# piwell/CS348B-pbrt

Measured on AMD Instinct MI355X. Metric: volumetric photon-gather throughput (camera samples through PhotonVolumeIntegrator::Li per second), higher is better.
Workload: dtype f32

## Files before the change

### cs348b-pbrt_amd/csrc/pvol_api.hip

```cpp
#include <hip/hip_runtime.h>
#include <math.h>
#include <stdlib.h>
#include <string.h>
#include <algorithm>
#include <mutex>
#include <new>
#include <vector>

#include "pvol_dev.h"

#include "pvol_host.h"

static bool ok(hipError_t e) { return e == hipSuccess; }

extern "C" {

int pvol_abi_version(void) { return PVOL_ABI_VERSION; }

const char *pvol_strerror(int s) {
    switch (s) {
    case PVOL_OK: return "ok";
    case PVOL_E_INVALID: return "invalid argument";
    case PVOL_E_NO_DEVICE: return "no usable HIP device (this library has no CPU path)";
    case PVOL_E_NO_SCENE: return "no scene set";
    case PVOL_E_NO_MEMORY: return "out of memory";
    case PVOL_E_UNSUPPORTED: return "unsupported volume/light/material kind or size";
    case PVOL_E_LIMIT: return "a ray needs more march steps than the kernel's LDS plan";
    case PVOL_E_SHOOT_FAILED: return "unable to store enough photons";
    default: return "unknown status";
    }
}

int pvol_device_count(void) {
    int n = 0;
    if (!ok(hipGetDeviceCount(&n))) return 0;
    return n;
}

void pvol_default_params(pvol_params *p) {
    memset(p, 0, sizeof(*p));
    p->step_size = 1.f;
    p->n_used = 250;
    p->max_dist = 0.1f;
    p->n_volume_photons = 0;
    p->shooter_step_size = 0.1f;
    p->max_photon_depth = 5;
    p->n_caustic_photons = 20000;
    p->n_indirect_photons = 10000;
    p->final_gather = 1;
    p->device = 0;
    p->grid_cell_scale = 0.f;
    p->keep_surface_photons = 0;
}

int pvol_create(const pvol_params *params, pvol_ctx **out) {
    if (!params || !out) return PVOL_E_INVALID;
    *out = 0;
    if (params->n_used < 1 || !(params->step_size > 0.f) || !(params->max_dist > 0.f)) return PVOL_E_INVALID;
    if (params->n_used > 576) return PVOL_E_UNSUPPORTED;
    int n = 0;
    if (!ok(hipGetDeviceCount(&n)) || n <= 0 || params->device < 0 || params->device >= n) return PVOL_E_NO_DEVICE;
    if (!ok(hipSetDevice(params->device))) return PVOL_E_NO_DEVICE;
    pvol_ctx *c = new (std::nothrow) pvol_ctx();
    if (!c) return PVOL_E_NO_MEMORY;
    c->params = *params;
    { const char *fs = getenv("PVOL_FORCE_SEQ"); c->forceSeq = fs && fs[0] == '1'; }
    { const char *ng = getenv("PVOL_NO_GROUP"); c->noGroup = ng && ng[0] == '1'; }
    { const char *nl = getenv("PVOL_NO_LITE"); c->noLite = nl && nl[0] == '1'; }
    { const char *nm = getenv("PVOL_NO_MOMENTS"); c->noMoments = nm && nm[0] == '1'; }
    { const char *gw = getenv("PVOL_GROUP_WAVES"); if (gw) c->groupWavesPerCU = std::max(1, atoi(gw)); }
    { const char *tw = getenv("PVOL_TILE_WAVES"); if (tw) c->tileWaves = std::max(0, atoi(tw)); }
    { const char *fw = getenv("PVOL_FIX_WAVES"); if (fw) c->fixWavesPerCU = std::max(1, atoi(fw)); }
    { const char *lc = getenv("PVOL_LI_COALESCE"); const long v = lc ? atol(lc) : 0; c->coMaxBatch = (v > 1 && v <= PVOL_LI_MAX_BATCH) ? (uint32_t)v : 0u; }
    { hipDeviceProp_t prop; if (ok(hipGetDeviceProperties(&prop, params->device))) c->nCU = prop.multiProcessorCount; }
    if (!c->ds.alloc(1) || !c->dCounters.alloc(1) || !c->dWords.alloc(4) || !c->dsh.alloc(1) ||
        !ok(hipMemset(c->dCounters.get(), 0, sizeof(DevCounters)))) {
        delete c;
        return PVOL_E_NO_DEVICE;
    }
    *out = c;
    return PVOL_OK;
}

void pvol_destroy(pvol_ctx *c) {
    if (!c) return;
    hipSetDevice(c->params.device);
    hipDeviceSynchronize();
    for (auto &p : c->pending) { hipEventDestroy(p.first); hipEventDestroy(p.second); }
    for (auto &p : c->pool) { hipEventDestroy(p.first); hipEventDestroy(p.second); }
    for (auto &p : c->phaseMarks) hipEventDestroy(p.second);
    for (auto &e : c->phasePool) hipEventDestroy(e);
    if (c->groupFilmEv) hipEventDestroy(c->groupFilmEv);
    if (c->groupStageEv) hipEventDestroy(c->groupStageEv);
    pvol_free_li_staging(c);
    delete c;
}

int pvol_get_accel_info(pvol_ctx *c, double *out2) {
    if (!c || !out2) return PVOL_E_INVALID;
    out2[0] = (double)c->hs.nBvhTris; out2[1] = c->bvhBuildMs;
    return PVOL_OK;
}

int pvol_push_scene(pvol_ctx *c) {
    return ok(hipMemcpy(c->ds.get(), &c->hs, sizeof(DevScene), hipMemcpyHostToDevice)) ? PVOL_OK : PVOL_E_NO_DEVICE;
}

size_t pvol_rec_stride(int maxSteps, bool grid) {
    const size_t stride = 16 + (size_t)((maxSteps + 15) & ~15) + (grid ? 8 * (size_t)maxSteps : 0);
    return (stride + 15) & ~(size_t)15;
}

BatchPlan plan_path(const PlanIn &in) {
    BatchPlan p = {};
    const bool tile = in.hasTile, grid = is_density_region(in.volKind), homog = in.volKind == PVOL_VOLUME_HOMOGENEOUS;
    const bool parOk = in.nLights <= 1 && !grid && !in.hasInit;
    const bool tileCount = tile && parOk && !in.roulette;
    const bool tileGridCount = tile && in.nLights <= 1 && grid && !in.hasInit && !in.roulette && !in.forceSeq && !in.noLite;
    const bool par = parOk && !in.forceSeq && (!tile || tileCount);
    const bool sliced = !par && !in.forceSeq && !in.transOnly && (in.volKind != PVOL_VOLUME_NONE || tile);
    p.kernel = "li_seq_kernel";
    p.path = par ? PVOL_PATH_PAR : sliced ? PVOL_PATH_SLICED : PVOL_PATH_SEQ;
    p.tile = !tile ? PVOL_TILE_NONE : !sliced ? PVOL_TILE_COUNT : tileGridCount ? PVOL_TILE_GRID_COUNT : PVOL_TILE_FUSED;
    if (p.tile == PVOL_TILE_COUNT && !tileCount) p.rc = PVOL_E_UNSUPPORTED;
    if (in.hasTauOut && grid) p.rc = PVOL_E_UNSUPPORTED;
    const bool bucket = !in.noGroup && in.g == 0.f && in.nPhotons > 0 && in.nUsed >= 10;
    if (par) {
        p.groupForm = bucket && homog && in.nUsed <= 64 && in.candCap <= 4 * 64;
#ifdef GRP_PHASE_DIAG
        const bool momStats = true;
#else
        const bool momStats = !in.statsOn;
#endif
        if (p.groupForm && in.momentTerms > 0 && in.outXYZ && !in.noMoments && momStats) p.groupForm = GRP_FORM_MOMENTS;
        p.kernel = p.groupForm ? "li_group_kernel" : "li_par_kernel";
    } else if (sliced) {
        p.liteResolve = !in.noLite && !in.roulette;
        p.resolve = p.tile == PVOL_TILE_NONE || p.tile == PVOL_TILE_GRID_COUNT;
        if (bucket && !in.statsOn && !in.roulette && (homog || grid)) p.groupForm = grid ? 2 : 1;
        p.fixGroup = p.groupForm && in.nUsed > 100 && !in.knobs.fixExact;
        p.kernel = p.groupForm ? "li_group_kernel" : "li_replay_kernel";
        if (in.specOn && !(p.tile == PVOL_TILE_FUSED && p.liteResolve)) p.rc = PVOL_E_UNSUPPORTED;
    }
    return p;
}

static int tile_waves_per_task(const PlanIn &in) {
    if (in.tileWaves > 0) return in.tileWaves;
    const double perCU = (double)in.nStreams / (double)std::max(1, in.nCU);
    return perCU >= 12.0 ? 1 : (perCU >= 3.0 ? 2 : 4);
}

void plan_size(const PlanIn &in, BatchPlan &p) {
    typedef unsigned long long ull;
    const bool slicedPath = p.path == PVOL_PATH_SLICED;
    p.ldsPar = (size_t)in.candCap * 8 + 256 * 4 + 1024 * 4; p.ldsResolve = 624 * 4 + (size_t)in.maxSteps * 4;
    p.ldsSeq = p.ldsResolve + p.ldsPar; p.ldsGroup = pvol_group_lds_bytes(in.candCap);
    if (p.tile == PVOL_TILE_FUSED) { p.ldsTile = pvol_tile_lds_bytes(in.maxSteps, in.spp, true, in.nTris, false); p.tileWavesPerTask = 1; }
    else if (p.tile != PVOL_TILE_NONE) { p.ldsTile = pvol_tile_lds_bytes(0, in.spp, false, in.nTris, in.distant != 0); p.tileWavesPerTask = tile_waves_per_task(in); }
    if (slicedPath) {
        const size_t stride = pvol_rec_stride(in.maxSteps, is_density_region(in.volKind));
        size_t m = ((size_t)4 << 30) / (stride * (size_t)in.nStreams);
        if (in.nUsed > 100) m = std::min<size_t>(m, std::max<size_t>(64, (((size_t)8 << 30) / sizeof(DeferRec) / 64) / (size_t)in.nStreams));
        if (in.specOn) m = std::min<size_t>(m, std::max<size_t>(64, ((size_t)8 << 20) / (size_t)in.nStreams));
        m = std::max<size_t>(64, std::min<size_t>(m, ((size_t)in.maxRays + 63) & ~(size_t)63));
        m &= ~(size_t)63;
        if (in.knobs.sliceRays >= 64) m = (size_t)in.knobs.sliceRays & ~(size_t)63;
        if (in.hasTile) {
            const size_t unit = std::max<size_t>(64, in.spp);
            m = std::max(unit, m / unit * unit);
        }
        p.recStride = (uint32_t)stride; p.sliceM = (uint32_t)m;
        p.nSlices = in.maxRays ? (in.maxRays + p.sliceM - 1) / p.sliceM : 1;
        p.recBytes = stride * (size_t)in.nStreams * p.sliceM; p.stateBytes = sizeof(uint32_t) * 625 * (size_t)in.nStreams;
    }
    const ull chunks = slicedPath ? (ull)((p.sliceM + 63) / 64) * in.nStreams : ((ull)in.nRays + 63ull) / 64ull;
    const ull gchunks = slicedPath ? (ull)((p.sliceM + 511) / 512) * in.nStreams : ((ull)in.nRays + 511ull) / 512ull;
    const size_t inFlight = slicedPath ? (size_t)p.sliceM * in.nStreams : (size_t)in.nRays;
    if (p.path != PVOL_PATH_SEQ) p.nWaves = (uint32_t)std::min<ull>(chunks, (ull)in.nCU * 16ull);
    p.fixWaves = (uint32_t)(in.nCU * in.fixWavesPerCU);
    if (p.groupForm) {
        p.gWaves = (uint32_t)std::min<ull>(gchunks, (ull)in.nCU * (ull)in.groupWavesPerCU);
        if (!slicedPath) p.deferWant = inFlight / 2 + 65536;
        else p.deferWant = std::min<size_t>((in.nUsed > 100 ? inFlight * 64 : inFlight) + 65536, ((size_t)8 << 30) / sizeof(DeferRec));
    }
    if (in.specOn) {
        const size_t cap = in.knobs.specPool > 0 ? (size_t)in.knobs.specPool : std::max<size_t>(65536, 2 * inFlight);
        p.specCap = std::min<size_t>(cap, (size_t)1 << 24);
    }
}

void pvol_plan_batch(const PlanIn *in, BatchPlan *out) {
    *out = plan_path(*in);
    if (out->rc == PVOL_OK) plan_size(*in, *out);
}

static float moment_sig_bar(const float *sigA, const float *sigS, double *maxDelta) {
    float lo = INFINITY, hi = -INFINITY;
    for (int b = 0; b < PVOL_NBINS; ++b) { const float t = sigA[b] + sigS[b]; lo = std::min(lo, t); hi = std::max(hi, t); }
    const float bar = (float)(0.5 * ((double)lo + (double)hi));
    *maxDelta = std::max((double)hi - (double)bar, (double)bar - (double)lo);
    return bar;
}
static int moment_terms(const float *sigA, const float *sigS, double pathBound, int maxN) {
    double maxDelta = 0.0;
    const float bar = moment_sig_bar(sigA, sigS, &maxDelta);
    if (!std::isfinite(bar) || !std::isfinite(pathBound) || !(pathBound >= 0.0)) return 0;
    const double x = maxDelta * pathBound;
    double term = exp(x);
    for (int n = 1; n <= maxN; ++n) {
        term *= x / n;
        if (term < ldexp(1.0, -25)) return n;
    }
    return 0;
}
int pvol_moment_gate(const float *sigA, const float *sigS, double pathBound) {
    if (!sigA || !sigS) return 0;
    return moment_terms(sigA, sigS, pathBound, MOM_ORDERS);
}

static double extent_world_diagonal(const DevScene &h) {
    const float *w = h.w2v;
    if (w[12] != 0.f || w[13] != 0.f || w[14] != 0.f || w[15] != 1.f) return INFINITY;
    const double m[3][3] = {{w[0], w[1], w[2]}, {w[4], w[5], w[6]}, {w[8], w[9], w[10]}};
    const double det = m[0][0] * (m[1][1] * m[2][2] - m[1][2] * m[2][1]) - m[0][1] * (m[1][0] * m[2][2] - m[1][2] * m[2][0]) +
                       m[0][2] * (m[1][0] * m[2][1] - m[1][1] * m[2][0]);
    if (!std::isfinite(det) || det == 0.0) return INFINITY;
    double inv[3][3];
    for (int i = 0; i < 3; ++i)
        for (int j = 0; j < 3; ++j) {
            const int a = (j + 1) % 3, b = (j + 2) % 3, c = (i + 1) % 3, d = (i + 2) % 3;
            inv[i][j] = (m[a][c] * m[b][d] - m[a][d] * m[b][c]) / det;
        }
    const double e[3] = {(double)h.extHi[0] - h.extLo[0], (double)h.extHi[1] - h.extLo[1], (double)h.extHi[2] - h.extLo[2]};
    double best = 0.0;
    for (int s = 0; s < 4; ++s) {
        const double v[3] = {e[0], (s & 1) ? -e[1] : e[1], (s & 2) ? -e[2] : e[2]};
        double l2 = 0.0;
        for (int i = 0; i < 3; ++i) { const double u = inv[i][0] * v[0] + inv[i][1] * v[1] + inv[i][2] * v[2]; l2 += u * u; }
        best = std::max(best, sqrt(l2));
    }
    return best * (1.0 + 1e-6);
}

int pvol_moment_scene(DevScene &h, MomentWeights *wts) {
    h.momSigBar = 0.f;
    memset(h.momEmit, 0, sizeof(h.momEmit)); memset(h.momDirect, 0, sizeof(h.momDirect));
    if (wts) memset(wts, 0, sizeof(*wts));
    if (h.volKind != PVOL_VOLUME_HOMOGENEOUS) return 0;
    const double diag = extent_world_diagonal(h);
    const int terms = moment_terms(h.sigA, h.sigS, diag, MOM_ORDERS);
    if (terms < 1 || moment_terms(h.sigA, h.sigS, 2.0 * diag, MOM_ORDERS + 1) < 1) return 0;
    double maxDelta = 0.0;
    h.momSigBar = moment_sig_bar(h.sigA, h.sigS, &maxDelta);
    const float *cie[3] = {h.cieX, h.cieY, h.cieZ};
    double emit[9] = {0}, direct[PVOL_MAX_LIGHTS][12] = {{0}};
    for (int b = 0; b < PVOL_NBINS; ++b) {
        const float sigT = h.sigA[b] + h.sigS[b];
        const double d = 0.6931471805599453 * ((double)sigT - (double)h.momSigBar);
        const double albedo = sigT != 0.f ? (double)h.sigS[b] / (double)sigT : 0.0;
        double pw = 1.0;
        for (int n = 0; n <= MOM_ORDERS; ++n) {
            for (int c = 0; c < 3; ++c) {
                if (n < MOM_ORDERS) {
                    if (wts) wts->w[4 * n + c][b] = (float)(cie[c][b] * albedo * pw);
                    emit[3 * n + c] += (double)cie[c][b] * ((double)h.sigA[b] * (double)h.le[b]) * pw;
                }
                for (int l = 0; l < h.nLights && l < PVOL_MAX_LIGHTS; ++l)
                    direct[l][3 * n + c] += (double)cie[c][b] * ((double)h.sigS[b] * (double)h.lights[l].intensity[b]) * pw;
            }
            pw *= d / (n + 1);
        }
    }
    for (int i = 0; i < 9; ++i) h.momEmit[i] = (float)emit[i];
    for (int l = 0; l < PVOL_MAX_LIGHTS; ++l) for (int i = 0; i < 12; ++i) h.momDirect[l][i] = (float)direct[l][i];
    return terms;
}

LaunchKnobs pvol_read_knobs() {
    auto num = [](const char *name) { const char *v = getenv(name); return v ? (int64_t)atoll(v) : (int64_t)0; };
    auto real = [](const char *name) { const char *v = getenv(name); return v ? (float)atof(v) : 0.f; };
    LaunchKnobs k;
    k.sliceRays = num("PVOL_SLICE_RAYS"); k.specPool = num("PVOL_SPEC_POOL"); k.tileBatchRays = num("PVOL_TILE_BATCH_RAYS");
    k.groupGuess = real("PVOL_GROUP_GUESS"); if (!(k.groupGuess >= 1.f)) k.groupGuess = 1.15f;
    k.fxgWiden = real("PVOL_FXG_WIDEN"); k.fxgAim = real("PVOL_FXG_AIM"); k.fixExact = getenv("PVOL_FIX_EXACT") != 0;
    return k;
}

static bool roulette_possible(const pvol_ctx *c) {
    float m = 0.f;
    for (int i = 0; i < PVOL_NBINS; ++i) m = std::max(m, c->hs.sigA[i] + c->hs.sigS[i]);
    const float dens = is_density_region(c->hs.volKind) ? 1.5f * c->maxDensity : 1.f;
    return !(c->hs.stepSize * m * dens < 6.8f);
}

static PlanIn plan_input(const pvol_ctx *c, const BatchArgs &b) {
    const DevScene &h = c->hs;
    PlanIn in = {};
    in.nLights = h.nLights; in.volKind = h.volKind; in.g = h.g; in.nPhotons = h.nPhotons; in.nUsed = h.nUsed; in.candCap = h.candCap;
    in.maxSteps = h.maxSteps; in.nTris = h.nTris; in.roulette = roulette_possible(c); in.distant = h.nLights > 0 && h.lights[0].kind == PVOL_LIGHT_DISTANT;
    in.forceSeq = c->forceSeq; in.noGroup = c->noGroup; in.noLite = c->noLite; in.statsOn = c->statsOn;
    in.nCU = c->nCU; in.groupWavesPerCU = c->groupWavesPerCU; in.fixWavesPerCU = c->fixWavesPerCU; in.tileWaves = c->tileWaves;
    in.nRays = b.nRays; in.nStreams = b.nStreams; in.maxRays = b.maxRaysPerStream; in.hasInit = b.initState != 0; in.transOnly = b.transOnly != 0; in.hasTile = b.tile != 0;
    in.spp = b.tile ? b.tile->spp : 0; in.specOn = b.tile && b.tile->specOn; in.hasTauOut = b.tauOut != 0;
    in.momentTerms = (int16_t)(h.mom ? c->momentTerms : 0); in.outXYZ = b.outputKind == PVOL_OUT_XYZ; in.noMoments = c->noMoments;
    in.knobs = pvol_read_knobs();
    return in;
}

bool pvol_reserve(DevBuf &b, size_t want, hipStream_t stream) {
    if (want <= b.bytes) return true;
    hipStreamSynchronize(stream);
    b.bytes = 0;
    if (!b.p.alloc(want)) return false;
    b.bytes = want;
    return true;
}

static bool harvest_events(pvol_ctx *c, bool wait) {
    size_t keep = 0;
    for (size_t i = 0; i < c->pending.size(); ++i) {
        std::pair<hipEvent_t, hipEvent_t> p = c->pending[i];
        const bool block = wait || c->pending.size() - i > 64;
        hipError_t q = block ? hipEventSynchronize(p.second) : hipEventQuery(p.second);
        if (q == hipSuccess) {
            float ms = 0.f;
            if (ok(hipEventElapsedTime(&ms, p.first, p.second))) { c->timeMs += ms; c->launches += 1; }
            c->pool.push_back(p);
        } else if (q == hipErrorNotReady) {
            c->pending[keep++] = p;
        } else {
            (void)hipGetLastError();
            c->pool.push_back(p);
            if (wait) { c->pending.erase(c->pending.begin(), c->pending.begin() + (i + 1 - keep)); return false; }
        }
    }
    c->pending.resize(keep);
    return true;
}

int pvol_order_after_pending(pvol_ctx *c, hipStream_t stream) {
    std::lock_guard<std::mutex> g(c->mu);
    harvest_events(c, false);
    for (const auto &p : c->pending)
        if (!ok(hipStreamWaitEvent(stream, p.second, 0))) return PVOL_E_NO_DEVICE;
    return PVOL_OK;
}

void pvol_phase_mark(pvol_ctx *c, hipStream_t stream, int id) {
    if (!c->phaseOn) return;
    std::lock_guard<std::mutex> g(c->mu);
    hipEvent_t e;
    if (!c->phasePool.empty()) { e = c->phasePool.back(); c->phasePool.pop_back(); }
    else if (!ok(hipEventCreate(&e))) return;
    hipEventRecord(e, stream);
    c->phaseMarks.push_back(std::make_pair(id, e));
}

static int spec_pool_reset(pvol_ctx *c, TileArgs *t, size_t cap, hipStream_t stream) {
    memset(&c->hSegStream, 0, sizeof(pvol_stream)); c->hSegStream.n_rays = (uint32_t)cap;
    pvol_ray *segRays = pvol_buf<pvol_ray>(c, PVOL_BUF_SEG_RAYS);
    uint32_t *segCounter = pvol_buf<uint32_t>(c, PVOL_BUF_SEG_COUNTER);
    if (!ok(hipMemsetAsync(segCounter, 0, 16, stream)) || !ok(hipMemcpyAsync(pvol_buf<pvol_stream>(c, PVOL_BUF_SEG_STREAM), &c->hSegStream, sizeof(pvol_stream), hipMemcpyHostToDevice, stream)) ||
        !ok(pvol_launch_spec_fill(segRays, (uint32_t)cap, stream)) || !ok(hipMemsetAsync(pvol_buf<float>(c, PVOL_BUF_SEG_OUT), 0, sizeof(float) * 60 * cap, stream)))
        return PVOL_E_NO_DEVICE;
    t->specOn = 1; t->segRays = segRays; t->segInfo = pvol_buf<SegInfo>(c, PVOL_BUF_SEG_INFO); t->segCounter = segCounter; t->segCap = (uint32_t)cap;
    t->segRecords = pvol_buf<unsigned char>(c, PVOL_BUF_SEG_RECORDS);
    return PVOL_OK;
}
static int spec_finish(pvol_ctx *c, const BatchArgs &b, const BatchPlan &p, const LiArgs &a, bool replay) {
    const size_t cap = p.specCap;
    pvol_ray *segRays = pvol_buf<pvol_ray>(c, PVOL_BUF_SEG_RAYS);
    float *segOut = pvol_buf<float>(c, PVOL_BUF_SEG_OUT);
    LiArgs sa = a;
    sa.rays = segRays; sa.nRays = (uint32_t)cap; sa.streams = pvol_buf<pvol_stream>(c, PVOL_BUF_SEG_STREAM); sa.nStreams = 1; sa.outputKind = PVOL_OUT_SPECTRAL;
    sa.out = segOut; sa.draws = 0; sa.initState = 0; sa.finalState = 0; sa.tauOut = 0; sa.defer = 0; sa.deferCount = 0; sa.deferCap = 0; sa.gated = 0;
    sa.records = pvol_buf<unsigned char>(c, PVOL_BUF_SEG_RECORDS); sa.sliceM = (uint32_t)cap; sa.sliceK = 0; sa.state = 0; sa.status = 0;
    const uint32_t nWaves = (uint32_t)std::min<unsigned long long>((cap + 63) / 64, (unsigned long long)c->nCU * 16ull);
    if (!ok(hipMemsetAsync(c->dWords.get(), 0, 4 * sizeof(uint32_t), b.stream))) return PVOL_E_NO_DEVICE;
    const RegionLaunchers &K = pvol_launchers(c->hs.volKind);
    hipError_t e = replay ? K.liReplay(&sa, p.ldsPar, c->hs.candCap, nWaves, b.stream)
                          : K.liPar(&sa, p.ldsPar, c->hs.candCap, false, nWaves, b.stream);
    if (!ok(e)) return PVOL_E_NO_DEVICE;
    SurfArgs su = {};
    su.scene = c->ds.get(); su.rays = segRays; su.nRays = (uint32_t)cap; su.out = segOut; su.tau = 0; su.surfOut = 0; su.counters = c->dCounters.get(); su.link = 0; su.spectral = 1;
    if (!ok(K.surface(&su, (uint32_t)std::min<unsigned long long>((cap + 63) / 64, (unsigned long long)c->nCU * 24ull), b.stream))) return PVOL_E_NO_DEVICE;
    SpecComposeArgs ca = {};
    ca.scene = c->ds.get(); ca.link = pvol_buf<uint32_t>(c, PVOL_BUF_SPEC_LINK); ca.info = pvol_buf<SegInfo>(c, PVOL_BUF_SEG_INFO); ca.segOut = segOut; ca.tau = a.tauOut;
    ca.out = b.out; ca.surfOut = b.specSurfOut; ca.first = 0; ca.nRays = b.nRays;
    return ok(pvol_launch_spec_compose(&ca, b.stream)) ? PVOL_OK : PVOL_E_NO_DEVICE;
}

static int run_tile_count(pvol_ctx *c, const BatchArgs &b, const BatchPlan &p, const LiArgs &t, const TileArgs *tile) {
    pvol_phase_mark(c, b.stream, PVOL_PHASE_TILE);
    return ok(pvol_launchers(c->hs.volKind).tile(&t, tile, false, p.ldsTile, c->hs.candCap, b.stream, p.tileWavesPerTask, &c->lastTileKernel)) ? PVOL_OK : PVOL_E_NO_DEVICE;
}
static int run_par(pvol_ctx *c, const BatchArgs &b, const BatchPlan &p, LiArgs &a) {
    const RegionLaunchers &K = pvol_launchers(c->hs.volKind);
    hipError_t e = p.groupForm ? K.liGroup(&a, p.ldsGroup, c->hs.candCap, c->statsOn, p.gWaves, p.fixWaves, 0, b.stream)
                               : K.liPar(&a, p.ldsPar, c->hs.candCap, c->statsOn, p.nWaves, b.stream);
    if (ok(e)) {
        a.gated = 1;
        e = K.liSeq(&a, p.ldsSeq, c->hs.candCap, c->statsOn, b.stream);
        a.gated = 0;
    }
    if (!ok(e)) return PVOL_E_NO_DEVICE;
    return p.specCap ? spec_finish(c, b, p, a, false) : PVOL_OK;
}

static int run_sliced(pvol_ctx *c, const BatchArgs &b, const BatchPlan &p, LiArgs &a, TileArgs *tile) {
    a.records = pvol_buf<unsigned char>(c, PVOL_BUF_RECORDS); a.recStride = p.recStride; a.sliceM = p.sliceM; a.state = pvol_buf<uint32_t>(c, PVOL_BUF_STATE);
    a.liteResolve = p.liteResolve; a.fixGroup = p.fixGroup;
    if (p.tile == PVOL_TILE_GRID_COUNT) {
        LiArgs t = a;
        t.sliceK = 0; t.sliceM = 0xffffffc0u; t.state = 0;
        if (run_tile_count(c, b, p, t, tile) != PVOL_OK) return PVOL_E_NO_DEVICE;
    }
    const RegionLaunchers &K = pvol_launchers(c->hs.volKind);
    for (uint32_t k = 0; k < p.nSlices; ++k) {
        a.sliceK = k;
        hipMemsetAsync(c->dWords.get(), 0, 4 * sizeof(uint32_t), b.stream);
        if (p.specCap && spec_pool_reset(c, tile, p.specCap, b.stream) != PVOL_OK) return PVOL_E_NO_DEVICE;
        if (p.tile == PVOL_TILE_FUSED) {
            pvol_phase_mark(c, b.stream, PVOL_PHASE_TILE);
            if (!ok(K.tile(&a, tile, true, p.ldsTile, c->hs.candCap, b.stream, p.tileWavesPerTask, &c->lastTileKernel))) return PVOL_E_NO_DEVICE;
        }
        pvol_phase_mark(c, b.stream, PVOL_PHASE_MARCH);
        if (!ok(K.liSlice(&a, p.ldsResolve, p.ldsPar, c->hs.candCap, c->statsOn, p.nWaves, b.stream, p.resolve != 0, p.groupForm, p.ldsGroup,
                                     p.gWaves, p.fixWaves))) return PVOL_E_NO_DEVICE;
        if (p.specCap && spec_finish(c, b, p, a, true) != PVOL_OK) return PVOL_E_NO_DEVICE;
    }
    return PVOL_OK;
}

static int run_seq(pvol_ctx *c, const BatchArgs &b, const BatchPlan &p, LiArgs &a) {
    return ok(pvol_launchers(c->hs.volKind).liSeq(&a, p.ldsSeq, c->hs.candCap, c->statsOn, b.stream)) ? PVOL_OK : PVOL_E_NO_DEVICE;
}

static int reserve_scratch(pvol_ctx *c, const BatchPlan &p, hipStream_t stream) {
    const size_t cap = p.specCap;
    if (!pvol_reserve(c->buf[PVOL_BUF_RECORDS], p.recBytes, stream) || !pvol_reserve(c->buf[PVOL_BUF_STATE], p.stateBytes, stream) ||
        !pvol_reserve(c->buf[PVOL_BUF_DEFER], p.deferWant * sizeof(DeferRec), stream) ||
        !pvol_reserve(c->buf[PVOL_BUF_SEG_RAYS], sizeof(pvol_ray) * cap, stream) || !pvol_reserve(c->buf[PVOL_BUF_SEG_INFO], sizeof(SegInfo) * cap, stream) ||
        !pvol_reserve(c->buf[PVOL_BUF_SEG_OUT], sizeof(float) * 60 * cap, stream) || !pvol_reserve(c->buf[PVOL_BUF_SEG_RECORDS], p.recStride * cap, stream) ||
        !pvol_reserve(c->buf[PVOL_BUF_SEG_COUNTER], cap ? 16 : 0, stream) || !pvol_reserve(c->buf[PVOL_BUF_SEG_STREAM], cap ? sizeof(pvol_stream) : 0, stream))
        return PVOL_E_NO_MEMORY;
    return PVOL_OK;
}

int pvol_launch_batch(pvol_ctx *c, const BatchArgs &b) {
    PlanIn in = plan_input(c, b);
    BatchPlan p = plan_path(in);
    if (p.rc != PVOL_OK) return p.rc;
    const hipStream_t stream = b.stream;
    std::pair<hipEvent_t, hipEvent_t> ev;
    {
        std::lock_guard<std::mutex> g(c->mu);
        harvest_events(c, false);
        if (!c->pool.empty()) { ev = c->pool.back(); c->pool.pop_back(); }
        else if (!ok(hipEventCreate(&ev.first)) || !ok(hipEventCreate(&ev.second))) return PVOL_E_NO_DEVICE;
    }
    struct EventReturn {
        pvol_ctx *c; std::pair<hipEvent_t, hipEvent_t> ev; bool keep = false;
        ~EventReturn() { if (!keep) { std::lock_guard<std::mutex> g(c->mu); c->pool.push_back(ev); } }
    } evGuard{c, ev};
    if (p.path == PVOL_PATH_SLICED && in.maxRays == 0) {
        std::vector<pvol_stream> hs(b.nStreams);
        if (!ok(hipMemcpyAsync(hs.data(), b.streams, sizeof(pvol_stream) * (size_t)b.nStreams, hipMemcpyDeviceToHost, stream)) ||
            !ok(hipStreamSynchronize(stream))) return PVOL_E_NO_DEVICE;
        for (uint32_t i = 0; i < b.nStreams; ++i) in.maxRays = std::max(in.maxRays, hs[i].n_rays);
    }
    plan_size(in, p);
    int rc = reserve_scratch(c, p, stream);
    if (rc != PVOL_OK) return rc;
    c->lastKernel = p.kernel;
    TileArgs tile;
    if (b.tile) tile = *b.tile;
    LiArgs a = {};
    a.scene = c->ds.get(); a.rays = b.rays; a.streams = b.streams; a.nStreams = b.nStreams; a.nRays = b.nRays; a.outputKind = b.outputKind;
    a.out = b.out; a.draws = b.draws; a.initState = b.initState; a.finalState = b.finalState; a.counters = c->dCounters.get();
    a.transmittanceOnly = b.transOnly; a.chunkCounter = c->dWords.get(); a.needSeq = c->dWords.get() + 1; a.gated = 0;
    a.tauOut = b.tauOut; a.status = b.status; a.grpGuess = in.knobs.groupGuess; a.moments = p.groupForm == GRP_FORM_MOMENTS;
    if (p.groupForm) {
        a.defer = pvol_buf<DeferRec>(c, PVOL_BUF_DEFER); a.deferCount = c->dWords.get() + 2;
        a.deferCap = (uint32_t)std::min<size_t>(c->buf[PVOL_BUF_DEFER].bytes / sizeof(DeferRec), 0xffffffffu);
        if (p.path == PVOL_PATH_SLICED) { a.fxgWiden = in.knobs.fxgWiden; a.fxgAim = in.knobs.fxgAim; }
    }
    if (p.path == PVOL_PATH_PAR) hipMemsetAsync(c->dWords.get(), 0, 3 * sizeof(uint32_t), stream);
    if (p.tile == PVOL_TILE_COUNT) {
        a.sliceK = 0; a.sliceM = 0xffffffc0u; a.state = 0;
        if (p.specCap) rc = spec_pool_reset(c, &tile, p.specCap, stream);
        if (rc == PVOL_OK) rc = run_tile_count(c, b, p, a, &tile);
        if (rc != PVOL_OK) return rc;
    }
    hipEventRecord(ev.first, stream);
    pvol_phase_mark(c, stream, PVOL_PHASE_MARCH);
    rc = p.path == PVOL_PATH_PAR ? run_par(c, b, p, a) : p.path == PVOL_PATH_SLICED ? run_sliced(c, b, p, a, &tile) : run_seq(c, b, p, a);
    if (rc != PVOL_OK) return rc;
    hipEventRecord(ev.second, stream);
    pvol_phase_mark(c, stream, PVOL_PHASE_END);
    std::lock_guard<std::mutex> g(c->mu);
    c->pending.push_back(ev);
    evGuard.keep = true;
    return PVOL_OK;
}

static int check_errors(pvol_ctx *c) {
    DevCounters h;
    if (!ok(hipMemcpy(&h, c->dCounters.get(), sizeof(h), hipMemcpyDeviceToHost))) return PVOL_E_NO_DEVICE;
    if (h.nErrors) {
        unsigned long long zero = 0;
        hipMemcpy(&c->dCounters.get()->nErrors, &zero, sizeof(zero), hipMemcpyHostToDevice);
        return PVOL_E_LIMIT;
    }
    return PVOL_OK;
}

int pvol_li_batch_device(pvol_ctx *c, const pvol_ray *dRays, uint32_t nRays, pvol_stream *dStreams, uint32_t nStreams,
                         int outputKind, float *dOut, uint32_t *dDraws, void *hipStream) {
    if (!c || (nRays && !dRays) || (nStreams && !dStreams) || (nRays && !dOut)) return PVOL_E_INVALID;
    if (outputKind != PVOL_OUT_SPECTRAL && outputKind != PVOL_OUT_XYZ) return PVOL_E_INVALID;
    if (!c->haveScene) return PVOL_E_NO_SCENE;
    if (!nStreams) return PVOL_OK;
    std::lock_guard<std::recursive_mutex> api(c->apiMu);
    if (!ok(hipSetDevice(c->params.device))) return PVOL_E_NO_DEVICE;
    BatchArgs b = {};
    b.rays = dRays; b.nRays = nRays; b.streams = dStreams; b.nStreams = nStreams; b.outputKind = outputKind; b.out = dOut; b.draws = dDraws;
    b.stream = (hipStream_t)hipStream;
    return pvol_launch_batch(c, b);
}

int pvol_check_errors(pvol_ctx *c) {
    if (!c) return PVOL_E_INVALID;
    std::lock_guard<std::recursive_mutex> api(c->apiMu);
    if (!ok(hipSetDevice(c->params.device)) || !ok(hipDeviceSynchronize())) return PVOL_E_NO_DEVICE;
    return check_errors(c);
}

static int host_batch(pvol_ctx *c, const pvol_ray *rays, uint32_t nRays, pvol_stream *streams, uint32_t nStreams, int outputKind,
                      float *out, uint32_t *draws, uint32_t *mtState, int transOnly) {
    if (!c || (nRays && (!rays || !out)) || (nStreams && !streams)) return PVOL_E_INVALID;
    if (!c->haveScene) return PVOL_E_NO_SCENE;
    std::lock_guard<std::recursive_mutex> api(c->apiMu);
    if (!ok(hipSetDevice(c->params.device))) return PVOL_E_NO_DEVICE;
    uint32_t maxRays = 1;
    {
        uint64_t next = 0;
        for (uint32_t s = 0; s < nStreams; ++s) {
            if (streams[s].first_ray != next) return PVOL_E_INVALID;
            next += streams[s].n_rays;
            maxRays = std::max(maxRays, streams[s].n_rays);
        }
        if (next != nRays) return PVOL_E_INVALID;
    }
    if (!nStreams || !nRays) return PVOL_OK;
    const size_t width = transOnly ? 60 : (outputKind == PVOL_OUT_SPECTRAL ? 60 : 4);
    DevPtr<pvol_ray> dRays; DevPtr<pvol_stream> dStreams; DevPtr<float> dOut; DevPtr<uint32_t> dDraws, dState;
    if (!dRays.alloc(nRays) || !dStreams.alloc(nStreams) || !dOut.alloc(width * nRays) || !dDraws.alloc(nRays) ||
        (mtState && !dState.alloc(625 * (size_t)nStreams)))
        return PVOL_E_NO_MEMORY;
    bool good = ok(hipMemcpy(dRays.get(), rays, sizeof(pvol_ray) * (size_t)nRays, hipMemcpyHostToDevice)) &&
                ok(hipMemcpy(dStreams.get(), streams, sizeof(pvol_stream) * (size_t)nStreams, hipMemcpyHostToDevice)) &&
                ok(hipMemset(dOut.get(), 0, sizeof(float) * width * nRays));
    if (good && mtState) good = ok(hipMemcpy(dState.get(), mtState, sizeof(uint32_t) * 625 * (size_t)nStreams, hipMemcpyHostToDevice));
    if (!good) return PVOL_E_NO_DEVICE;
    BatchArgs b = {};
    b.rays = dRays.get(); b.nRays = nRays; b.streams = dStreams.get(); b.nStreams = nStreams; b.outputKind = transOnly ? PVOL_OUT_SPECTRAL : outputKind;
    b.out = dOut.get(); b.draws = dDraws.get(); b.initState = dState.get(); b.finalState = dState.get(); b.transOnly = transOnly; b.maxRaysPerStream = maxRays;
    int rc = pvol_launch_batch(c, b);
    if (rc == PVOL_OK && !ok(hipStreamSynchronize(0))) rc = PVOL_E_NO_DEVICE;
    if (rc == PVOL_OK) rc = check_errors(c);
    if (rc != PVOL_OK) return rc;
    if (transOnly) {
        std::vector<float> tmp(width * nRays);
        good = ok(hipMemcpy(tmp.data(), dOut.get(), sizeof(float) * width * nRays, hipMemcpyDeviceToHost));
        if (good) for (uint32_t i = 0; i < nRays; ++i) memcpy(out + (size_t)i * 30, tmp.data() + (size_t)i * 60 + 30, sizeof(float) * 30);
    } else {
        good = ok(hipMemcpy(out, dOut.get(), sizeof(float) * width * nRays, hipMemcpyDeviceToHost));
    }
    good = good && ok(hipMemcpy(streams, dStreams.get(), sizeof(pvol_stream) * (size_t)nStreams, hipMemcpyDeviceToHost));
    if (good && draws) good = ok(hipMemcpy(draws, dDraws.get(), sizeof(uint32_t) * (size_t)nRays, hipMemcpyDeviceToHost));
    if (good && mtState) good = ok(hipMemcpy(mtState, dState.get(), sizeof(uint32_t) * 625 * (size_t)nStreams, hipMemcpyDeviceToHost));
    return good ? PVOL_OK : PVOL_E_NO_DEVICE;
}

int pvol_li_batch(pvol_ctx *c, const pvol_ray *rays, uint32_t nRays, pvol_stream *streams, uint32_t nStreams, int outputKind,
                  float *out, uint32_t *draws) {
    if (outputKind != PVOL_OUT_SPECTRAL && outputKind != PVOL_OUT_XYZ) return PVOL_E_INVALID;
    return host_batch(c, rays, nRays, streams, nStreams, outputKind, out, draws, 0, 0);
}

int pvol_transmittance_batch(pvol_ctx *c, const pvol_ray *rays, uint32_t nRays, pvol_stream *streams, uint32_t nStreams, float *out) {
    return host_batch(c, rays, nRays, streams, nStreams, PVOL_OUT_SPECTRAL, out, 0, 0, 1);
}

int pvol_li(pvol_ctx *c, const pvol_ray *ray, uint32_t *mt, int32_t *mti, float *Lv, float *T) {
    if (!c || !ray || !mt || !mti || !Lv || !T) return PVOL_E_INVALID;
    if (*mti < 0 || *mti > 624) return PVOL_E_INVALID;
    if (c->coMaxBatch.load(std::memory_order_relaxed) > 1) return pvol_li_coalesced(c, ray, mt, mti, Lv, T);
    return pvol_li_lone(c, ray, mt, mti, Lv, T);
}

int pvol_li_lone(pvol_ctx *c, const pvol_ray *ray, uint32_t *mt, int32_t *mti, float *Lv, float *T) {
    uint32_t state[625];
    memcpy(state, mt, sizeof(uint32_t) * 624);
    state[624] = (uint32_t)*mti;
    pvol_stream st;
    memset(&st, 0, sizeof(st));
    st.n_rays = 1;
    float out[60];
    int rc = host_batch(c, ray, 1, &st, 1, PVOL_OUT_SPECTRAL, out, 0, state, 0);
    if (rc != PVOL_OK) return rc;
    memcpy(Lv, out, sizeof(float) * 30);
    memcpy(T, out + 30, sizeof(float) * 30);
    memcpy(mt, state, sizeof(uint32_t) * 624);
    *mti = (int32_t)state[624];
    return PVOL_OK;
}

int pvol_enable_stats(pvol_ctx *c, int on) {
    if (!c) return PVOL_E_INVALID;
    c->statsOn = on != 0;
    return PVOL_OK;
}

int pvol_get_stats(pvol_ctx *c, pvol_stats *out, int reset) {
    if (!c || !out) return PVOL_E_INVALID;
    if (!ok(hipSetDevice(c->params.device)) || !ok(hipDeviceSynchronize())) return PVOL_E_NO_DEVICE;
    DevCounters h;
    if (!ok(hipMemcpy(&h, c->dCounters.get(), sizeof(h), hipMemcpyDeviceToHost))) return PVOL_E_NO_DEVICE;
    memset(out, 0, sizeof(*out));
    out->n_rays = h.nRays; out->n_steps = h.nSteps; out->n_tested = h.nTested; out->n_kept = h.nKept;
    out->n_lookups_lt10 = h.nLookupsLt10; out->n_shadow_unoccluded = h.nShadowUnoccluded;
    out->n_guess_retries = h.pad;
    out->group_guess_failed = h.diag[0]; out->group_plan_skipped = h.diag[1]; out->cy_fallback = h.diag[2];
    out->group_deferred_overflow = h.diag[3]; out->group_deferred_too_few = h.diag[4]; out->group_attempts = h.diag[5];
    out->cy_search = h.cySearch; out->cy_select = h.cySelect; out->cy_flux = h.cyFlux; out->cy_total = h.cyTotal;
    if (reset && !ok(hipMemset(c->dCounters.get(), 0, sizeof(DevCounters)))) return PVOL_E_NO_DEVICE;
    return PVOL_OK;
}

const char *pvol_march_kernel_name(pvol_ctx *c) { return c ? c->lastKernel : ""; }
const char *pvol_tile_kernel_name(pvol_ctx *c) { return c ? c->lastTileKernel : ""; }

int pvol_enable_phase_timing(pvol_ctx *c, int on) {
    if (!c) return PVOL_E_INVALID;
    c->phaseOn = on != 0;
    return PVOL_OK;
}

int pvol_get_phase_ms(pvol_ctx *c, double *out6, int reset) {
    if (!c || !out6) return PVOL_E_INVALID;
    if (!ok(hipSetDevice(c->params.device)) || !ok(hipDeviceSynchronize())) return PVOL_E_NO_DEVICE;
    std::lock_guard<std::mutex> g(c->mu);
    for (size_t i = 0; i + 1 < c->phaseMarks.size(); ++i) {
        const int id = c->phaseMarks[i].first;
        float ms = 0.f;
        if (id >= 0 && id < PVOL_N_PHASES && ok(hipEventElapsedTime(&ms, c->phaseMarks[i].second, c->phaseMarks[i + 1].second))) c->phaseMs[id] += ms;
    }
    for (size_t i = 0; i < c->phaseMarks.size(); ++i) c->phasePool.push_back(c->phaseMarks[i].second);
    c->phaseMarks.clear();
    for (int i = 0; i < PVOL_N_PHASES; ++i) out6[i] = c->phaseMs[i];
    if (reset) for (int i = 0; i < PVOL_N_PHASES; ++i) c->phaseMs[i] = 0.0;
    return PVOL_OK;
}

int pvol_kernel_time_ms(pvol_ctx *c, double *avgMs, uint64_t *launches, int reset) {
    if (!c || !avgMs) return PVOL_E_INVALID;
    std::lock_guard<std::mutex> g(c->mu);
    if (!harvest_events(c, true)) return PVOL_E_NO_DEVICE;
    *avgMs = c->launches ? c->timeMs / (double)c->launches : 0.0;
    if (launches) *launches = c->launches;
    if (reset) { c->timeMs = 0; c->launches = 0; }
    return PVOL_OK;
}

}
```

### cs348b-pbrt_amd/csrc/pvol_host.h

```cpp
#ifndef PVOL_HOST_H
#define PVOL_HOST_H
#include <hip/hip_runtime.h>
#include <atomic>
#include <condition_variable>
#include <deque>
#include <functional>
#include <mutex>
#include <vector>
#include "pvol_dev.h"

#define PVOL_LOCAL __attribute__((visibility("hidden")))

template <class T> struct PVOL_LOCAL DevPtr {
    DevPtr() {}
    DevPtr(DevPtr &&o) : p(o.release()) {}
    DevPtr &operator=(DevPtr &&o) { reset(o.release()); return *this; }
    DevPtr(const DevPtr &) = delete;
    DevPtr &operator=(const DevPtr &) = delete;
    ~DevPtr() { reset(); }
    bool alloc(size_t count) {
        reset();
        if (hipMalloc(&p, sizeof(T) * count) == hipSuccess) return true;
        p = 0; (void)hipGetLastError();
        return false;
    }
    T *get() const { return p; }
    T *release() { T *q = p; p = 0; return q; }
    void reset(T *q = 0) { if (p) hipFree(p); p = q; }
private:
    T *p = 0;
};

#include "pvol_liargs.h"
struct GridBuildArgs {
    const float *p;
    const float *wi;
    const float *alpha;
    uint32_t n;
    float lo[3];
    float inv;
    int32_t gdim[3];
    int32_t sub;
    int32_t volKind;
    float extLo[3], extHi[3];
    float w2v[16];
};
extern "C" hipError_t pvol_launch_li_seq(const LiArgs *args, size_t ldsBytes, int candCap, bool stats, hipStream_t stream);
extern "C" hipError_t pvol_launch_li_slice(const LiArgs *args, size_t ldsResolve, size_t ldsReplay, int candCap, bool stats,
                                           uint32_t nWaves, hipStream_t stream, bool resolve, int groupForm, size_t ldsGroup, uint32_t nGroupWaves,
                                           uint32_t nFixWaves);
extern "C" size_t pvol_group_lds_bytes(int candCap);
extern "C" hipError_t pvol_launch_li_group(const LiArgs *args, size_t ldsBytes, int candCap, bool stats, uint32_t nWaves, uint32_t nFixWaves,
                                           int replay, hipStream_t stream);
extern "C" hipError_t pvol_launch_spec_compose(const SpecComposeArgs *a, hipStream_t stream);
extern "C" hipError_t pvol_launch_spec_fill(pvol_ray *rays, uint32_t n, hipStream_t stream);
extern "C" hipError_t pvol_launch_li_replay(const LiArgs *args, size_t ldsReplay, int candCap, uint32_t nWaves, hipStream_t stream);
extern "C" hipError_t pvol_launch_surface(const SurfArgs *a, uint32_t nWaves, hipStream_t stream);
extern "C" size_t pvol_tile_lds_bytes(int maxSteps, uint32_t spp, bool fused, int nTris, bool shadowRows);
extern "C" hipError_t pvol_launch_tile(const LiArgs *args, const TileArgs *tile, bool fused, size_t ldsBytes, int candCap, hipStream_t stream, int wavesPerTask,
                                       const char **form);
extern "C" hipError_t pvol_launch_li_par(const LiArgs *args, size_t ldsBytes, int candCap, bool stats, uint32_t nWaves, hipStream_t stream);
struct RegionLaunchers {
    decltype(&pvol_launch_li_seq) liSeq;
    decltype(&pvol_launch_li_slice) liSlice;
    decltype(&pvol_launch_li_group) liGroup;
    decltype(&pvol_launch_li_replay) liReplay;
    decltype(&pvol_launch_li_par) liPar;
    decltype(&pvol_launch_surface) surface;
    decltype(&pvol_launch_tile) tile;
};
#if !PVOL_REGION_EXP
extern "C" hipError_t pvol_launch_li_seq_exp(const LiArgs *args, size_t ldsBytes, int candCap, bool stats, hipStream_t stream);
extern "C" hipError_t pvol_launch_li_slice_exp(const LiArgs *args, size_t ldsResolve, size_t ldsReplay, int candCap, bool stats,
                                               uint32_t nWaves, hipStream_t stream, bool resolve, int groupForm, size_t ldsGroup, uint32_t nGroupWaves,
                                               uint32_t nFixWaves);
extern "C" hipError_t pvol_launch_li_group_exp(const LiArgs *args, size_t ldsBytes, int candCap, bool stats, uint32_t nWaves, uint32_t nFixWaves,
                                               int replay, hipStream_t stream);
extern "C" hipError_t pvol_launch_li_replay_exp(const LiArgs *args, size_t ldsReplay, int candCap, uint32_t nWaves, hipStream_t stream);
extern "C" hipError_t pvol_launch_li_par_exp(const LiArgs *args, size_t ldsBytes, int candCap, bool stats, uint32_t nWaves, hipStream_t stream);
extern "C" hipError_t pvol_launch_surface_exp(const SurfArgs *a, uint32_t nWaves, hipStream_t stream);
extern "C" hipError_t pvol_launch_tile_exp(const LiArgs *args, const TileArgs *tile, bool fused, size_t ldsBytes, int candCap, hipStream_t stream,
                                           int wavesPerTask, const char **form);
static inline const RegionLaunchers &pvol_launchers(int volKind) {
    static const RegionLaunchers base = {pvol_launch_li_seq, pvol_launch_li_slice, pvol_launch_li_group, pvol_launch_li_replay, pvol_launch_li_par,
                                         pvol_launch_surface, pvol_launch_tile};
    static const RegionLaunchers expo = {pvol_launch_li_seq_exp, pvol_launch_li_slice_exp, pvol_launch_li_group_exp, pvol_launch_li_replay_exp,
                                         pvol_launch_li_par_exp, pvol_launch_surface_exp, pvol_launch_tile_exp};
    return volKind == PVOL_VOLUME_EXPONENTIAL ? expo : base;
}
#endif
extern "C" hipError_t pvol_build_grid(const GridBuildArgs *args, float4 *pos4, float4 *alpha4, float4 *wi4,
                                      uint32_t *cellStart, uint32_t *subStart, hipStream_t stream);
extern "C" hipError_t pvol_build_bvh(const float *dTri, const int32_t *dMat, const int32_t *dFlip, uint32_t n, float pad, float4 *tris,
                                     float4 *nodes, hipStream_t stream);
extern "C" hipError_t pvol_grid_occupancy(const uint32_t *cellStart, uint32_t ncells, double *sumSquares, hipStream_t stream);

#define PVOL_N_PHASES 6
enum { PVOL_PHASE_END = -1, PVOL_PHASE_TILE = 0, PVOL_PHASE_RNG = 1, PVOL_PHASE_MARCH = 2, PVOL_PHASE_SURFACE = 3, PVOL_PHASE_FILM = 4, PVOL_PHASE_OTHER = 5 };

struct PVOL_LOCAL DevBuf { DevPtr<unsigned char> p; size_t bytes = 0; };
enum {
    PVOL_BUF_RECORDS, PVOL_BUF_STATE,
    PVOL_BUF_DEFER,
    PVOL_BUF_TAU, PVOL_BUF_SPEC_LINK,
    PVOL_BUF_SEG_RAYS, PVOL_BUF_SEG_INFO, PVOL_BUF_SEG_OUT, PVOL_BUF_SEG_RECORDS,
    PVOL_BUF_SEG_COUNTER, PVOL_BUF_SEG_STREAM,
    PVOL_BUF_TILE_RAYS, PVOL_BUF_TILE_XY, PVOL_BUF_TILE_OUT, PVOL_BUF_TILE_STREAMS, PVOL_BUF_TILE_WINDOWS,
    PVOL_BUF_LI_IN, PVOL_BUF_LI_OUT,
    PVOL_BUF_GROUP_STAGE,
    PVOL_BUF_FG_DIRS, PVOL_BUF_FG_RAYS,
    PVOL_N_BUFS
};
extern "C" bool pvol_reserve(DevBuf &b, size_t want, hipStream_t stream);

struct PVOL_LOCAL PhotonGrid {
    DevPtr<float4> pos4, alpha4, wi4;
    DevPtr<uint32_t> cellStart, subStart;
    DevPtr<float> mom;
    uint32_t n = 0;
    float gridLo[3] = {0.f, 0.f, 0.f}, cellSize = 0.f, invCell = 0.f;
    int32_t gdim[3] = {0, 0, 0};
    size_t cells() const { return (size_t)gdim[0] * gdim[1] * gdim[2]; }
};

struct MapFilter { int32_t volKind; float extLo[3], extHi[3], w2v[16]; };
PVOL_LOCAL int build_photon_grid(PhotonGrid &G, const float *const raw[3], const float *hostP, uint32_t n, double minExt,
                                 const std::function<double(double)> &firstCell, const MapFilter &f);

struct PVOL_LOCAL RadianceResult {
    bool have = false;
    uint32_t n = 0;
    DevPtr<float> p, nrm, lo;
    PhotonGrid map;
};

struct PVOL_LOCAL GatherMap {
    bool have = false;
    uint32_t n = 0;
    int depth = 0;
    DevPtr<float4> nodes4;
    DevPtr<float> wi;
};

struct pvol_ctx {
    pvol_params params = {};
    bool haveScene = false;
    DevScene hs = {};
    DevPtr<DevScene> ds;
    DevPtr<float> dDensity;
    DevPtr<float4> dBvhNodes, dBvhTris;
    std::vector<int32_t> triMatHost;
    uint32_t nSceneTris = 0;
    DevPtr<float> dTriN;
    double bvhBuildMs = 0.0;
    DevPtr<float> dRawP, dRawWi, dRawAlpha;
    PhotonGrid volMap;
    DevPtr<DevCounters> dCounters;
    DevPtr<uint32_t> dWords;
    int nCU = 256;
    float maxDensity = 1.f;
    bool noLite = false;
    const char *lastKernel = "";
    const char *lastTileKernel = "";
    int fixWavesPerCU = 16;
    int groupWavesPerCU = 12;
    bool noGroup = false;
    bool forceSeq = false;
    bool noMoments = false;
    int momentTerms = 0;
    bool statsOn = false;
    std::vector<std::pair<hipEvent_t, hipEvent_t> > pending;
    std::vector<std::pair<hipEvent_t, hipEvent_t> > pool;
    double timeMs = 0.0;
    uint64_t launches = 0;
    std::mutex mu;
    int tileWaves = 0;
    bool phaseOn = false;
    std::vector<std::pair<int, hipEvent_t> > phaseMarks;
    std::vector<hipEvent_t> phasePool;
    double phaseMs[PVOL_N_PHASES] = {0, 0, 0, 0, 0, 0};
    std::recursive_mutex apiMu;
    DevBuf buf[PVOL_N_BUFS];
    DevShootScene hsh = {};
    DevPtr<DevShootScene> dsh;
    uint64_t shootStats[12] = {};
    struct PVOL_LOCAL SurfStore { DevPtr<float> p, wo, alpha; uint32_t n = 0, nPaths = 0; } surf[3];
    bool surfKept = false;
    DevPtr<float> dRad;
    uint32_t nRad = 0;
    RadianceResult rad;
    GatherMap gather;
    uint64_t fgScratchBound = 0;
    PhotonGrid causticMap;
    PhotonGrid indirectMap;
    bool specOn = false;
    pvol_stream hSegStream = {};
    double exchangeSeconds = 0.0;
    double prepSeconds[2] = {0.0, 0.0};
    std::atomic<uint32_t> coMaxBatch{0};
    uint32_t coMaxWaitUs = 0;
    std::mutex coMu;
    std::condition_variable coDone, coMore;
    std::deque<struct LiRequest *> coQueue;
    bool coBusy = false;
    uint64_t coStats[6] = {0, 0, 0, 0, 0, 0};
    hipStream_t coStream = 0;
    unsigned char *coHostIn = 0, *coHostOut = 0;
    uint32_t coCap = 0;
    hipEvent_t groupFilmEv = 0, groupStageEv = 0;
};

struct LiRequest {
    const pvol_ray *ray;
    uint32_t *mt;
    int32_t *mti;
    float *Lv, *T;
    int rc;
    bool done;
};
#define PVOL_LI_MAX_BATCH 4096u
#define PVOL_LI_MAX_WAIT_US 1000u

struct BatchArgs {
    const pvol_ray *rays; uint32_t nRays; pvol_stream *streams; uint32_t nStreams;
    int outputKind; float *out; uint32_t *draws; const uint32_t *initState; uint32_t *finalState;
    int transOnly; uint32_t maxRaysPerStream; const TileArgs *tile; hipStream_t stream;
    TauRec *tauOut;
    int32_t *status;
    float *specSurfOut;
};
extern "C" int pvol_launch_batch(pvol_ctx *c, const BatchArgs &b);
template <class T> static inline T *pvol_buf(const pvol_ctx *c, int which) { return (T *)c->buf[which].p.get(); }

struct LaunchKnobs {
    int64_t sliceRays, specPool, tileBatchRays;
    float groupGuess;
    float fxgWiden, fxgAim;
    int32_t fixExact;
};
extern "C" LaunchKnobs pvol_read_knobs();
struct PlanIn {
    int32_t nLights, volKind; float g; uint32_t nPhotons; int32_t nUsed, candCap, maxSteps, nTris;
    int32_t roulette, distant;
    int32_t forceSeq, noGroup, noLite, statsOn, nCU, groupWavesPerCU, fixWavesPerCU, tileWaves;
    uint32_t nRays, nStreams, maxRays; int32_t hasInit, transOnly, hasTile; uint32_t spp; int32_t specOn, hasTauOut;
    int16_t momentTerms; int8_t outXYZ, noMoments;
    LaunchKnobs knobs;
};
enum { PVOL_PATH_PAR, PVOL_PATH_SLICED, PVOL_PATH_SEQ };
enum { PVOL_TILE_NONE, PVOL_TILE_COUNT, PVOL_TILE_GRID_COUNT, PVOL_TILE_FUSED };
struct BatchPlan {
    int32_t rc, path, tile;
    int32_t groupForm;
    int32_t fixGroup, liteResolve;
    int32_t resolve;
    uint32_t recStride, sliceM, nSlices, nWaves, gWaves, fixWaves; int32_t tileWavesPerTask;
    uint64_t recBytes, stateBytes, deferWant, specCap, ldsSeq, ldsPar, ldsResolve, ldsGroup, ldsTile;
    const char *kernel;
};
static_assert(sizeof(PlanIn) == 152 && sizeof(BatchPlan) == 136, "tests/test_launch_plan.py mirrors both");
extern "C" size_t pvol_rec_stride(int maxSteps, bool grid);
extern "C" BatchPlan plan_path(const PlanIn &in);
extern "C" void plan_size(const PlanIn &in, BatchPlan &p);
#define GRP_FORM_MOMENTS 3
extern "C" int pvol_moment_gate(const float *sigA, const float *sigS, double pathBound);
struct MomentWeights { float w[12][32]; };
extern "C" int pvol_moment_scene(DevScene &h, MomentWeights *w);
extern "C" hipError_t pvol_fill_moments(const MomentWeights *w, const float4 *alpha4, float *mom, uint32_t n, hipStream_t stream);

extern "C" {
void pvol_phase_mark(pvol_ctx *c, hipStream_t stream, int id);
int pvol_finish_map(pvol_ctx *c, uint32_t n, const float *hostPositions);
void pvol_free_photons(pvol_ctx *c);
void pvol_free_surface_stores(pvol_ctx *c);
void pvol_free_caustic_map(pvol_ctx *c);
int pvol_push_scene(pvol_ctx *c);
int pvol_li_lone(pvol_ctx *c, const pvol_ray *ray, uint32_t *mt, int32_t *mti, float *Lv, float *T);
int pvol_li_coalesced(pvol_ctx *c, const pvol_ray *ray, uint32_t *mt, int32_t *mti, float *Lv, float *T);
void pvol_free_li_staging(pvol_ctx *c);
int pvol_order_after_pending(pvol_ctx *c, hipStream_t stream);
void *pvol_rccl_symbol(const char *name);
void pvol_plan_batch(const PlanIn *in, BatchPlan *out);
int pvol_gather_tree_build(const float *p, uint32_t n, void *nodes, int32_t *depth);
struct GatherCheck {
    const pvol_photon_array *indirect;
    const float *p; uint32_t count; float maxDist;
    const void *outIndex, *outD2, *outFound, *outRounds;
    const float *frames, *wo, *uBsdf, *uPhoton; int32_t nSamples; float cosGatherAngle; const void *outBsdf, *outPhoton;
};
int pvol_check_gather(int what, int haveCtx, int haveState, uint32_t storeN, const GatherCheck *args, int hostPointers);
struct FinalGatherCheck {
    const float *p, *frames, *wo, *kd, *rayEps; uint32_t count; float maxDist; int32_t nSamples; float cosGatherAngle;
    const float *uBsdf, *uPhoton; const void *L, *draws;
};
int pvol_check_final_gather(int haveCtx, const FinalGatherCheck *args, int haveScene, int volKind, int haveGather, int haveRad, uint32_t radN);
uint32_t pvol_final_gather_slice(int32_t nSamples, uint64_t bound);
int pvol_final_gather_set_scratch_bound(pvol_ctx *c, uint64_t bytes);
size_t pvol_shoot_merge_replay(const uint32_t *cfg, const uint32_t *tables, uint32_t nTables, uint64_t *out, size_t cap);
size_t pvol_render_plan_flat(const pvol_camera *camera, const pvol_film *film, const pvol_film_window *window, const pvol_sampler *smp,
                             const uint32_t *taskIds, uint32_t nTaskIds, const int32_t *flags, int64_t tileBatchRays, uint64_t *out, size_t cap);
int pvol_check_scene(const pvol_params *params, const pvol_scene *s);
int pvol_check_triangle_normals(const pvol_scene *s, const float *n, uint32_t nTriangles);
int pvol_check_exponential(const pvol_volume *v, float *up3);
int pvol_check_radiance(int what, int haveCtx, int haveState, int32_t nLookup, float maxDist, const pvol_photon_array *const *maps, const float *a,
                        const float *b, const float *rhoR, const float *rhoT, uint32_t count, const void *outLo, const void *outFound, int hostPointers);
int pvol_check_surface_maps(const pvol_surface_params *sp, int haveScene, int materials, int storesKept, const uint32_t *storeN,
                            const uint32_t *storePaths, const pvol_photon_array *caustic, const pvol_photon_array *indirect, int hostPointers);
int pvol_probe_hits(pvol_ctx *c, const pvol_ray *rays, uint32_t n, int mode, float *out, int32_t *outi);
float pvol_exponential_max_density(const pvol_volume *v, const float *up3);
}

struct PVOL_LOCAL SceneImage {
    DevScene scene;
    DevShootScene shoot;
    float maxDensity;
    float bvhPad;
    std::vector<int32_t> primMat;
};
PVOL_LOCAL int pvol_scene_image(const pvol_params *params, const pvol_scene *s, SceneImage *out);

PVOL_LOCAL void pvol_map_to_scene(const PhotonGrid &G, DevScene &h);
PVOL_LOCAL int pvol_map_moments(const PhotonGrid &G, DevScene &h, DevPtr<float> &mom, int *terms);

static inline bool pvol_window_ok(const pvol_film *f, const pvol_film_window *w) {
    return !w || (w->x_pixel_start >= 0 && w->y_pixel_start >= 0 && w->x_pixel_count > 0 && w->y_pixel_count > 0 &&
                  w->x_pixel_count <= f->x_resolution - w->x_pixel_start && w->y_pixel_count <= f->y_resolution - w->y_pixel_start);
}
static inline pvol_film_window pvol_window_or_full(const pvol_film *f, const pvol_film_window *w) {
    if (w) return *w;
    pvol_film_window full = {0, 0, f->x_resolution, f->y_resolution};
    return full;
}
static inline bool film_ok(const pvol_film *f) {
    return f && f->x_resolution > 0 && f->y_resolution > 0 && f->filter_xwidth > 0.f && f->filter_ywidth > 0.f &&
           f->filter_xwidth <= 3.f && f->filter_ywidth <= 3.f;
}
PVOL_LOCAL int film_add(pvol_ctx *c, const pvol_film *film, const pvol_film_window *window, const float *dXY, const float *dXYZ, uint32_t stride,
                        uint64_t n, int guard, float *dPixels, hipStream_t stream);

static inline uint64_t pvol_task_samples(const pvol_sampler *s, uint32_t task, int32_t win[4]) {
    pvol_compute_sub_window(s, task, win);
    return (uint64_t)(win[1] - win[0]) * (uint64_t)(win[3] - win[2]) * s->pixel_samples;
}
struct RenderBatch {
    uint32_t b0, b1;
    uint32_t maxRays;
    int32_t surfOn, specOn;
    uint64_t nRays;
    uint64_t doneRays;
    uint64_t want[7];
};
struct PVOL_LOCAL RenderPlan {
    int rc;
    TileArgs tile;
    uint64_t batchRays;
    std::vector<int32_t> win;
    std::vector<uint64_t> count;
    std::vector<pvol_stream> streams;
    std::vector<RenderBatch> batches;
};
PVOL_LOCAL RenderPlan pvol_render_plan(const pvol_camera *camera, const pvol_film *film, const pvol_film_window *window, const pvol_sampler *smp,
                                       const uint32_t *taskIds, uint32_t nTaskIds, bool havePixels, bool haveScene, bool surfOn, bool specOn,
                                       int64_t tileBatchRays);
PVOL_LOCAL int render_share(pvol_ctx *c, const pvol_camera *camera, const pvol_film *film, const pvol_film_window *window, const pvol_sampler *smp,
                            uint32_t rank, uint32_t nRanks, float *dPixels, hipStream_t stream);
#endif
```

### cs348b-pbrt_amd/csrc/pvol_tile_dev.h

```cpp

__device__ __forceinline__ float sobol2(uint32_t n, uint32_t scramble) {
    for (uint32_t v = 1u << 31; n != 0; n >>= 1, v ^= v >> 1)
        if (n & 0x1) scramble ^= v;
    return fminf(((scramble >> 8) & 0xffffff) / float(1 << 24), 0x1.fffffep-1f);
}

template <bool WG1 = true>
__device__ void tile_shuffle(float *samp, uint32_t count, uint32_t dims, uint32_t *oth, Rng &rng, int lane, bool skipSwaps = false) {
    for (uint32_t base = 0; base < count; base += LANES) {
        const int cnt = (int)min((uint32_t)LANES, count - base);
        const uint32_t r = rng_bulk<WG1>(rng, cnt, lane);
        const uint32_t i = base + (uint32_t)lane;
        if (lane < cnt) oth[i] = i + (r % (count - i));
    }
    rng_sync<WG1>();
    if (lane == 0 && !skipSwaps) {
        uint32_t oNext = oth[0];
        for (uint32_t i = 0; i < count; ++i) {
            const uint32_t o = oNext;
            if (i + 1 < count) oNext = oth[i + 1];
            if (dims == 2) {
                float2 *s2 = reinterpret_cast<float2 *>(samp);
                const float2 a = s2[i], b = s2[o];
                s2[i] = b;
                s2[o] = a;
            } else {
                for (uint32_t j = 0; j < dims; ++j) {
                    float a = samp[dims * i + j], b = samp[dims * o + j];
                    samp[dims * i + j] = b;
                    samp[dims * o + j] = a;
                }
            }
        }
    }
    rng_sync<WG1>();
}

struct TileLds {
    float *image;
    float *time;
    float *scatter;
    uint32_t *oth;
};

template <bool WG1 = true>
__device__ void tile_pixel_sample(const TileArgs &T, TileLds &L, Rng &rng, int lane) {
    const uint32_t n = T.spp;
    {
        const uint32_t s0 = rng_uint<true, WG1>(rng, lane), s1 = rng_uint<true, WG1>(rng, lane);
        for (uint32_t i = lane; i < n; i += LANES) { L.image[2 * i] = van_der_corput(i, s0); L.image[2 * i + 1] = sobol2(i, s1); }
        rng_skip<true, WG1>(rng, n, lane);
        rng_sync<WG1>();
        tile_shuffle<WG1>(L.image, n, 2, L.oth, rng, lane, (T.debugSkip & 1u) != 0u);
    }
    rng_skip<true, WG1>(rng, 2ull + 2ull * n, lane);
    {
        const uint32_t s = rng_uint<true, WG1>(rng, lane);
        for (uint32_t i = lane; i < n; i += LANES) L.time[i] = van_der_corput(i, s);
        rng_skip<true, WG1>(rng, n, lane);
        rng_sync<WG1>();
        tile_shuffle<WG1>(L.time, n, 1, L.oth, rng, lane, (T.debugSkip & 1u) != 0u);
    }
    unsigned long long pend = 0ull;
    for (uint32_t a = 0; a < T.n1dCount; ++a) {
        if (a == T.scatterIndex) {
            if (pend) { rng_skip<true, WG1, true>(rng, pend, lane); pend = 0ull; }
            const uint32_t s = rng_uint<true, WG1>(rng, lane);
            for (uint32_t i = lane; i < n; i += LANES) L.scatter[i] = van_der_corput(i, s);
            rng_skip<true, WG1>(rng, n, lane);
            rng_sync<WG1>();
            tile_shuffle<WG1>(L.scatter, n, 1, L.oth, rng, lane, (T.debugSkip & 1u) != 0u);
        } else {
            pend += 1ull + (unsigned long long)T.n1d[a] * n + n;
        }
    }
    for (uint32_t a = 0; a < T.n2dCount; ++a) pend += 2ull + (unsigned long long)T.n2d[a] * n + n;
    if (pend) rng_skip<true, WG1, true>(rng, pend, lane);
}

__device__ __forceinline__ void tile_camera_ray(const TileArgs &T, float imageX, float imageY, V3 *o, V3 *d) {
    const float *m = T.r2c;
    V3 pc;
    pc.x = m[0] * imageX + m[1] * imageY + m[2] * 0.f + m[3];
    pc.y = m[4] * imageX + m[5] * imageY + m[6] * 0.f + m[7];
    pc.z = m[8] * imageX + m[9] * imageY + m[10] * 0.f + m[11];
    const float w = m[12] * imageX + m[13] * imageY + m[14] * 0.f + m[15];
    if (w != 1.f) { const float inv = 1.f / w; pc.x *= inv; pc.y *= inv; pc.z *= inv; }
    const V3 dir = normalize(pc);
    const float *c = T.c2w;
    V3 ow = v3(c[0] * 0.f + c[1] * 0.f + c[2] * 0.f + c[3], c[4] * 0.f + c[5] * 0.f + c[6] * 0.f + c[7],
               c[8] * 0.f + c[9] * 0.f + c[10] * 0.f + c[11]);
    const float ww = c[12] * 0.f + c[13] * 0.f + c[14] * 0.f + c[15];
    if (ww != 1.f) { const float inv = 1.f / ww; ow.x *= inv; ow.y *= inv; ow.z *= inv; }
    *o = ow;
    *d = xform_vector(c, dir);
}

__device__ __forceinline__ float tile_clip(const float *ltri, int nTris, V3 o, V3 d) {
    float mt = INFINITY;
    for (int i = 0; i < nTris; ++i) {
        const f4 a = *reinterpret_cast<const f4 *>(ltri + 12 * i), b = *reinterpret_cast<const f4 *>(ltri + 12 * i + 4),
                 c = *reinterpret_cast<const f4 *>(ltri + 12 * i + 8);
        float t;
        if (tri_closest_v(v3(a.x, a.y, a.z), v3(a.w, b.x, b.y), v3(b.z, b.w, c.x), o, d, 0.f, mt, &t)) mt = t;
    }
    return mt;
}

struct CountConsts {
    float w2v[16];
    float lo[3], hi[3];
    float stepSize;
    int volKind, nLights, nTris, lightKind;
    bool bvh;
    int nSpheres;
    float ldir[3], lpos[3], w2l[9], cosTotalWidth, cosFalloffStart;
};
__device__ __forceinline__ CountConsts count_consts(const DevScene &S) {
    CountConsts C;
    for (int i = 0; i < 16; ++i) C.w2v[i] = S.w2v[i];
    for (int i = 0; i < 3; ++i) { C.lo[i] = S.extLo[i]; C.hi[i] = S.extHi[i]; }
    C.stepSize = S.stepSize; C.volKind = S.volKind; C.nLights = S.nLights; C.nTris = S.nTris; C.bvh = S.bvhNodes != 0; C.nSpheres = S.nSpheres;
    const DevLight &light = S.lights[0];
    C.lightKind = light.kind;
    for (int i = 0; i < 3; ++i) { C.ldir[i] = light.dir[i]; C.lpos[i] = light.pos[i]; }
    for (int r = 0; r < 3; ++r) for (int c = 0; c < 3; ++c) C.w2l[3 * r + c] = light.w2l[4 * r + c];
    C.cosTotalWidth = light.cosTotalWidth; C.cosFalloffStart = light.cosFalloffStart;
    return C;
}

__device__ uint32_t tile_count_draws(const DevScene &S, const CountConsts &C, const float *ltri, const float *trows, V3 o, V3 d, float maxt, float scatterU, bool blackS, bool lightBlack, uint32_t dbg = 0u,
                                     int slice = 0, int nSlices = 1, float mint = 0.f) {
    float t0, t1;
    if (C.volKind == PVOL_VOLUME_NONE || !box_intersect(C.lo, C.hi, xform_point(C.w2v, o), xform_vector(C.w2v, d), mint, maxt, &t0, &t1) || (t1 - t0) == 0.f) return 0u;
    const int nSamples = (int)ceilf((t1 - t0) / C.stepSize);
    const float step = (t1 - t0) / nSamples;
    float tcur = t0 + scatterU * step;
    uint32_t u = 0;
    const bool tryLight = !blackS && C.nLights > 0 && !lightBlack;
    const uint32_t fixedDraws = slice == 0 ? 4u + 7u * (uint32_t)nSamples : 0u;
    if (!tryLight || (dbg & 16u)) return fixedDraws;
    if (trows && !C.bvh && !C.nSpheres && !(dbg & 8u)) {
        const V3 ld = v3(C.ldir[0], C.ldir[1], C.ldir[2]);
        for (int j = 0; j < nSamples; j += 2) {
            const V3 pA = o + d * tcur;
            tcur += step;
            const V3 pB = o + d * tcur;
            tcur += step;
            if (nSlices > 1 && ((j >> 1) % nSlices) != slice) continue;
            const V3 pvA = xform_point(C.w2v, pA), pvB = xform_point(C.w2v, pB);
            bool inA, inB = j + 1 < nSamples;
            if (is_region(C.volKind)) { inA = region_density(S, pvA) != 0.f; inB = inB && region_density(S, pvB) != 0.f; }
            else { inA = box_inside(C.lo, C.hi, pvA); inB = inB && box_inside(C.lo, C.hi, pvB); }
            if (!inA && !inB) continue;
            bool occA = false, occB = false;
            for (int t = 0; t < C.nTris; ++t) {
                const f4 r0 = *reinterpret_cast<const f4 *>(trows + 16 * t), r1 = *reinterpret_cast<const f4 *>(trows + 16 * t + 4),
                         r2 = *reinterpret_cast<const f4 *>(trows + 16 * t + 8), r3 = *reinterpret_cast<const f4 *>(trows + 16 * t + 12);
                TriPre tp;
                tp.p1 = v3(r0.x, r0.y, r0.z); tp.e1 = v3(r0.w, r1.x, r1.y); tp.e2 = v3(r1.z, r1.w, r2.x); tp.s1 = v3(r2.y, r2.z, r2.w);
                tp.invDivisor = r3.x; tp.valid = r3.y != 0.f;
                occA = occA | tri_test(tp, pA, ld, 0.f, INFINITY);
                occB = occB | tri_test(tp, pB, ld, 0.f, INFINITY);
            }
            u += ((inA && !occA) ? 1u : 0u) + ((inB && !occB) ? 1u : 0u);
        }
        return fixedDraws + u;
    }
    for (int j = 0; j < nSamples; ++j) {
        const V3 p = o + d * tcur;
        tcur += step;
        if (nSlices > 1 && (j % nSlices) != slice) continue;
        const V3 pv = xform_point(C.w2v, p);
        if (is_region(C.volKind) ? region_density(S, pv) == 0.f : !box_inside(C.lo, C.hi, pv)) continue;
        RayD vis;
        if (C.lightKind == PVOL_LIGHT_DISTANT) {
            vis.o = p; vis.d = v3(C.ldir[0], C.ldir[1], C.ldir[2]); vis.mint = 0.f; vis.maxt = INFINITY;
        } else {
            const V3 lp = v3(C.lpos[0], C.lpos[1], C.lpos[2]);
            const V3 wo = normalize(lp - p);
            const float dist = len(p - lp);
            vis.o = p; vis.d = vdiv(lp - p, dist); vis.mint = 0.f; vis.maxt = dist * (1.f - 0.f);
            if (C.lightKind == PVOL_LIGHT_SPOT) {
                V3 wl = normalize(v3(C.w2l[0] * -wo.x + C.w2l[1] * -wo.y + C.w2l[2] * -wo.z,
                                     C.w2l[3] * -wo.x + C.w2l[4] * -wo.y + C.w2l[5] * -wo.z,
                                     C.w2l[6] * -wo.x + C.w2l[7] * -wo.y + C.w2l[8] * -wo.z));
                const float costheta = wl.z;
                float fall = 1.f;
                if (costheta < C.cosTotalWidth) fall = 0.f;
                else if (!(costheta > C.cosFalloffStart)) {
                    const float delta = (costheta - C.cosTotalWidth) / (C.cosFalloffStart - C.cosTotalWidth);
                    fall = delta * delta * delta * delta;
                }
                if (fall == 0.f) continue;
            }
        }
        bool occ = false;
        if (C.nSpheres && spheres_occluded(S, vis.o, vis.d, vis.mint, vis.maxt)) {
            occ = true;
        } else if (C.bvh) {
            occ = bvh_occluded(S, vis.o, vis.d, vis.mint, vis.maxt);
        } else if (trows) {
            if (!(dbg & 8u)) occ = tri_rows_occluded(trows, C.nTris, vis.o, vis.d, vis.mint, vis.maxt);
        } else {
            for (int t = 0; t < ((dbg & 8u) ? 0 : C.nTris); ++t) {
                const f4 a = *reinterpret_cast<const f4 *>(ltri + 12 * t), b = *reinterpret_cast<const f4 *>(ltri + 12 * t + 4),
                         c = *reinterpret_cast<const f4 *>(ltri + 12 * t + 8);
                occ = occ | tri_hit_v(v3(a.x, a.y, a.z), v3(a.w, b.x, b.y), v3(b.z, b.w, c.x), vis);
            }
        }
        if (!occ) ++u;
    }
    return fixedDraws + u;
}

struct SpecCountPol {
    const DevScene *S; const CountConsts *C; const float *ltri, *trows; float su; bool blackS, lightBlack;
    uint32_t total;
    __device__ void visit(SpecCtx &X, int, int, int, float, float, float, V3 o, V3 d, float mint, float maxt) {
        total += X.pending + tile_count_draws(*S, *C, ltri, trows, o, d, maxt, su, blackS, lightBlack, 0u, 0, 1, mint);
        X.pending = 0u;
    }
};
struct SpecEmitPol {
    pvol_ray *rays; SegInfo *info; uint32_t base, sample; float su, time;
    __device__ void visit(SpecCtx &X, int D, int lobe, int mat, float Fs, float awz, float g, V3 o, V3 d, float mint, float maxt) {
        const uint32_t idx = base + X.nSeg;
        pvol_ray r;
        r.o[0] = o.x; r.o[1] = o.y; r.o[2] = o.z; r.mint = mint;
        r.d[0] = d.x; r.d[1] = d.y; r.d[2] = d.z; r.maxt = maxt;
        r.time = time; r.scatter_u = su; r.rng_skip = X.pending; r.flags = 0u;
        rays[idx] = r;
        SegInfo si;
        si.sample = sample; si.depthLobeMat = (uint32_t)D | ((uint32_t)lobe << 8) | ((uint32_t)mat << 16);
        si.Fs = Fs; si.awz = awz; si.g = g; si.pad[0] = si.pad[1] = si.pad[2] = 0u;
        info[idx] = si;
        X.pending = 0u;
    }
};
template <bool SPEC>
__device__ uint32_t tile_surface_draws(const DevScene &S, const TileArgs &T, const CountConsts &CC, const float *ltri, const float *trows, const SurfHit &sh,
                                       V3 d, float su, float tm, size_t ri, bool blackS, bool lightBlack, unsigned blackMask, DevCounters *counters, uint32_t *link) {
    *link = 0u;
    if (!SPEC || S.shootScene->mats[sh.mat].kind == PVOL_MATERIAL_MATTE || !T.specOn) return surf_count_draws(S, sh, d, blackMask);
    if constexpr (SPEC) {
    SpecCtx X;
    X.blackMask = blackMask; X.pending = 0u; X.nSeg = 0u;
    SpecCountPol cp;
    cp.S = &S; cp.C = &CC; cp.ltri = ltri; cp.trows = trows; cp.su = su; cp.blackS = blackS; cp.lightBlack = lightBlack; cp.total = 0u;
    spec_surface<0>(S, X, cp, d, sh);
    const uint32_t draws = cp.total + X.pending, n = X.nSeg;
    if (n) {
        const uint32_t base = atomicAdd(T.segCounter, n);
        if (base + n <= T.segCap) {
            SpecEmitPol ep;
            ep.rays = T.segRays; ep.info = T.segInfo; ep.base = base; ep.sample = (uint32_t)ri; ep.su = su; ep.time = tm;
            X.pending = 0u; X.nSeg = 0u;
            spec_surface<0>(S, X, ep, d, sh);
            *link = (base << SPEC_LINK_COUNT_BITS) | n;
        } else {
            atomicAdd(&counters->nErrors, 1ull);
        }
    }
    return draws;
    }
    return 0u;
}

struct SpecNullPol {
    __device__ void visit(SpecCtx &X, int, int, int, float, float, float, V3, V3, float, float) { X.pending = 0u; }
};
struct SpecWalkPol {
    const DevScene *S; const LiArgs *A; const TileArgs *T; Rng *rng; float *lightNum;
    uint32_t base, sample; float su, time; int lane; bool grid, blackS; unsigned blackMask;
    __device__ void visit(SpecCtx &X, int D, int lobe, int mat, float Fs, float awz, float g, V3 o, V3 d, float mint, float maxt) {
        rng_skip<true>(*rng, X.pending, lane);
        const uint32_t idx = base + X.nSeg;
        pvol_ray r;
        r.o[0] = o.x; r.o[1] = o.y; r.o[2] = o.z; r.mint = mint;
        r.d[0] = d.x; r.d[1] = d.y; r.d[2] = d.z; r.maxt = maxt;
        r.time = time; r.scatter_u = su; r.rng_skip = X.pending; r.flags = 0u;
        if (lane == 0) {
            T->segRays[idx] = r;
            SegInfo si;
            si.sample = sample; si.depthLobeMat = (uint32_t)D | ((uint32_t)lobe << 8) | ((uint32_t)mat << 16);
            si.Fs = Fs; si.awz = awz; si.g = g; si.pad[0] = si.pad[1] = si.pad[2] = 0u;
            T->segInfo[idx] = si;
        }
        X.pending = 0u;
        RayRec rec = ray_rec(T->segRecords + (size_t)idx * A->recStride, S->maxSteps, grid);
        const unsigned long long r0 = rng->draws;
        const int nSteps = geo_ray(*S, *A, r, rec, lane, grid, blackS, blackMask);
        lite_ray(*S, rec, nSteps, *rng, lightNum, lane, grid, S->nLights);
        if (lane == 0) rec.hdr[2] = (uint32_t)(rng->draws - r0);
    }
};

template <bool FUSED, int NREG, bool SPEC>
__global__ __launch_bounds__(LANES, FUSED ? 2 : 4) void tile_kernel(LiArgs A, TileArgs T) {
    extern __shared__ __align__(16) unsigned char lds[];
    const DevScene &S = *A.scene;
    const int lane = threadIdx.x;
    const uint32_t sidx = blockIdx.x;
    if (sidx >= A.nStreams) return;
    uint32_t *mt = reinterpret_cast<uint32_t *>(lds);
    MarchLds M;
    M.G.cap = 0; M.G.cd = 0; M.G.ci = 0; M.G.paint = 0;
    M.lightNum = reinterpret_cast<float *>(lds + MT_N * 4);
    M.prevRk = 0;
    TileLds L;
    L.image = M.lightNum + (FUSED ? ((S.maxSteps + 1) & ~1) : 0);
    L.time = L.image + 2 * T.spp;
    L.scatter = L.time + T.spp;
    L.oth = reinterpret_cast<uint32_t *>(L.scatter + T.spp);
    const size_t triOff = (((size_t)MT_N * 4 + (FUSED ? (size_t)((S.maxSteps + 1) & ~1) * 4 : 0) + (size_t)T.spp * 5 * 4) + 15) & ~(size_t)15;
    float *ltri = reinterpret_cast<float *>(lds + triOff);
    for (int i = lane; i < S.nTris * 12; i += LANES) {
        const int t = i / 12, c = i - 12 * t;
        const DevTri &tr = S.tris[t];
        ltri[i] = c < 3 ? tr.p1[c] : c < 6 ? tr.p2[c - 3] : c < 9 ? tr.p3[c - 6] : 0.f;
    }
    __syncthreads();
    float *trows = 0;
    if (!FUSED && S.nLights > 0 && S.lights[0].kind == PVOL_LIGHT_DISTANT) {
        trows = ltri + S.nTris * 12;
        tri_rows_prepare(S, v3(S.lights[0].dir[0], S.lights[0].dir[1], S.lights[0].dir[2]), trows, lane);
    }
    const pvol_stream st = A.streams[sidx];
    const uint32_t begin = A.sliceK * A.sliceM;
    if (begin >= st.n_rays && !(A.sliceK == 0)) return;
    Rng rng;
    rng.mt = mt;
    rng.draws = 0;
    uint32_t *state = A.state ? A.state + (size_t)sidx * (MT_N + 1) : 0;
    if (A.sliceK == 0) {
        mt_seed(mt, st.seed, lane);
        rng.mti = MT_N;
        rng_skip<true>(rng, st.start_draw, lane);
    } else {
        for (int i = lane; i < MT_N; i += LANES) mt[i] = state[i];
        rng.mti = (int)state[MT_N];
        rng.draws = st.end_draw;
        __syncthreads();
    }
    WaveCounters wc = {};
    const bool grid = is_region(S.volKind);
    const uint32_t end = min(st.n_rays, begin + A.sliceM);
    const int4 w = T.windows[sidx];
    const uint32_t width = (uint32_t)(w.y - w.x);
    const int q = lane & 7;
    const bool blackS = spec_is_black(ld4(S.sigS, q));
    const bool lightBlack = S.nLights > 0 ? spec_is_black(ld4(S.lights[0].intensity, q)) : true;
    unsigned blackMask = 0u;
    for (int l = 0; l < S.nLights; ++l) if (spec_is_black(ld4(S.lights[l].intensity, q))) blackMask |= 1u << l;
    const bool surfOn = S.surf.enabled != 0;
    pvol_ray *rays = T.rays;
    const CountConsts CC = count_consts(S);
    for (uint32_t k = begin; k < end; k += T.spp) {
        const uint32_t pix = k / T.spp;
        const int xPos = w.x + (int)(pix % width), yPos = w.z + (int)(pix / width);
        const unsigned long long d0 = rng.draws;
        tile_pixel_sample(T, L, rng, lane);
        const uint32_t samplerDraws = (uint32_t)(rng.draws - d0);
        for (uint32_t s0 = 0; s0 < T.spp; s0 += LANES) {
            const uint32_t i = s0 + (uint32_t)lane;
            const bool on = i < T.spp;
            const int cnt = (int)min((uint32_t)LANES, T.spp - s0);
            float imageX = 0.f, imageY = 0.f, tm = 0.f, su = 0.f, maxt = INFINITY;
            V3 o = v3(0.f, 0.f, 0.f), d = v3(0.f, 0.f, 1.f);
            const size_t ri = (size_t)st.first_ray + k + i;
            uint32_t surfDraws = 0u;
            int glass = 0;
            if (on) {
                imageX = xPos + L.image[2 * i];
                imageY = yPos + L.image[2 * i + 1];
                tm = lerpf(L.time[i], T.shutterOpen, T.shutterClose);
                su = L.scatter[i];
                tile_camera_ray(T, imageX, imageY, &o, &d);
                if (S.bvhNodes) { float th; if (bvh_closest(S, o, d, 0.f, INFINITY, &th) >= 0) maxt = th; }
                else maxt = tile_clip(ltri, S.nTris, o, d);
                if (S.nSpheres) { V3 ph; spheres_closest(S, o, d, 0.f, &maxt, &ph); }
                uint32_t link = 0u;
                if (surfOn && maxt < INFINITY) {
                    SurfHit sh;
                    if (surf_closest(S, o, d, 0.f, &sh)) {
                        if (!FUSED) surfDraws = tile_surface_draws<SPEC>(S, T, CC, ltri, trows, sh, d, su, tm, ri, blackS, lightBlack, blackMask, A.counters, &link);
                        else if (!SPEC || S.shootScene->mats[sh.mat].kind == PVOL_MATERIAL_MATTE || !T.specOn) surfDraws = surf_count_draws(S, sh, d, blackMask);
                        else glass = 1;
                    }
                }
                if (!FUSED && T.specLink) T.specLink[ri] = link;
                pvol_ray pr;
                pr.o[0] = o.x; pr.o[1] = o.y; pr.o[2] = o.z; pr.mint = 0.f;
                pr.d[0] = d.x; pr.d[1] = d.y; pr.d[2] = d.z; pr.maxt = maxt;
                pr.time = tm; pr.scatter_u = su; pr.rng_skip = ((i == 0) ? samplerDraws : 0u) + surfDraws; pr.flags = 0u;
                rays[ri] = pr;
                T.xy[2 * ri] = imageX;
                T.xy[2 * ri + 1] = imageY;
            }
            if (!FUSED) {
                uint32_t nd = (on && !(T.debugSkip & 2u)) ? tile_count_draws(S, CC, ltri, trows, o, d, maxt, su, blackS, lightBlack, T.debugSkip) : ((T.debugSkip & 2u) ? 270u : 0u);
                unsigned long long tot = nd + surfDraws;
                for (int off = 32; off > 0; off >>= 1) tot += __shfl_xor(tot, off);
                if (!(T.debugSkip & 4u)) rng_skip<true, true, true>(rng, tot, lane);

            } else {
                for (int j = 0; j < cnt; ++j) {
                    pvol_ray pr;
                    pr.o[0] = lane_f(o.x, j); pr.o[1] = lane_f(o.y, j); pr.o[2] = lane_f(o.z, j); pr.mint = 0.f;
                    pr.d[0] = lane_f(d.x, j); pr.d[1] = lane_f(d.y, j); pr.d[2] = lane_f(d.z, j); pr.maxt = lane_f(maxt, j);
                    pr.time = lane_f(tm, j); pr.scatter_u = lane_f(su, j); pr.rng_skip = 0u; pr.flags = 0u;
                    const size_t rj = (size_t)st.first_ray + k + s0 + (uint32_t)j;
                    if (surfOn) {
                        uint32_t linkj = 0u;
                        bool walked = false;
                        if constexpr (SPEC) if (lane_i(glass, j)) {
                            walked = true;
                            const unsigned long long t0 = rng.draws;
                            const V3 oj = v3(pr.o[0], pr.o[1], pr.o[2]), dj = v3(pr.d[0], pr.d[1], pr.d[2]);
                            SurfHit shj;
                            shj.tri = 0; shj.mat = 0; shj.t = 0.f; shj.rayEps = 0.f; shj.p = shj.nn = shj.dpdu = v3(0.f, 0.f, 0.f);
                            surf_closest(S, oj, dj, 0.f, &shj);
                            SpecCtx X;
                            X.blackMask = blackMask; X.pending = 0u; X.nSeg = 0u;
                            SpecNullPol np;
                            spec_surface<0>(S, X, np, dj, shj);
                            const uint32_t nSeg = X.nSeg;
                            uint32_t base = 0u;
                            if (nSeg) { if (lane == 0) base = atomicAdd(T.segCounter, nSeg); base = (uint32_t)lane_i((int)base, 0); }
                            X.pending = 0u; X.nSeg = 0u;
                            if (nSeg && base + nSeg <= T.segCap && A.liteResolve) {
                                SpecWalkPol wp;
                                wp.S = &S; wp.A = &A; wp.T = &T; wp.rng = &rng; wp.lightNum = M.lightNum; wp.base = base; wp.sample = (uint32_t)rj;
                                wp.su = pr.scatter_u; wp.time = pr.time; wp.lane = lane; wp.grid = grid; wp.blackS = blackS; wp.blackMask = blackMask;
                                spec_surface<0>(S, X, wp, dj, shj);
                                linkj = (base << SPEC_LINK_COUNT_BITS) | nSeg;
                            } else {
                                if (nSeg && lane == 0) atomicAdd(&A.counters->nErrors, 1ull);
                                spec_surface<0>(S, X, np, dj, shj);
                            }
                            rng_skip<true>(rng, X.pending, lane);
                            if (lane == j) rays[rj].rng_skip += (uint32_t)(rng.draws - t0);
                        }
                        if (!walked) rng_skip<true>(rng, (unsigned long long)lane_i((int)surfDraws, j), lane);
                        if (T.specLink && lane == j) T.specLink[rj] = linkj;
                    }
                    const unsigned long long r0 = rng.draws;
                    RayRec rec = ray_rec(A.records + ((size_t)sidx * A.sliceM + (k + s0 + (uint32_t)j - begin)) * A.recStride, S.maxSteps, grid);
                    if (A.liteResolve) {
                        const int nSteps = geo_ray(S, A, pr, rec, lane, grid, (T.debugSkip & 32u) ? true : blackS, blackMask);
                        if (T.debugSkip & 128u) rng_skip<true>(rng, 4ull + 7ull * (unsigned long long)nSteps, lane);
                        else lite_ray(S, rec, nSteps, rng, M.lightNum, lane, grid, (T.debugSkip & 64u) ? 1 : S.nLights, (T.debugSkip & 256u) != 0u);
                    } else {
                        f4 Lv, Tr;
                        march_ray<false, MODE_RESOLVE, NREG>(S, A, pr, rng, M, lane, wc, &Lv, &Tr, rec);
                    }
                    if (lane == 0) rec.hdr[2] = (uint32_t)(rng.draws - r0);
                    if (A.draws && lane == 0) A.draws[rj] = (uint32_t)(rng.draws - r0);
                }
            }
        }
    }
    if (lane == 0) A.streams[sidx].end_draw = rng.draws;
    if (state) {
        __syncthreads();
        for (int i = lane; i < MT_N; i += LANES) state[i] = mt[i];
        if (lane == 0) state[MT_N] = (uint32_t)rng.mti;
    }
}

template <int NW, bool SPEC>
__global__ __launch_bounds__(LANES * NW, (NW >= 8 ? 4 : 2)) void tile_mw_kernel(LiArgs A, TileArgs T, uint32_t partOff) {
    extern __shared__ __align__(16) unsigned char lds[];
    constexpr bool W1 = (NW == 1);
    const DevScene &S = *A.scene;
    const int tid = threadIdx.x, lane = tid & (LANES - 1), wave = tid / LANES;
    const uint32_t sidx = blockIdx.x;
    if (sidx >= A.nStreams) return;
    uint32_t *mt = reinterpret_cast<uint32_t *>(lds);
    TileLds L;
    L.image = reinterpret_cast<float *>(lds + MT_N * 4);
    L.time = L.image + 2 * T.spp;
    L.scatter = L.time + T.spp;
    L.oth = reinterpret_cast<uint32_t *>(L.scatter + T.spp);
    const size_t triOff = (((size_t)MT_N * 4 + (size_t)T.spp * 5 * 4) + 15) & ~(size_t)15;
    float *ltri = reinterpret_cast<float *>(lds + triOff);
    const bool shadowRows = S.nLights > 0 && S.lights[0].kind == PVOL_LIGHT_DISTANT;
    const size_t partHere = (triOff + (size_t)S.nTris * 12 * 4 + (shadowRows ? (size_t)S.nTris * 16 * 4 : 0) + 64 + 15) & ~(size_t)15;
    unsigned long long *part = reinterpret_cast<unsigned long long *>(lds + partHere);
    for (int i = tid; i < S.nTris * 12; i += LANES * NW) {
        const int t = i / 12, c = i - 12 * t;
        const DevTri &tr = S.tris[t];
        ltri[i] = c < 3 ? tr.p1[c] : c < 6 ? tr.p2[c - 3] : c < 9 ? tr.p3[c - 6] : 0.f;
    }
    __syncthreads();
    float *trows = 0;
    if (S.nLights > 0 && S.lights[0].kind == PVOL_LIGHT_DISTANT) {
        trows = ltri + S.nTris * 12;
        tri_rows_prepare(S, v3(S.lights[0].dir[0], S.lights[0].dir[1], S.lights[0].dir[2]), trows, tid);
    }
    const pvol_stream st = A.streams[sidx];
    Rng rng;
    rng.mt = mt; rng.draws = 0; rng.mti = MT_N;
    if (wave == 0) {
        mt_seed<W1>(mt, st.seed, lane);
        rng_skip<true, W1>(rng, st.start_draw, lane);
    }
    const int4 w = T.windows[sidx];
    const uint32_t width = (uint32_t)(w.y - w.x);
    const int q = lane & 7;
    const bool blackS = spec_is_black(ld4(S.sigS, q));
    const bool lightBlack = S.nLights > 0 ? spec_is_black(ld4(S.lights[0].intensity, q)) : true;
    unsigned blackMask = 0u;
    for (int l = 0; l < S.nLights; ++l) if (spec_is_black(ld4(S.lights[l].intensity, q))) blackMask |= 1u << l;
    const bool surfOn = S.surf.enabled != 0;
    pvol_ray *rays = T.rays;
    const CountConsts CC = count_consts(S);
    const int groupsPerPixel = (int)((T.spp + LANES - 1) / LANES);
    const int G = groupsPerPixel < NW ? groupsPerPixel : NW;
    const int NSL = NW / G;
    const int g = wave % G, slice = wave / G;
    for (uint32_t k = 0; k < st.n_rays; k += T.spp) {
        const uint32_t pix = k / T.spp;
        const int xPos = w.x + (int)(pix % width), yPos = w.z + (int)(pix / width);
        uint32_t samplerDraws = 0u;
        if (wave == 0) {
            const unsigned long long d0 = rng.draws;
            tile_pixel_sample<W1>(T, L, rng, lane);
            samplerDraws = (uint32_t)(rng.draws - d0);
        }
        __syncthreads();
        unsigned long long mine = 0ull;
        for (uint32_t s0 = (uint32_t)g * LANES; s0 < T.spp; s0 += (uint32_t)G * LANES) {
            const uint32_t i = s0 + (uint32_t)lane;
            if (i >= T.spp) continue;
            const float imageX = xPos + L.image[2 * i], imageY = yPos + L.image[2 * i + 1];
            const float tm = lerpf(L.time[i], T.shutterOpen, T.shutterClose), su = L.scatter[i];
            V3 o, d;
            tile_camera_ray(T, imageX, imageY, &o, &d);
            float maxt = INFINITY;
            if (S.bvhNodes) { float th; if (bvh_closest(S, o, d, 0.f, INFINITY, &th) >= 0) maxt = th; }
            else maxt = tile_clip(ltri, S.nTris, o, d);
            if (S.nSpheres) { V3 ph; spheres_closest(S, o, d, 0.f, &maxt, &ph); }
            if (slice == 0) {
                uint32_t surfDraws = 0u;
                const size_t ri = (size_t)st.first_ray + k + i;
                uint32_t link = 0u;
                if (surfOn && maxt < INFINITY) {
                    SurfHit sh;
                    if (surf_closest(S, o, d, 0.f, &sh)) surfDraws = tile_surface_draws<SPEC>(S, T, CC, ltri, trows, sh, d, su, tm, ri, blackS, lightBlack, blackMask, A.counters, &link);
                }
                if (T.specLink) T.specLink[ri] = link;
                pvol_ray pr;
                pr.o[0] = o.x; pr.o[1] = o.y; pr.o[2] = o.z; pr.mint = 0.f;
                pr.d[0] = d.x; pr.d[1] = d.y; pr.d[2] = d.z; pr.maxt = maxt;
                pr.time = tm; pr.scatter_u = su; pr.rng_skip = ((i == 0) ? samplerDraws : 0u) + surfDraws; pr.flags = 0u;
                rays[ri] = pr;
                T.xy[2 * ri] = imageX;
                T.xy[2 * ri + 1] = imageY;
                mine += surfDraws;
            }
            if (!(T.debugSkip & 2u)) mine += tile_count_draws(S, CC, ltri, trows, o, d, maxt, su, blackS, lightBlack, 0u, slice, NSL);
            else if (slice == 0) mine += 270ull;
        }
        for (int off = 32; off > 0; off >>= 1) mine += __shfl_xor(mine, off);
        if (lane == 0) part[wave] = mine;
        __syncthreads();
        if (wave == 0) {
            unsigned long long tot = lane < NW ? part[lane] : 0ull;
            for (int off = 32; off > 0; off >>= 1) tot += __shfl_xor(tot, off);
            if (!(T.debugSkip & 4u)) rng_skip<true, W1>(rng, tot, lane);
        }
    }
    if (wave == 0 && lane == 0) A.streams[sidx].end_draw = rng.draws;
}

extern "C" size_t pvol_tile_lds_bytes(int maxSteps, uint32_t spp, bool fused, int nTris, bool shadowRows) {
    return (((size_t)MT_N * 4 + (fused ? (size_t)((maxSteps + 1) & ~1) * 4 : 0) + (size_t)spp * 5 * 4 + 15) & ~(size_t)15) + (size_t)nTris * 12 * 4 +
           (shadowRows ? (size_t)nTris * 16 * 4 : 0) + 64;
}

template <bool SPEC>
static hipError_t launch_tile_t(const LiArgs *args, const TileArgs *tile, bool fused, size_t ldsBytes, int candCap, hipStream_t stream, int wavesPerTask,
                                const char **form) {
    dim3 grid(args->nStreams), block(LANES);
    if (!fused && wavesPerTask > 1 && args->state == 0 && args->sliceK == 0) {
        const uint32_t partOff = (uint32_t)((ldsBytes + 15) & ~(size_t)15);
        const size_t bytes = partOff + 16 * 8;
        if (wavesPerTask >= 16) { *form = "tile_mw_kernel<16>"; hipLaunchKernelGGL((tile_mw_kernel<16, SPEC>), grid, dim3(LANES * 16), bytes, stream, *args, *tile, partOff); }
        else if (wavesPerTask >= 8) { *form = "tile_mw_kernel<8>"; hipLaunchKernelGGL((tile_mw_kernel<8, SPEC>), grid, dim3(LANES * 8), bytes, stream, *args, *tile, partOff); }
        else if (wavesPerTask >= 4) { *form = "tile_mw_kernel<4>"; hipLaunchKernelGGL((tile_mw_kernel<4, SPEC>), grid, dim3(LANES * 4), bytes, stream, *args, *tile, partOff); }
        else { *form = "tile_mw_kernel<2>"; hipLaunchKernelGGL((tile_mw_kernel<2, SPEC>), grid, dim3(LANES * 2), bytes, stream, *args, *tile, partOff); }
        return hipGetLastError();
    }
    *form = fused ? "tile_kernel<fused>" : "tile_kernel<count>";
    if (!fused) hipLaunchKernelGGL((tile_kernel<false, 4, SPEC>), grid, block, ldsBytes, stream, *args, *tile);
    else if (candCap <= 4 * LANES) hipLaunchKernelGGL((tile_kernel<true, 4, SPEC>), grid, block, ldsBytes, stream, *args, *tile);
    else hipLaunchKernelGGL((tile_kernel<true, 12, SPEC>), grid, block, ldsBytes, stream, *args, *tile);
    return hipGetLastError();
}
extern "C" hipError_t pvol_launch_tile(const LiArgs *args, const TileArgs *tile, bool fused, size_t ldsBytes, int candCap, hipStream_t stream, int wavesPerTask,
                                       const char **form) {
    return tile->specOn ? launch_tile_t<true>(args, tile, fused, ldsBytes, candCap, stream, wavesPerTask, form)
                        : launch_tile_t<false>(args, tile, fused, ldsBytes, candCap, stream, wavesPerTask, form);
}
```

### cs348b-pbrt_amd/pvol.py

```python
import ctypes as C
import os

import numpy as np

from . import abi

_HERE = os.path.dirname(os.path.abspath(__file__))
LIB_PATH = os.environ.get("PVOL_LIB") or os.path.join(_HERE, "libpvol.so")

_f32p = C.POINTER(C.c_float)
_u32p = C.POINTER(C.c_uint32)


class PvolError(RuntimeError):
    def __init__(self, status, where):
        self.status = status
        RuntimeError.__init__(self, "%s: %s (%d)" % (where, lib().pvol_strerror(status).decode(), status))


ALLGATHER_FN = C.CFUNCTYPE(C.c_int, C.c_void_p, C.c_void_p, C.c_void_p, C.c_uint64)


class ShootComm(C.Structure):
    _fields_ = [("nccl_comm", C.c_void_p), ("allgather", ALLGATHER_FN), ("user", C.c_void_p)]


GATHER_K = 50
GATHER_SAMPLE_DTYPE = np.dtype([("wi", "<f4", 3), ("weight", "<f4"), ("bsdf_pdf", "<f4"), ("photon_pdf", "<f4"), ("photon_index", "<u4"), ("valid", "<u4")])
GATHER_NODE_DTYPE = np.dtype([("p", "<f4", 3), ("split_pos", "<f4"), ("split_axis", "<u4"), ("has_left_child", "<u4"), ("right_child", "<u4"),
                              ("index", "<u4")])
GATHER_RAY_DTYPE = np.dtype([("t", "<f4"), ("n_gather", "<f4", 3), ("radiance_index", "<u4"), ("prim", "<i4"), ("hit", "<u4"), ("drew", "<u4")])
GATHER_NONE = 0xffffffff
assert GATHER_SAMPLE_DTYPE.itemsize == 32 and GATHER_NODE_DTYPE.itemsize == 32 and GATHER_RAY_DTYPE.itemsize == 32


class GatherCheck(C.Structure):
    _fields_ = [("indirect", C.POINTER(abi.PhotonArray)), ("p", _f32p), ("count", C.c_uint32), ("max_dist", C.c_float),
                ("out_index", C.c_void_p), ("out_d2", C.c_void_p), ("out_found", C.c_void_p), ("out_rounds", C.c_void_p),
                ("frames", _f32p), ("wo", _f32p), ("u_bsdf", _f32p), ("u_photon", _f32p), ("n_samples", C.c_int32), ("cos_gather_angle", C.c_float),
                ("out_bsdf", C.c_void_p), ("out_photon", C.c_void_p)]


class FinalGatherCheck(C.Structure):
    _fields_ = [("p", _f32p), ("frames", _f32p), ("wo", _f32p), ("kd", _f32p), ("ray_eps", _f32p), ("count", C.c_uint32), ("max_dist", C.c_float),
                ("n_samples", C.c_int32), ("cos_gather_angle", C.c_float), ("u_bsdf", _f32p), ("u_photon", _f32p), ("L", C.c_void_p),
                ("draws", C.c_void_p)]


def gather_cos_angle(gather_angle):
    rad = np.float32(np.float32(np.float32(3.14159265358979323846) / np.float32(180.0)) * np.float32(gather_angle))
    return float(np.float32(np.cos(np.float64(rad))))


def gather_tree(p):
    p = np.ascontiguousarray(p, np.float32).reshape(-1)
    n = p.size // 3
    nodes, depth = np.zeros(n, GATHER_NODE_DTYPE), C.c_int32()
    _check(lib().pvol_gather_tree_build(p.ctypes.data_as(_f32p), n, nodes.ctypes.data, C.byref(depth)), "pvol_gather_tree_build")
    return nodes, depth.value


def gloo_allgather(group=None):
    import torch
    import torch.distributed as dist

    def allgather(data):
        n = dist.get_world_size(group)
        if not data:
            return [b""] * n
        t = torch.frombuffer(bytearray(data), dtype=torch.uint8)
        out = [torch.empty_like(t) for _ in range(n)]
        dist.all_gather(out, t, group=group)
        return [o.numpy().tobytes() for o in out]
    return allgather


_lib = None


def lib():
    global _lib
    if _lib is None:
        if not os.path.exists(LIB_PATH):
            raise ImportError("%s is missing: run `python -c 'import __graft_entry__ as g; g.build()'` "
                              "(hipcc --offload-arch=gfx950); there is no fallback path" % LIB_PATH)
        L = C.CDLL(LIB_PATH)
        L.pvol_abi_version.restype = C.c_int
        L.pvol_strerror.restype = C.c_char_p
        L.pvol_strerror.argtypes = [C.c_int]
        L.pvol_device_count.restype = C.c_int
        L.pvol_default_params.argtypes = [C.POINTER(abi.Params)]
        L.pvol_default_params.restype = None
        L.pvol_create.argtypes = [C.POINTER(abi.Params), C.POINTER(C.c_void_p)]
        L.pvol_destroy.argtypes = [C.c_void_p]
        L.pvol_destroy.restype = None
        L.pvol_set_scene.argtypes = [C.c_void_p, C.POINTER(abi.Scene)]
        L.pvol_set_triangle_normals.argtypes = [C.c_void_p, _f32p, C.c_uint32]
        L.pvol_check_triangle_normals.argtypes = [C.POINTER(abi.Scene), _f32p, C.c_uint32]
        L.pvol_upload_photons.argtypes = [C.c_void_p, _f32p, _f32p, _f32p, C.c_uint32]
        L.pvol_preprocess.argtypes = [C.c_void_p, C.c_uint32]
        L.pvol_preprocess_blocks.argtypes = [C.c_void_p, C.c_uint32, C.c_uint32]
        L.pvol_preprocess_ranks.argtypes = [C.c_void_p, C.c_uint32, C.c_uint32, C.c_uint32, C.c_uint32, C.POINTER(ShootComm)]
        L.pvol_get_exchange_seconds.argtypes = [C.c_void_p, C.POINTER(C.c_double)]
        L.pvol_photon_count.argtypes = [C.c_void_p, _u32p]
        L.pvol_download_photons.argtypes = [C.c_void_p, _f32p, _f32p, _f32p, C.c_uint32]
        L.pvol_li_batch.argtypes = [C.c_void_p, C.c_void_p, C.c_uint32, C.c_void_p, C.c_uint32, C.c_int, _f32p, _u32p]
        L.pvol_li_batch_device.argtypes = [C.c_void_p, C.c_void_p, C.c_uint32, C.c_void_p, C.c_uint32, C.c_int,
                                           C.c_void_p, C.c_void_p, C.c_void_p]
        L.pvol_li.argtypes = [C.c_void_p, C.c_void_p, _u32p, C.POINTER(C.c_int32), _f32p, _f32p]
        L.pvol_li_many.argtypes = [C.c_void_p, C.c_void_p, C.c_uint32, _u32p, C.POINTER(C.c_int32), _f32p, _f32p, C.POINTER(C.c_int32)]
        L.pvol_set_li_coalescing.argtypes = [C.c_void_p, C.c_uint32, C.c_uint32]
        L.pvol_get_li_coalescing_stats.argtypes = [C.c_void_p, C.POINTER(C.c_uint64), C.c_int]
        L.pvol_transmittance_batch.argtypes = [C.c_void_p, C.c_void_p, C.c_uint32, C.c_void_p, C.c_uint32, _f32p]
        L.pvol_get_stats.argtypes = [C.c_void_p, C.POINTER(abi.Stats), C.c_int]
        L.pvol_enable_stats.argtypes = [C.c_void_p, C.c_int]
        L.pvol_kernel_time_ms.argtypes = [C.c_void_p, C.POINTER(C.c_double), C.POINTER(C.c_uint64), C.c_int]
        L.pvol_get_shoot_stats.argtypes = [C.c_void_p, C.POINTER(C.c_uint64)]
        L.pvol_march_kernel_name.argtypes = [C.c_void_p]
        L.pvol_check_errors.argtypes = [C.c_void_p]
        L.pvol_get_preprocess_seconds.argtypes = [C.c_void_p, C.POINTER(C.c_double)]
        L.pvol_get_accel_info.argtypes = [C.c_void_p, C.POINTER(C.c_double)]
        L.pvol_surface_photon_count.argtypes = [C.c_void_p, C.c_int, _u32p, _u32p]
        L.pvol_download_surface_photons.argtypes = [C.c_void_p, C.c_int, _f32p, _f32p, _f32p, C.c_uint32]
        L.pvol_radiance_photon_count.argtypes = [C.c_void_p, _u32p]
        L.pvol_download_radiance_photons.argtypes = [C.c_void_p, _f32p, _f32p, _f32p, _f32p, C.c_uint32]
        L.pvol_compute_radiance.argtypes = [C.c_void_p, C.c_int32, C.c_float]
        L.pvol_compute_radiance_arrays.argtypes = [C.c_void_p, C.c_int32, C.c_float, C.POINTER(C.POINTER(abi.PhotonArray)), _f32p, _f32p, _f32p, _f32p,
                                                   C.c_uint32]
        L.pvol_radiance_lo_count.argtypes = [C.c_void_p, _u32p]
        L.pvol_download_radiance_lo.argtypes = [C.c_void_p, _f32p, _f32p, _f32p, C.c_uint32]
        L.pvol_radiance_lookup.argtypes = [C.c_void_p, _f32p, _f32p, C.c_uint32, _f32p, _u32p]
        L.pvol_radiance_lookup_device.argtypes = [C.c_void_p, C.c_void_p, C.c_void_p, C.c_uint32, C.c_void_p, C.c_void_p, C.c_void_p]
        L.pvol_check_radiance.argtypes = [C.c_int, C.c_int, C.c_int, C.c_int32, C.c_float, C.POINTER(C.POINTER(abi.PhotonArray)), _f32p, _f32p, _f32p,
                                          _f32p, C.c_uint32, C.c_void_p, C.c_void_p, C.c_int]
        L.pvol_build_gather_map.argtypes = [C.c_void_p]
        L.pvol_build_gather_map_arrays.argtypes = [C.c_void_p, C.POINTER(abi.PhotonArray)]
        L.pvol_gather_map_count.argtypes = [C.c_void_p, _u32p]
        L.pvol_gather_photons.argtypes = [C.c_void_p, _f32p, C.c_uint32, C.c_float, _u32p, _f32p, _u32p, _u32p]
        L.pvol_gather_photons_device.argtypes = [C.c_void_p, C.c_void_p, C.c_uint32, C.c_float, C.c_void_p, C.c_void_p, C.c_void_p, C.c_void_p, C.c_void_p]
        L.pvol_gather_directions.argtypes = [C.c_void_p, _f32p, _f32p, _f32p, C.c_uint32, C.c_float, C.c_int32, C.c_float, _f32p, _f32p, C.c_void_p,
                                             C.c_void_p]
        L.pvol_gather_directions_device.argtypes = [C.c_void_p, C.c_void_p, C.c_void_p, C.c_void_p, C.c_uint32, C.c_float, C.c_int32, C.c_float,
                                                    C.c_void_p, C.c_void_p, C.c_void_p, C.c_void_p, C.c_void_p]
        L.pvol_gather_tree_build.argtypes = [_f32p, C.c_uint32, C.c_void_p, C.POINTER(C.c_int32)]
        L.pvol_check_gather.argtypes = [C.c_int, C.c_int, C.c_int, C.c_uint32, C.POINTER(GatherCheck), C.c_int]
        L.pvol_final_gather.argtypes = [C.c_void_p, _f32p, _f32p, _f32p, _f32p, _f32p, C.c_uint32, C.c_float, C.c_int32, C.c_float, _f32p, _f32p,
                                        _f32p, _u32p, C.c_void_p, C.c_void_p]
        L.pvol_final_gather_device.argtypes = [C.c_void_p] + [C.c_void_p] * 5 + [C.c_uint32, C.c_float, C.c_int32, C.c_float] + [C.c_void_p] * 7
        L.pvol_check_final_gather.argtypes = [C.c_int, C.POINTER(FinalGatherCheck), C.c_int, C.c_int, C.c_int, C.c_int, C.c_uint32]
        L.pvol_final_gather_slice.argtypes = [C.c_int32, C.c_uint64]
        L.pvol_final_gather_slice.restype = C.c_uint32
        L.pvol_final_gather_set_scratch_bound.argtypes = [C.c_void_p, C.c_uint64]
        L.pvol_probe_hits.argtypes =[C.c_void_p, C.c_void_p, C.c_uint32, C.c_int, _f32p, C.POINTER(C.c_int32)]
        L.pvol_set_surface_integrator.argtypes = [C.c_void_p, C.POINTER(abi.SurfaceParams), _f32p, _f32p, _f32p, C.c_uint32]
        L.pvol_set_surface_integrator_maps.argtypes = [C.c_void_p, C.POINTER(abi.SurfaceParams), C.POINTER(abi.PhotonArray), C.POINTER(abi.PhotonArray)]
        L.pvol_check_surface_maps.argtypes = [C.POINTER(abi.SurfaceParams), C.c_int, C.c_int, C.c_int, _u32p, _u32p, C.POINTER(abi.PhotonArray),
                                              C.POINTER(abi.PhotonArray), C.c_int]
        L.pvol_march_kernel_name.restype = C.c_char_p
        L.pvol_tile_kernel_name.argtypes = [C.c_void_p]
        L.pvol_tile_kernel_name.restype = C.c_char_p
        L.pvol_gaussian_filter_table.argtypes = [C.c_float, C.c_float, C.c_float, _f32p]
        L.pvol_gaussian_filter_table.restype = None
        L.pvol_compute_sub_window.argtypes = [C.POINTER(abi.Sampler), C.c_uint32, C.POINTER(C.c_int32)]
        L.pvol_compute_sub_window.restype = None
        L.pvol_render_sample_count.argtypes = [C.POINTER(abi.Sampler), _u32p, C.c_uint32]
        L.pvol_render_sample_count.restype = C.c_uint64
        L.pvol_render_tasks_device.argtypes = [C.c_void_p, C.POINTER(abi.Camera), C.POINTER(abi.Film), C.POINTER(abi.Sampler), _u32p, C.c_uint32,
                                               C.c_void_p, C.POINTER(abi.RenderDebug), C.c_void_p]
        L.pvol_film_add_samples_device.argtypes = [C.c_void_p, C.POINTER(abi.Film), C.c_void_p, C.c_void_p, C.c_uint32, C.c_uint64, C.c_void_p, C.c_void_p]
        L.pvol_film_resolve_device.argtypes = [C.c_void_p, C.POINTER(abi.Film), C.c_void_p, C.c_void_p, C.c_void_p]
        L.pvol_partition_tasks.argtypes = [C.c_uint32, C.c_uint32, C.c_uint32, _u32p, C.c_uint32, _u32p]
        L.pvol_render_frame_ranks.argtypes = [C.c_void_p, C.POINTER(abi.Camera), C.POINTER(abi.Film), C.POINTER(abi.Sampler), C.c_uint32, C.c_uint32,
                                              C.c_void_p, C.c_void_p, C.c_void_p, C.c_void_p]
        L.pvol_preprocess_group.argtypes = [C.POINTER(C.c_void_p), C.c_uint32, C.c_uint32, C.c_uint32]
        L.pvol_render_frame_group.argtypes = [C.POINTER(C.c_void_p), C.c_uint32, C.POINTER(abi.Camera), C.POINTER(abi.Film), C.POINTER(abi.Sampler),
                                              C.POINTER(C.c_void_p), C.c_void_p, C.POINTER(C.c_void_p)]
        _cam, _film, _win, _smp = C.POINTER(abi.Camera), C.POINTER(abi.Film), C.POINTER(abi.FilmWindow), C.POINTER(abi.Sampler)
        L.pvol_film_window_from_crop.argtypes = [_film, _f32p, _win]
        L.pvol_film_sample_extent.argtypes = [_film, _win, C.POINTER(C.c_int32)]
        L.pvol_render_tasks_window_device.argtypes = [C.c_void_p, _cam, _film, _win, _smp, _u32p, C.c_uint32, C.c_void_p, C.POINTER(abi.RenderDebug),
                                                      C.c_void_p]
        L.pvol_film_add_samples_window_device.argtypes = [C.c_void_p, _film, _win, C.c_void_p, C.c_void_p, C.c_uint32, C.c_uint64, C.c_void_p, C.c_void_p]
        L.pvol_film_resolve_window_device.argtypes = [C.c_void_p, _film, _win, C.c_void_p, C.c_void_p, C.c_void_p]
        L.pvol_render_frame_ranks_window.argtypes = [C.c_void_p, _cam, _film, _win, _smp, C.c_uint32, C.c_uint32, C.c_void_p, C.c_void_p, C.c_void_p,
                                                     C.c_void_p]
        L.pvol_render_frame_group_window.argtypes = [C.POINTER(C.c_void_p), C.c_uint32, _cam, _film, _win, _smp, C.POINTER(C.c_void_p), C.c_void_p,
                                                     C.POINTER(C.c_void_p)]
        L.pvol_enable_phase_timing.argtypes = [C.c_void_p, C.c_int]
        L.pvol_get_phase_ms.argtypes = [C.c_void_p, C.POINTER(C.c_double), C.c_int]
        _lib = L
    return _lib


EXPORTS = ["pvol_abi_version", "pvol_strerror", "pvol_device_count", "pvol_default_params", "pvol_create",
           "pvol_destroy", "pvol_set_scene", "pvol_upload_photons", "pvol_preprocess", "pvol_photon_count",
           "pvol_download_photons", "pvol_li_batch", "pvol_li_batch_device", "pvol_li", "pvol_transmittance_batch",
           "pvol_get_stats", "pvol_enable_stats", "pvol_kernel_time_ms", "pvol_get_shoot_stats",
           "pvol_gaussian_filter_table", "pvol_compute_sub_window", "pvol_render_sample_count", "pvol_render_tasks_device",
           "pvol_film_add_samples_device", "pvol_film_resolve_device", "pvol_march_kernel_name", "pvol_check_errors", "pvol_get_preprocess_seconds", "pvol_get_accel_info", "pvol_surface_photon_count",
           "pvol_download_surface_photons", "pvol_radiance_photon_count", "pvol_download_radiance_photons",
           "pvol_set_surface_integrator", "pvol_enable_phase_timing", "pvol_get_phase_ms",
           "pvol_partition_tasks", "pvol_render_frame_ranks", "pvol_preprocess_blocks",
           "pvol_preprocess_ranks", "pvol_get_exchange_seconds", "pvol_li_many", "pvol_set_li_coalescing",
           "pvol_get_li_coalescing_stats", "pvol_preprocess_group", "pvol_render_frame_group",
           "pvol_film_window_from_crop", "pvol_film_sample_extent", "pvol_render_tasks_window_device",
           "pvol_film_add_samples_window_device", "pvol_film_resolve_window_device", "pvol_render_frame_ranks_window",
           "pvol_render_frame_group_window", "pvol_tile_kernel_name", "pvol_set_triangle_normals",
           "pvol_compute_radiance", "pvol_compute_radiance_arrays", "pvol_radiance_lo_count", "pvol_download_radiance_lo",
           "pvol_radiance_lookup", "pvol_radiance_lookup_device", "pvol_set_surface_integrator_maps",
           "pvol_build_gather_map", "pvol_build_gather_map_arrays", "pvol_gather_map_count", "pvol_gather_photons",
           "pvol_gather_photons_device", "pvol_gather_directions", "pvol_gather_directions_device", "pvol_final_gather",
           "pvol_final_gather_device"]

SHOOT_STAT_NAMES = ["paths", "follow_calls", "no_hit", "march_steps", "interactions", "absorbed", "stored_volume",
                    "stored_caustic", "stored_direct", "stored_indirect", "split_children", "nshot"]


def partition_tasks(n_tasks, rank, n_ranks):
    n = C.c_uint32()
    _check(lib().pvol_partition_tasks(n_tasks, rank, n_ranks, None, 0, C.byref(n)), "pvol_partition_tasks")
    ids = np.zeros(n.value, np.uint32)
    _check(lib().pvol_partition_tasks(n_tasks, rank, n_ranks, ids.ctypes.data_as(_u32p), n.value, C.byref(n)), "pvol_partition_tasks")
    return ids


def _ptrs(values):
    return (C.c_void_p * len(values))(*[v or None for v in values])


def preprocess_group(pvs, n_tasks, block_paths=4096):
    _check(lib().pvol_preprocess_group(_ptrs([pv._h.value for pv in pvs]), len(pvs), n_tasks, block_paths), "pvol_preprocess_group")


def render_frame_group(pvs, cam, film, smp, d_pixels, d_rgb, hip_streams=None, window=None):
    if len(d_pixels) != len(pvs) or (hip_streams is not None and len(hip_streams) != len(pvs)):
        raise ValueError("render_frame_group: one film (and stream) per context")
    streams = None if hip_streams is None else _ptrs(list(hip_streams))
    if window is not None:
        _check(lib().pvol_render_frame_group_window(_ptrs([pv._h.value for pv in pvs]), len(pvs), C.byref(cam), C.byref(film), C.byref(window),
                                                    C.byref(smp), _ptrs(list(d_pixels)), d_rgb or None, streams), "pvol_render_frame_group_window")
        return
    _check(lib().pvol_render_frame_group(_ptrs([pv._h.value for pv in pvs]), len(pvs), C.byref(cam), C.byref(film), C.byref(smp),
                                         _ptrs(list(d_pixels)), d_rgb or None, streams), "pvol_render_frame_group")


def _check(rc, where):
    if rc != abi.PVOL_OK:
        raise PvolError(rc, where)


def photon_array(m):
    if m is None:
        return None, None
    p, w, a = (np.ascontiguousarray(x, np.float32).reshape(-1) for x in m[:3])
    n = p.size // 3
    if w.size != 3 * n or a.size != 30 * n:
        raise ValueError("photon arrays disagree: %d positions, %d directions, %d weights" % (n, w.size // 3, a.size // 30))
    return abi.PhotonArray(p.ctypes.data_as(_f32p), w.ctypes.data_as(_f32p), a.ctypes.data_as(_f32p), n, int(m[3])), (p, w, a)


def photon_arrays(maps):
    if len(maps) != 3:
        raise ValueError("three maps (caustic, direct, indirect), got %d" % len(maps))
    ptrs = (C.POINTER(abi.PhotonArray) * 3)()
    keep = []
    for i, m in enumerate(maps):
        if m is None:
            continue
        p, w, a = (np.ascontiguousarray(x, np.float32).reshape(-1) for x in m[:3])
        n = p.size // 3
        if w.size != 3 * n or a.size != 30 * n:
            raise ValueError("photon arrays disagree: %d positions, %d directions, %d weights" % (n, w.size // 3, a.size // 30))
        pa = abi.PhotonArray(p.ctypes.data_as(_f32p), w.ctypes.data_as(_f32p), a.ctypes.data_as(_f32p), n, int(m[3]))
        keep.append((pa, p, w, a))
        ptrs[i] = C.pointer(pa)
    return ptrs, keep


class PhotonVolume:

    def __init__(self, params):
        self._h = C.c_void_p()
        self.params = params
        _check(lib().pvol_create(C.byref(params), C.byref(self._h)), "pvol_create")
        self._scene = None

    def close(self):
        if getattr(self, "_h", None) and self._h.value:
            lib().pvol_destroy(self._h)
            self._h = C.c_void_p()

    def __del__(self):
        try:
            self.close()
        except Exception:
            pass

    def set_scene(self, holder):
        self._scene = holder
        _check(lib().pvol_set_scene(self._h, C.byref(holder.scene)), "pvol_set_scene")
        if getattr(holder, "tri_normals", None) is not None:
            self.set_triangle_normals(holder.tri_normals)

    def set_triangle_normals(self, n):
        if n is None:
            _check(lib().pvol_set_triangle_normals(self._h, None, 0), "pvol_set_triangle_normals")
            return
        n = np.ascontiguousarray(n, np.float32).reshape(-1, 9)
        _check(lib().pvol_set_triangle_normals(self._h, n.ctypes.data_as(_f32p), len(n)), "pvol_set_triangle_normals")

    def upload_photons(self, p, wi, alpha):
        p = np.ascontiguousarray(p, np.float32).reshape(-1)
        wi = np.ascontiguousarray(wi, np.float32).reshape(-1)
        alpha = np.ascontiguousarray(alpha, np.float32).reshape(-1)
        n = p.size // 3
        if wi.size != 3 * n or alpha.size != 30 * n:
            raise ValueError("photon arrays disagree: %d positions, %d directions, %d weights" % (n, wi.size // 3, alpha.size // 30))
        _check(lib().pvol_upload_photons(self._h, p.ctypes.data_as(_f32p), wi.ctypes.data_as(_f32p), alpha.ctypes.data_as(_f32p), n),
               "pvol_upload_photons")

    def preprocess(self, n_tasks=1, block_paths=4096):
        if block_paths == 4096:
            _check(lib().pvol_preprocess(self._h, n_tasks), "pvol_preprocess")
        else:
            _check(lib().pvol_preprocess_blocks(self._h, n_tasks, block_paths), "pvol_preprocess_blocks")

    def preprocess_ranks(self, n_tasks, rank, n_ranks, *, allgather=None, nccl_comm=None, block_paths=4096):
        comm = ShootComm()
        err = []
        cb = None
        if allgather is not None:
            def _cb(user, send, recv, nbytes):
                try:
                    parts = allgather(C.string_at(send, nbytes) if nbytes else b"")
                    if len(parts) != n_ranks or any(len(p) != nbytes for p in parts):
                        raise ValueError("allgather returned %d parts of %s bytes, wanted %d of %d"
                                         % (len(parts), sorted({len(p) for p in parts}), n_ranks, nbytes))
                    if nbytes:
                        C.memmove(recv, b"".join(parts), nbytes * n_ranks)
                    return 0
                except BaseException as e:
                    err.append(e)
                    return 1
            cb = ALLGATHER_FN(_cb)
            comm.allgather = cb
        if nccl_comm is not None:
            comm.nccl_comm = nccl_comm
        rc = lib().pvol_preprocess_ranks(self._h, n_tasks, block_paths, rank, n_ranks, C.byref(comm))
        del cb
        if err:
            raise PvolError(rc, "pvol_preprocess_ranks") from err[0]
        _check(rc, "pvol_preprocess_ranks")

    def exchange_seconds(self):
        v = C.c_double()
        _check(lib().pvol_get_exchange_seconds(self._h, C.byref(v)), "pvol_get_exchange_seconds")
        return float(v.value)

    def preprocess_times(self):
        v = (C.c_double * 2)()
        _check(lib().pvol_get_preprocess_seconds(self._h, v), "pvol_get_preprocess_seconds")
        return float(v[0]), float(v[1])

    def accel_info(self):
        v = (C.c_double * 2)()
        _check(lib().pvol_get_accel_info(self._h, v), "pvol_get_accel_info")
        return int(v[0]), float(v[1])

    def probe_hits(self, rays, mode):
        assert rays.dtype == abi.RAY_DTYPE
        rays = np.ascontiguousarray(rays)
        f = np.zeros((len(rays), 11), np.float32)
        i = np.zeros((len(rays), 3), np.int32)
        _check(lib().pvol_probe_hits(self._h, rays.ctypes.data, len(rays), mode, f.ctypes.data_as(_f32p), i.ctypes.data_as(C.POINTER(C.c_int32))),
               "pvol_probe_hits")
        return f, i

    def surface_photons(self, kind):
        n, npaths = C.c_uint32(), C.c_uint32()
        _check(lib().pvol_surface_photon_count(self._h, kind, C.byref(n), C.byref(npaths)), "pvol_surface_photon_count")
        p, wo, a = np.zeros((n.value, 3), np.float32), np.zeros((n.value, 3), np.float32), np.zeros((n.value, 30), np.float32)
        _check(lib().pvol_download_surface_photons(self._h, kind, p.ctypes.data_as(_f32p), wo.ctypes.data_as(_f32p), a.ctypes.data_as(_f32p), n.value),
               "pvol_download_surface_photons")
        return p, wo, a, int(npaths.value)

    def radiance_photons(self):
        n = C.c_uint32()
        _check(lib().pvol_radiance_photon_count(self._h, C.byref(n)), "pvol_radiance_photon_count")
        p, nn = np.zeros((n.value, 3), np.float32), np.zeros((n.value, 3), np.float32)
        rr, rt = np.zeros((n.value, 30), np.float32), np.zeros((n.value, 30), np.float32)
        _check(lib().pvol_download_radiance_photons(self._h, p.ctypes.data_as(_f32p), nn.ctypes.data_as(_f32p), rr.ctypes.data_as(_f32p),
                                                    rt.ctypes.data_as(_f32p), n.value), "pvol_download_radiance_photons")
        return p, nn, rr, rt

    def compute_radiance(self, n_lookup, max_dist, maps=None, radiance=None):
        if maps is None and radiance is None:
            _check(lib().pvol_compute_radiance(self._h, int(n_lookup), float(max_dist)), "pvol_compute_radiance")
            return
        if maps is None or radiance is None:
            raise ValueError("compute_radiance: maps and radiance go together")
        ptrs, keep = photon_arrays(maps)
        p, nn, rr, rt = (np.ascontiguousarray(x, np.float32).reshape(-1) for x in radiance)
        n = p.size // 3
        if nn.size != 3 * n or rr.size != 30 * n or rt.size != 30 * n:
            raise ValueError("radiance photon arrays disagree on their count")
        _check(lib().pvol_compute_radiance_arrays(self._h, int(n_lookup), float(max_dist), ptrs, p.ctypes.data_as(_f32p), nn.ctypes.data_as(_f32p),
                                                  rr.ctypes.data_as(_f32p), rt.ctypes.data_as(_f32p), n), "pvol_compute_radiance_arrays")
        del keep

    def radiance_lo_count(self):
        n = C.c_uint32()
        _check(lib().pvol_radiance_lo_count(self._h, C.byref(n)), "pvol_radiance_lo_count")
        return n.value

    def radiance_lo(self):
        n = self.radiance_lo_count()
        p, nn, lo = np.zeros((n, 3), np.float32), np.zeros((n, 3), np.float32), np.zeros((n, 30), np.float32)
        _check(lib().pvol_download_radiance_lo(self._h, p.ctypes.data_as(_f32p), nn.ctypes.data_as(_f32p), lo.ctypes.data_as(_f32p), n),
               "pvol_download_radiance_lo")
        return p, nn, lo

    def radiance_lookup(self, p, n):
        p = np.ascontiguousarray(p, np.float32).reshape(-1)
        n = np.ascontiguousarray(n, np.float32).reshape(-1)
        count = p.size // 3
        if n.size != 3 * count:
            raise ValueError("radiance_lookup: %d points, %d normals" % (count, n.size // 3))
        lo, found = np.zeros((count, 30), np.float32), np.zeros(count, np.uint32)
        _check(lib().pvol_radiance_lookup(self._h, p.ctypes.data_as(_f32p), n.ctypes.data_as(_f32p), count, lo.ctypes.data_as(_f32p),
                                          found.ctypes.data_as(_u32p)), "pvol_radiance_lookup")
        return lo, found

    def radiance_lookup_device(self, d_p, d_n, count, d_lo, d_found, hip_stream=0):
        _check(lib().pvol_radiance_lookup_device(self._h, d_p, d_n, count, d_lo, d_found, hip_stream), "pvol_radiance_lookup_device")

    def build_gather_map(self, indirect=None):
        if indirect is None:
            _check(lib().pvol_build_gather_map(self._h), "pvol_build_gather_map")
        else:
            p, w = (np.ascontiguousarray(x, np.float32).reshape(-1) for x in indirect[:2])
            if w.size != p.size:
                raise ValueError("build_gather_map: %d positions, %d directions" % (p.size // 3, w.size // 3))
            pa = abi.PhotonArray(p.ctypes.data_as(_f32p), w.ctypes.data_as(_f32p), None, p.size // 3, 0)
            _check(lib().pvol_build_gather_map_arrays(self._h, C.byref(pa)), "pvol_build_gather_map_arrays")
        return self.gather_map_count()

    def gather_map_count(self):
        n = C.c_uint32()
        _check(lib().pvol_gather_map_count(self._h, C.byref(n)), "pvol_gather_map_count")
        return n.value

    def gather_photons(self, p, max_dist):
        p = np.ascontiguousarray(p, np.float32).reshape(-1)
        count = p.size // 3
        index, d2 = np.zeros((count, GATHER_K), np.uint32), np.zeros((count, GATHER_K), np.float32)
        found, rounds = np.zeros(count, np.uint32), np.zeros(count, np.uint32)
        _check(lib().pvol_gather_photons(self._h, p.ctypes.data_as(_f32p), count, float(max_dist), index.ctypes.data_as(_u32p),
                                         d2.ctypes.data_as(_f32p), found.ctypes.data_as(_u32p), rounds.ctypes.data_as(_u32p)), "pvol_gather_photons")
        return index, d2, found, rounds

    def gather_photons_device(self, d_p, count, max_dist, d_index, d_d2, d_found, d_rounds, hip_stream=0):
        _check(lib().pvol_gather_photons_device(self._h, d_p, count, float(max_dist), d_index, d_d2, d_found, d_rounds, hip_stream),
               "pvol_gather_photons_device")

    def gather_directions(self, p, frames, wo, max_dist, cos_gather_angle, u_bsdf, u_photon):
        p, frames, wo = (np.ascontiguousarray(x, np.float32).reshape(-1) for x in (p, frames, wo))
        u_bsdf, u_photon = np.ascontiguousarray(u_bsdf, np.float32), np.ascontiguousarray(u_photon, np.float32)
        count = p.size // 3
        if u_bsdf.ndim != 3 or u_bsdf.shape != u_photon.shape or u_bsdf.shape[0] != count or u_bsdf.shape[2] != 3:
            raise ValueError("gather_directions: u_bsdf and u_photon are [count, n_samples, 3]")
        if frames.size != 9 * count or wo.size != 3 * count:
            raise ValueError("gather_directions: %d points, %d frames, %d wo" % (count, frames.size // 9, wo.size // 3))
        ns = u_bsdf.shape[1]
        ob, op = np.zeros((count, ns), GATHER_SAMPLE_DTYPE), np.zeros((count, ns), GATHER_SAMPLE_DTYPE)
        _check(lib().pvol_gather_directions(self._h, p.ctypes.data_as(_f32p), frames.ctypes.data_as(_f32p), wo.ctypes.data_as(_f32p), count,
                                            float(max_dist), ns, float(cos_gather_angle), u_bsdf.ctypes.data_as(_f32p), u_photon.ctypes.data_as(_f32p),
                                            ob.ctypes.data, op.ctypes.data), "pvol_gather_directions")
        return ob, op

    def gather_directions_device(self, d_p, d_frames, d_wo, count, max_dist, n_samples, cos_gather_angle, d_u_bsdf, d_u_photon, d_out_bsdf,
                                 d_out_photon, hip_stream=0):
        _check(lib().pvol_gather_directions_device(self._h, d_p, d_frames, d_wo, count, float(max_dist), int(n_samples), float(cos_gather_angle),
                                                   d_u_bsdf, d_u_photon, d_out_bsdf, d_out_photon, hip_stream), "pvol_gather_directions_device")

    def final_gather(self, p, frames, wo, kd, ray_eps, max_dist, cos_gather_angle, u_bsdf, u_photon, rays=False):
        p, frames, wo, kd, ray_eps = (np.ascontiguousarray(x, np.float32).reshape(-1) for x in (p, frames, wo, kd, ray_eps))
        u_bsdf, u_photon = np.ascontiguousarray(u_bsdf, np.float32), np.ascontiguousarray(u_photon, np.float32)
        count = p.size // 3
        if u_bsdf.ndim != 3 or u_bsdf.shape != u_photon.shape or u_bsdf.shape[0] != count or u_bsdf.shape[2] != 3:
            raise ValueError("final_gather: u_bsdf and u_photon are [count, n_samples, 3]")
        if frames.size != 9 * count or wo.size != 3 * count or kd.size != 30 * count or ray_eps.size != count:
            raise ValueError("final_gather: %d points, %d frames, %d wo, %d kd, %d ray_eps" % (count, frames.size // 9, wo.size // 3, kd.size // 30,
                                                                                             ray_eps.size))
        ns = u_bsdf.shape[1]
        L, draws = np.zeros((count, 30), np.float32), np.zeros(count, np.uint32)
        rb = np.zeros((count, ns), GATHER_RAY_DTYPE) if rays else None
        rp = np.zeros((count, ns), GATHER_RAY_DTYPE) if rays else None
        _check(lib().pvol_final_gather(self._h, p.ctypes.data_as(_f32p), frames.ctypes.data_as(_f32p), wo.ctypes.data_as(_f32p),
                                       kd.ctypes.data_as(_f32p), ray_eps.ctypes.data_as(_f32p), count, float(max_dist), ns, float(cos_gather_angle),
                                       u_bsdf.ctypes.data_as(_f32p), u_photon.ctypes.data_as(_f32p), L.ctypes.data_as(_f32p),
                                       draws.ctypes.data_as(_u32p), rb.ctypes.data if rays else None, rp.ctypes.data if rays else None),
               "pvol_final_gather")
        return (L, draws, (rb, rp)) if rays else (L, draws)

    def final_gather_device(self, d_p, d_frames, d_wo, d_kd, d_ray_eps, count, max_dist, n_samples, cos_gather_angle, d_u_bsdf, d_u_photon, d_L,
                            d_draws, d_rays_bsdf=0, d_rays_photon=0, hip_stream=0):
        _check(lib().pvol_final_gather_device(self._h, d_p, d_frames, d_wo, d_kd, d_ray_eps, count, float(max_dist), int(n_samples),
                                              float(cos_gather_angle), d_u_bsdf, d_u_photon, d_L, d_draws, d_rays_bsdf or None,
                                              d_rays_photon or None, hip_stream), "pvol_final_gather_device")

    def final_gather_set_scratch_bound(self, nbytes):
        _check(lib().pvol_final_gather_set_scratch_bound(self._h, int(nbytes)), "pvol_final_gather_set_scratch_bound")

    def check_errors(self):
        _check(lib().pvol_check_errors(self._h), "pvol_check_errors")

    def render_frame_ranks(self, cam, film, smp, rank, n_ranks, nccl_comm, d_pixels, d_rgb=0, hip_stream=0, window=None):
        if window is not None:
            _check(lib().pvol_render_frame_ranks_window(self._h, C.byref(cam), C.byref(film), C.byref(window), C.byref(smp), rank, n_ranks, nccl_comm,
                                                        d_pixels, d_rgb, hip_stream), "pvol_render_frame_ranks_window")
            return
        _check(lib().pvol_render_frame_ranks(self._h, C.byref(cam), C.byref(film), C.byref(smp), rank, n_ranks, nccl_comm, d_pixels, d_rgb, hip_stream),
               "pvol_render_frame_ranks")

    def enable_phase_timing(self, on=True):
        _check(lib().pvol_enable_phase_timing(self._h, int(bool(on))), "pvol_enable_phase_timing")

    def phase_ms(self, reset=False):
        v = (C.c_double * 6)()
        _check(lib().pvol_get_phase_ms(self._h, v, int(bool(reset))), "pvol_get_phase_ms")
        return {"tile_prepass": v[0], "march_gather": v[2], "surface": v[3], "film_add": v[4]}

    def shoot_stats(self):
        v = (C.c_uint64 * 12)()
        _check(lib().pvol_get_shoot_stats(self._h, v), "pvol_get_shoot_stats")
        return dict(zip(SHOOT_STAT_NAMES, [int(x) for x in v]))

    def photon_count(self):
        n = C.c_uint32()
        _check(lib().pvol_photon_count(self._h, C.byref(n)), "pvol_photon_count")
        return n.value

    def download_photons(self):
        n = self.photon_count()
        p = np.zeros((n, 3), np.float32)
        wi = np.zeros((n, 3), np.float32)
        alpha = np.zeros((n, 30), np.float32)
        _check(lib().pvol_download_photons(self._h, p.ctypes.data_as(_f32p), wi.ctypes.data_as(_f32p), alpha.ctypes.data_as(_f32p), n),
               "pvol_download_photons")
        return p, wi, alpha

    def li(self, rays, streams, output_kind=abi.OUT_SPECTRAL):
        rays = np.ascontiguousarray(rays)
        assert rays.dtype == abi.RAY_DTYPE and streams.dtype == abi.STREAM_DTYPE and streams.flags["C_CONTIGUOUS"]
        n = len(rays)
        out = np.zeros((n, 60 if output_kind == abi.OUT_SPECTRAL else 4), np.float32)
        draws = np.zeros(n, np.uint32)
        _check(lib().pvol_li_batch(self._h, rays.ctypes.data, n, streams.ctypes.data, len(streams), output_kind,
                                   out.ctypes.data_as(_f32p), draws.ctypes.data_as(_u32p)), "pvol_li_batch")
        return out, draws

    def li_device(self, d_rays, n_rays, d_streams, n_streams, output_kind, d_out, d_draws=0, hip_stream=0):
        _check(lib().pvol_li_batch_device(self._h, d_rays, n_rays, d_streams, n_streams, output_kind, d_out, d_draws, hip_stream),
               "pvol_li_batch_device")

    def render_tasks(self, camera, film, sampler, task_ids, d_pixels, debug=None, hip_stream=0, window=None):
        ids = np.ascontiguousarray(task_ids, np.uint32)
        if window is not None:
            _check(lib().pvol_render_tasks_window_device(self._h, C.byref(camera), C.byref(film), C.byref(window), C.byref(sampler),
                                                         ids.ctypes.data_as(_u32p), len(ids), d_pixels, C.byref(debug) if debug is not None else None,
                                                         hip_stream), "pvol_render_tasks_window_device")
            return
        _check(lib().pvol_render_tasks_device(self._h, C.byref(camera), C.byref(film), C.byref(sampler), ids.ctypes.data_as(_u32p), len(ids),
                                              d_pixels, C.byref(debug) if debug is not None else None, hip_stream), "pvol_render_tasks_device")

    def set_surface_integrator(self, n_used=50, max_dist=0.1, max_specular_depth=5, final_gather=False, caustic=None, n_paths=0,
                               from_preprocess=False, off=False, n_indirect=0):
        if off:
            _check(lib().pvol_set_surface_integrator(self._h, None, None, None, None, 0), "pvol_set_surface_integrator")
            return
        sp = abi.SurfaceParams()
        sp.n_used, sp.max_dist, sp.max_specular_depth, sp.final_gather = int(n_used), float(max_dist), int(max_specular_depth), int(bool(final_gather))
        sp.n_caustic_paths, sp.use_preprocess_store = int(n_paths), int(bool(from_preprocess))
        sp.n_indirect_photons = int(n_indirect)
        if caustic is None or from_preprocess:
            _check(lib().pvol_set_surface_integrator(self._h, C.byref(sp), None, None, None, 0), "pvol_set_surface_integrator")
            return
        p, w, a = (np.ascontiguousarray(x, np.float32) for x in caustic)
        n = p.size // 3
        assert w.size == 3 * n and a.size == 30 * n
        _check(lib().pvol_set_surface_integrator(self._h, C.byref(sp), p.ctypes.data_as(_f32p), w.ctypes.data_as(_f32p), a.ctypes.data_as(_f32p), n),
               "pvol_set_surface_integrator")

    def set_surface_integrator_maps(self, n_used=50, max_dist=0.1, max_specular_depth=5, final_gather=False, caustic=None, indirect=None,
                                    from_preprocess=False):
        sp = abi.SurfaceParams()
        sp.n_used, sp.max_dist, sp.max_specular_depth, sp.final_gather = int(n_used), float(max_dist), int(max_specular_depth), int(bool(final_gather))
        sp.use_preprocess_store = int(bool(from_preprocess))
        ca, keep_c = photon_array(caustic)
        ia, keep_i = photon_array(indirect)
        _check(lib().pvol_set_surface_integrator_maps(self._h, C.byref(sp), C.byref(ca) if ca is not None else None,
                                                      C.byref(ia) if ia is not None else None), "pvol_set_surface_integrator_maps")
        del keep_c, keep_i

    def film_add_samples(self, film, d_image_xy, d_xyz, stride, n, d_pixels, hip_stream=0, window=None):
        if window is not None:
            _check(lib().pvol_film_add_samples_window_device(self._h, C.byref(film), C.byref(window), d_image_xy, d_xyz, stride, n, d_pixels, hip_stream),
                   "pvol_film_add_samples_window_device")
            return
        _check(lib().pvol_film_add_samples_device(self._h, C.byref(film), d_image_xy, d_xyz, stride, n, d_pixels, hip_stream),
               "pvol_film_add_samples_device")

    def film_resolve(self, film, d_pixels, d_rgb, hip_stream=0, window=None):
        if window is not None:
            _check(lib().pvol_film_resolve_window_device(self._h, C.byref(film), C.byref(window), d_pixels, d_rgb, hip_stream),
                   "pvol_film_resolve_window_device")
            return
        _check(lib().pvol_film_resolve_device(self._h, C.byref(film), d_pixels, d_rgb, hip_stream), "pvol_film_resolve_device")

    def li_single(self, ray, mt, mti):
        Lv = np.zeros(30, np.float32)
        T = np.zeros(30, np.float32)
        i = C.c_int32(int(mti))
        ray = np.ascontiguousarray(ray)
        _check(lib().pvol_li(self._h, ray.ctypes.data, mt.ctypes.data_as(_u32p), C.byref(i), Lv.ctypes.data_as(_f32p), T.ctypes.data_as(_f32p)),
               "pvol_li")
        return Lv, T, i.value

    def li_many(self, rays, mt, mti):
        rays = np.ascontiguousarray(rays)
        assert rays.dtype == abi.RAY_DTYPE and mt.dtype == np.uint32 and mt.flags["C_CONTIGUOUS"]
        n = len(rays)
        assert mt.shape == (n, 624)
        mti = np.ascontiguousarray(mti, np.int32).copy()
        Lv = np.zeros((n, 30), np.float32)
        T = np.zeros((n, 30), np.float32)
        status = np.zeros(n, np.int32)
        rc = lib().pvol_li_many(self._h, rays.ctypes.data, n, mt.ctypes.data_as(_u32p), mti.ctypes.data_as(C.POINTER(C.c_int32)),
                                Lv.ctypes.data_as(_f32p), T.ctypes.data_as(_f32p), status.ctypes.data_as(C.POINTER(C.c_int32)))
        if rc != abi.PVOL_OK and not (status != abi.PVOL_OK).any():
            _check(rc, "pvol_li_many")
        return Lv, T, mti, status

    def set_li_coalescing(self, max_batch, max_wait_us=0):
        _check(lib().pvol_set_li_coalescing(self._h, int(max_batch), int(max_wait_us)), "pvol_set_li_coalescing")

    def li_coalescing_stats(self, reset=False):
        v = (C.c_uint64 * 6)()
        _check(lib().pvol_get_li_coalescing_stats(self._h, v, int(reset)), "pvol_get_li_coalescing_stats")
        return dict(zip(["calls", "batches", "largest_batch", "queued_behind", "batches_redone", "calls_failed"], (int(x) for x in v)))

    def transmittance(self, rays, streams):
        rays = np.ascontiguousarray(rays)
        n = len(rays)
        out = np.zeros((n, 30), np.float32)
        _check(lib().pvol_transmittance_batch(self._h, rays.ctypes.data, n, streams.ctypes.data, len(streams), out.ctypes.data_as(_f32p)),
               "pvol_transmittance_batch")
        return out

    def enable_stats(self, on=True):
        _check(lib().pvol_enable_stats(self._h, int(on)), "pvol_enable_stats")

    def stats(self, reset=False):
        s = abi.Stats()
        _check(lib().pvol_get_stats(self._h, C.byref(s), int(reset)), "pvol_get_stats")
        return {k: int(getattr(s, k)) for k, _ in abi.Stats._fields_}

    def march_kernel_name(self):
        return lib().pvol_march_kernel_name(self._h).decode()

    def tile_kernel_name(self):
        return lib().pvol_tile_kernel_name(self._h).decode()

    def kernel_time_ms(self, reset=False):
        avg = C.c_double()
        n = C.c_uint64()
        _check(lib().pvol_kernel_time_ms(self._h, C.byref(avg), C.byref(n), int(reset)), "pvol_kernel_time_ms")
        return avg.value, n.value


def gaussian_filter_table(xwidth=2.0, ywidth=2.0, alpha=2.0):
    t = np.zeros(256, np.float32)
    lib().pvol_gaussian_filter_table(xwidth, ywidth, alpha, t.ctypes.data_as(_f32p))
    return t


def sub_window(sampler, task):
    w = (C.c_int32 * 4)()
    lib().pvol_compute_sub_window(C.byref(sampler), task, w)
    return list(w)


def film_window_from_crop(film, crop):
    c = np.ascontiguousarray(crop, np.float32).reshape(-1)
    if c.size != 4:
        raise ValueError("cropwindow takes four numbers (x0 x1 y0 y1), got %d" % c.size)
    w = abi.FilmWindow()
    _check(lib().pvol_film_window_from_crop(C.byref(film), c.ctypes.data_as(_f32p), C.byref(w)), "pvol_film_window_from_crop")
    return w


def film_sample_extent(film, window=None):
    e = (C.c_int32 * 4)()
    _check(lib().pvol_film_sample_extent(C.byref(film), C.byref(window) if window is not None else None, e), "pvol_film_sample_extent")
    return list(e)


def render_sample_count(sampler, task_ids):
    ids = np.ascontiguousarray(task_ids, np.uint32)
    return int(lib().pvol_render_sample_count(C.byref(sampler), ids.ctypes.data_as(_u32p), len(ids)))
```

### include/pvol.h

```cpp
#ifndef PVOL_H
#define PVOL_H

#include <stddef.h>
#include <stdint.h>

#ifdef __cplusplus
extern "C" {
#endif

#define PVOL_NBINS 30
#define PVOL_MT_N 624
#define PVOL_ABI_VERSION 3

typedef enum pvol_status {
    PVOL_OK = 0,
    PVOL_E_INVALID = -1,
    PVOL_E_NO_DEVICE = -2,
    PVOL_E_NO_SCENE = -3,
    PVOL_E_NO_MEMORY = -4,
    PVOL_E_UNSUPPORTED = -5,
    PVOL_E_LIMIT = -6,
    PVOL_E_SHOOT_FAILED = -7
} pvol_status;

typedef struct pvol_spectrum { float c[PVOL_NBINS]; } pvol_spectrum;


typedef enum pvol_volume_kind {
    PVOL_VOLUME_NONE = 0,
    PVOL_VOLUME_HOMOGENEOUS = 1,
    PVOL_VOLUME_GRID = 2,
    PVOL_VOLUME_RAINBOW = 3,
    PVOL_VOLUME_EXPONENTIAL = 4
} pvol_volume_kind;

typedef struct pvol_volume {
    int32_t kind;
    float extent_min[3], extent_max[3];
    float world_to_volume[16];
    float volume_to_world[16];
    pvol_spectrum sigma_a, sigma_s, le;
    float g;
    int32_t nx, ny, nz;
    const float *density;
} pvol_volume;

typedef enum pvol_light_kind {
    PVOL_LIGHT_POINT = 0,
    PVOL_LIGHT_SPOT = 1,
    PVOL_LIGHT_DISTANT = 2
} pvol_light_kind;

typedef struct pvol_light {
    int32_t kind;
    float pos[3];
    float dir[3];
    float light_to_world[16];
    float world_to_light[16];
    pvol_spectrum intensity;
    float cos_total_width;
    float cos_falloff_start;
} pvol_light;

typedef enum pvol_material_kind {
    PVOL_MATERIAL_MATTE = 0,
    PVOL_MATERIAL_GLASS = 1
} pvol_material_kind;

typedef struct pvol_material {
    int32_t kind;
    pvol_spectrum kd;
    pvol_spectrum kr;
    pvol_spectrum kt;
    float ior;
    float vn;
} pvol_material;

typedef struct pvol_triangle {
    float p[3][3];
    int32_t material;
    int32_t flip_normal;
} pvol_triangle;

typedef struct pvol_sphere {
    float object_to_world[16];
    float world_to_object[16];
    float radius;
    float z_min, z_max;
    float theta_min, theta_max;
    float phi_max;
    int32_t material;
    int32_t flip_normal;
} pvol_sphere;

typedef struct pvol_scene {
    pvol_volume volume;
    uint32_t n_lights;
    const pvol_light *lights;
    uint32_t n_triangles;
    const pvol_triangle *triangles;
    uint32_t n_materials;
    const pvol_material *materials;
    float world_min[3], world_max[3];
    pvol_spectrum cie_x, cie_y, cie_z;
    float xyz_scale;
    uint32_t n_spheres;
    const pvol_sphere *spheres;
} pvol_scene;

typedef struct pvol_params {
    float step_size;
    int32_t n_used;
    float max_dist;
    uint32_t n_volume_photons;
    float shooter_step_size;
    int32_t max_photon_depth;
    uint32_t n_caustic_photons;
    uint32_t n_indirect_photons;
    int32_t final_gather;
    int32_t device;
    float grid_cell_scale;
    uint32_t keep_surface_photons;
    uint32_t reserved[6];
} pvol_params;


typedef struct pvol_ray {
    float o[3];
    float mint;
    float d[3];
    float maxt;
    float time;
    float scatter_u;
    uint32_t rng_skip;
    uint32_t flags;
} pvol_ray;

typedef struct pvol_stream {
    uint32_t seed;
    uint32_t first_ray;
    uint32_t n_rays;
    uint32_t reserved;
    uint64_t start_draw;
    uint64_t end_draw;
} pvol_stream;

typedef enum pvol_output_kind {
    PVOL_OUT_SPECTRAL = 0,
    PVOL_OUT_XYZ = 1
} pvol_output_kind;

typedef struct pvol_stats {
    uint64_t n_rays;
    uint64_t n_steps;
    uint64_t n_tested;
    uint64_t n_kept;
    uint64_t n_lookups_lt10;
    uint64_t n_shadow_unoccluded;
    uint64_t n_guess_retries;
    uint64_t cy_search;
    uint64_t cy_select;
    uint64_t cy_flux;
    uint64_t cy_total;
    uint64_t group_guess_failed;
    uint64_t group_plan_skipped;
    uint64_t cy_fallback;
    uint64_t group_deferred_overflow;
    uint64_t group_deferred_too_few;
    uint64_t group_attempts;
} pvol_stats;

#define PVOL_MAX_SAMPLE_ARRAYS 16
#define PVOL_FILTER_TABLE_SIZE 16
#define PVOL_MAX_PIXEL_SAMPLES 1024

typedef struct pvol_camera {
    float raster_to_camera[16];
    float camera_to_world[16];
    float shutter_open, shutter_close;
    float lens_radius;
    float focal_distance;
} pvol_camera;

typedef struct pvol_film {
    int32_t x_resolution, y_resolution;
    float filter_xwidth, filter_ywidth;
    float filter_table[PVOL_FILTER_TABLE_SIZE * PVOL_FILTER_TABLE_SIZE];
} pvol_film;

typedef struct pvol_film_window {
    int32_t x_pixel_start, y_pixel_start;
    int32_t x_pixel_count, y_pixel_count;
} pvol_film_window;

typedef struct pvol_sampler {
    int32_t x_start, x_end, y_start, y_end;
    uint32_t pixel_samples;
    uint32_t n_tasks;
    uint32_t n1d_count, n2d_count;
    uint32_t n1d[PVOL_MAX_SAMPLE_ARRAYS], n2d[PVOL_MAX_SAMPLE_ARRAYS];
    uint32_t tau_index, scatter_index;
} pvol_sampler;

typedef struct pvol_render_debug {
    pvol_ray *d_rays;
    float *d_image_xy;
    float *d_xyz;
    pvol_stream *d_streams;
    float *d_surf_xyz;
} pvol_render_debug;

typedef struct pvol_surface_params {
    int32_t n_used;
    float max_dist;
    int32_t max_specular_depth;
    int32_t final_gather;
    uint32_t n_caustic_paths;
    int32_t use_preprocess_store;
    uint32_t n_indirect_photons;
    uint32_t reserved[1];
} pvol_surface_params;

typedef struct pvol_ctx pvol_ctx;

int pvol_abi_version(void);
const char *pvol_strerror(int status);
int pvol_device_count(void);

void pvol_default_params(pvol_params *p);

int pvol_create(const pvol_params *params, pvol_ctx **out);
void pvol_destroy(pvol_ctx *ctx);

int pvol_set_scene(pvol_ctx *ctx, const pvol_scene *scene);

int pvol_set_triangle_normals(pvol_ctx *ctx, const float *n, uint32_t n_triangles);

int pvol_upload_photons(pvol_ctx *ctx, const float *p, const float *wi,
                        const float *alpha, uint32_t n);

int pvol_preprocess(pvol_ctx *ctx, uint32_t n_tasks);

int pvol_preprocess_blocks(pvol_ctx *ctx, uint32_t n_tasks, uint32_t block_paths);

typedef struct pvol_shoot_comm {
    void *nccl_comm;
    int (*allgather)(void *user, const void *send, void *recv, uint64_t bytes);
    void *user;
} pvol_shoot_comm;

int pvol_preprocess_ranks(pvol_ctx *ctx, uint32_t n_tasks, uint32_t block_paths, uint32_t rank, uint32_t n_ranks,
                          const pvol_shoot_comm *comm);

int pvol_get_exchange_seconds(pvol_ctx *ctx, double *out);

int pvol_get_shoot_stats(pvol_ctx *ctx, uint64_t *out12);

int pvol_get_preprocess_seconds(pvol_ctx *ctx, double *out2);

int pvol_get_accel_info(pvol_ctx *ctx, double *out2);

int pvol_surface_photon_count(pvol_ctx *ctx, int kind, uint32_t *n, uint32_t *n_paths);
int pvol_download_surface_photons(pvol_ctx *ctx, int kind, float *p, float *wo, float *alpha, uint32_t capacity);
int pvol_radiance_photon_count(pvol_ctx *ctx, uint32_t *n);
int pvol_download_radiance_photons(pvol_ctx *ctx, float *p, float *n, float *rho_r, float *rho_t, uint32_t capacity);

typedef struct pvol_photon_array {
    const float *p, *wi, *alpha; uint32_t n; uint32_t n_paths;
} pvol_photon_array;

int pvol_compute_radiance(pvol_ctx *ctx, int32_t n_lookup, float max_dist);

int pvol_compute_radiance_arrays(pvol_ctx *ctx, int32_t n_lookup, float max_dist, const pvol_photon_array *const maps[3],
                                 const float *rp_p, const float *rp_n, const float *rho_r, const float *rho_t, uint32_t n_rp);

int pvol_radiance_lo_count(pvol_ctx *ctx, uint32_t *n);
int pvol_download_radiance_lo(pvol_ctx *ctx, float *p, float *n, float *lo, uint32_t capacity);

int pvol_radiance_lookup(pvol_ctx *ctx, const float *p, const float *n, uint32_t count, float *lo, uint32_t *found);
int pvol_radiance_lookup_device(pvol_ctx *ctx, const float *d_p, const float *d_n, uint32_t count, float *d_lo,
                                uint32_t *d_found, void *hip_stream);


int pvol_build_gather_map(pvol_ctx *ctx);
int pvol_build_gather_map_arrays(pvol_ctx *ctx, const pvol_photon_array *indirect);
int pvol_gather_map_count(pvol_ctx *ctx, uint32_t *n);

int pvol_gather_photons(pvol_ctx *ctx, const float *p, uint32_t count, float max_dist, uint32_t *index, float *d2, uint32_t *found,
                        uint32_t *rounds);
int pvol_gather_photons_device(pvol_ctx *ctx, const float *d_p, uint32_t count, float max_dist, uint32_t *d_index, float *d_d2,
                               uint32_t *d_found, uint32_t *d_rounds, void *hip_stream);

typedef struct pvol_gather_sample {
    float wi[3], weight, bsdf_pdf, photon_pdf; uint32_t photon_index, valid;
} pvol_gather_sample;

int pvol_gather_directions(pvol_ctx *ctx, const float *p, const float *frames, const float *wo, uint32_t count, float max_dist,
                           int32_t n_samples, float cos_gather_angle, const float *u_bsdf, const float *u_photon,
                           pvol_gather_sample *out_bsdf, pvol_gather_sample *out_photon);
int pvol_gather_directions_device(pvol_ctx *ctx, const float *d_p, const float *d_frames, const float *d_wo, uint32_t count,
                                  float max_dist, int32_t n_samples, float cos_gather_angle, const float *d_u_bsdf,
                                  const float *d_u_photon, pvol_gather_sample *d_out_bsdf, pvol_gather_sample *d_out_photon,
                                  void *hip_stream);


typedef struct pvol_gather_ray {
    float t, n_gather[3];
    uint32_t radiance_index;
    int32_t prim;
    uint32_t hit, drew;
} pvol_gather_ray;

#define PVOL_FINAL_GATHER_SCRATCH_BYTES (256ull << 20)

int pvol_final_gather(pvol_ctx *ctx, const float *p, const float *frames, const float *wo, const float *kd, const float *ray_eps,
                      uint32_t count, float max_dist, int32_t n_samples, float cos_gather_angle, const float *u_bsdf,
                      const float *u_photon, float *L, uint32_t *draws, pvol_gather_ray *rays_bsdf, pvol_gather_ray *rays_photon);
int pvol_final_gather_device(pvol_ctx *ctx, const float *d_p, const float *d_frames, const float *d_wo, const float *d_kd,
                             const float *d_ray_eps, uint32_t count, float max_dist, int32_t n_samples, float cos_gather_angle,
                             const float *d_u_bsdf, const float *d_u_photon, float *d_L, uint32_t *d_draws,
                             pvol_gather_ray *d_rays_bsdf, pvol_gather_ray *d_rays_photon, void *hip_stream);

int pvol_photon_count(pvol_ctx *ctx, uint32_t *n);
int pvol_download_photons(pvol_ctx *ctx, float *p, float *wi, float *alpha, uint32_t capacity);

int pvol_li_batch(pvol_ctx *ctx, const pvol_ray *rays, uint32_t n_rays,
                  pvol_stream *streams, uint32_t n_streams,
                  int output_kind, float *out, uint32_t *draws);

int pvol_li_batch_device(pvol_ctx *ctx, const pvol_ray *d_rays, uint32_t n_rays,
                         pvol_stream *d_streams, uint32_t n_streams,
                         int output_kind, float *d_out, uint32_t *d_draws,
                         void *hip_stream);

int pvol_check_errors(pvol_ctx *ctx);

int pvol_li(pvol_ctx *ctx, const pvol_ray *ray, uint32_t *mt, int32_t *mti,
            float *Lv, float *T);

int pvol_li_many(pvol_ctx *ctx, const pvol_ray *rays, uint32_t n, uint32_t *mt, int32_t *mti,
                 float *Lv, float *T, int32_t *status);

int pvol_set_li_coalescing(pvol_ctx *ctx, uint32_t max_batch, uint32_t max_wait_us);
int pvol_get_li_coalescing_stats(pvol_ctx *ctx, uint64_t *out6, int reset);

int pvol_transmittance_batch(pvol_ctx *ctx, const pvol_ray *rays, uint32_t n_rays,
                             pvol_stream *streams, uint32_t n_streams, float *out);

int pvol_get_stats(pvol_ctx *ctx, pvol_stats *out, int reset);
int pvol_enable_stats(pvol_ctx *ctx, int on);

int pvol_kernel_time_ms(pvol_ctx *ctx, double *avg_ms, uint64_t *launches, int reset);
const char *pvol_march_kernel_name(pvol_ctx *ctx);
const char *pvol_tile_kernel_name(pvol_ctx *ctx);

int pvol_enable_phase_timing(pvol_ctx *ctx, int on);
int pvol_get_phase_ms(pvol_ctx *ctx, double *out6, int reset);

void pvol_gaussian_filter_table(float xwidth, float ywidth, float alpha, float *table256);

void pvol_compute_sub_window(const pvol_sampler *s, uint32_t task, int32_t out[4]);

uint64_t pvol_render_sample_count(const pvol_sampler *s, const uint32_t *task_ids, uint32_t n_task_ids);

int pvol_render_tasks_device(pvol_ctx *ctx, const pvol_camera *camera, const pvol_film *film,
                             const pvol_sampler *sampler, const uint32_t *task_ids, uint32_t n_task_ids,
                             float *d_pixels, const pvol_render_debug *debug, void *hip_stream);

int pvol_set_surface_integrator(pvol_ctx *ctx, const pvol_surface_params *sp, const float *p, const float *wo,
                                const float *alpha, uint32_t n);

int pvol_set_surface_integrator_maps(pvol_ctx *ctx, const pvol_surface_params *sp, const pvol_photon_array *caustic,
                                     const pvol_photon_array *indirect);

int pvol_partition_tasks(uint32_t n_tasks, uint32_t rank, uint32_t n_ranks, uint32_t *out_ids, uint32_t capacity, uint32_t *n_out);

int pvol_render_frame_ranks(pvol_ctx *ctx, const pvol_camera *camera, const pvol_film *film, const pvol_sampler *sampler,
                            uint32_t rank, uint32_t n_ranks, void *nccl_comm, float *d_pixels, float *d_rgb, void *hip_stream);


int pvol_preprocess_group(pvol_ctx *const *ctxs, uint32_t n_ctx, uint32_t n_tasks, uint32_t block_paths);

int pvol_render_frame_group(pvol_ctx *const *ctxs, uint32_t n_ctx, const pvol_camera *camera, const pvol_film *film,
                            const pvol_sampler *sampler, float *const *d_pixels, float *d_rgb, void *const *hip_streams);

int pvol_film_add_samples_device(pvol_ctx *ctx, const pvol_film *film, const float *d_image_xy,
                                 const float *d_xyz, uint32_t xyz_stride, uint64_t n,
                                 float *d_pixels, void *hip_stream);

int pvol_film_resolve_device(pvol_ctx *ctx, const pvol_film *film, const float *d_pixels, float *d_rgb,
                             void *hip_stream);


int pvol_film_window_from_crop(const pvol_film *film, const float *crop4, pvol_film_window *out);

int pvol_film_sample_extent(const pvol_film *film, const pvol_film_window *window, int32_t out[4]);

int pvol_render_tasks_window_device(pvol_ctx *ctx, const pvol_camera *camera, const pvol_film *film, const pvol_film_window *window,
                                    const pvol_sampler *sampler, const uint32_t *task_ids, uint32_t n_task_ids,
                                    float *d_pixels, const pvol_render_debug *debug, void *hip_stream);

int pvol_film_add_samples_window_device(pvol_ctx *ctx, const pvol_film *film, const pvol_film_window *window, const float *d_image_xy,
                                        const float *d_xyz, uint32_t xyz_stride, uint64_t n, float *d_pixels, void *hip_stream);
int pvol_film_resolve_window_device(pvol_ctx *ctx, const pvol_film *film, const pvol_film_window *window, const float *d_pixels,
                                    float *d_rgb, void *hip_stream);

int pvol_render_frame_ranks_window(pvol_ctx *ctx, const pvol_camera *camera, const pvol_film *film, const pvol_film_window *window,
                                   const pvol_sampler *sampler, uint32_t rank, uint32_t n_ranks, void *nccl_comm, float *d_pixels,
                                   float *d_rgb, void *hip_stream);
int pvol_render_frame_group_window(pvol_ctx *const *ctxs, uint32_t n_ctx, const pvol_camera *camera, const pvol_film *film,
                                   const pvol_film_window *window, const pvol_sampler *sampler, float *const *d_pixels, float *d_rgb,
                                   void *const *hip_streams);

#ifdef __cplusplus
}
#endif
#endif
```

Measured before the change: 146.8.

## Add plain specialized COUNT tile pre-pass for simple distant-light box scenes

Adds a host-side gate that picks a PLAIN template variant of the COUNT-mode tile kernels when the scene has a homogeneous or rainbow extent, a distant first light, no BVH, no spheres, no surface integrator and no specular linking. The PLAIN variant compiles out the BVH, sphere, surface, region-density and general light-visibility branches and always takes the precomputed shadow-row path. It also uses its own waves-per-task heuristic with different thresholds. This is meant to cut register pressure and branching in the pre-pass, at the cost of an extra template instantiation, a new environment override, and the risk that the gate misclassifies a scene.

```diff
diff --git a/cs348b-pbrt_amd/csrc/pvol_api.hip b/cs348b-pbrt_amd/csrc/pvol_api.hip
--- a/cs348b-pbrt_amd/csrc/pvol_api.hip
+++ b/cs348b-pbrt_amd/csrc/pvol_api.hip
@@ -68,6 +68,7 @@
     { const char *ng = getenv("PVOL_NO_GROUP"); c->noGroup = ng && ng[0] == '1'; }
     { const char *nl = getenv("PVOL_NO_LITE"); c->noLite = nl && nl[0] == '1'; }
     { const char *nm = getenv("PVOL_NO_MOMENTS"); c->noMoments = nm && nm[0] == '1'; }
+    { const char *tg = getenv("PVOL_TILE_GENERAL"); c->tileGeneral = tg && tg[0] == '1'; }
     { const char *gw = getenv("PVOL_GROUP_WAVES"); if (gw) c->groupWavesPerCU = std::max(1, atoi(gw)); }
     { const char *tw = getenv("PVOL_TILE_WAVES"); if (tw) c->tileWaves = std::max(0, atoi(tw)); }
     { const char *fw = getenv("PVOL_FIX_WAVES"); if (fw) c->fixWavesPerCU = std::max(1, atoi(fw)); }
@@ -145,10 +146,22 @@
     return p;
 }
 
+int pvol_tile_plain_gate(const TilePlainIn *in) {
+    const bool extent = in->volKind == PVOL_VOLUME_HOMOGENEOUS || in->volKind == PVOL_VOLUME_RAINBOW;
+    return in->tile == PVOL_TILE_COUNT && !in->tileGeneral && extent && in->nLights > 0 &&
+           in->light0Kind == PVOL_LIGHT_DISTANT && !in->hasBvh && in->nSpheres == 0 && in->nTris >= 0 && in->nTris <= PVOL_MAX_TRIS &&
+           !in->surfOn && !in->specLink;
+}
+
 static int tile_waves_per_task(const PlanIn &in) {
     if (in.tileWaves > 0) return in.tileWaves;
     const double perCU = (double)in.nStreams / (double)std::max(1, in.nCU);
     return perCU >= 12.0 ? 1 : (perCU >= 3.0 ? 2 : 4);
+}
+static int tile_waves_per_task_plain(uint32_t nStreams, int nCU, int tileWaves) {
+    if (tileWaves > 0) return tileWaves;
+    const double perCU = (double)nStreams / (double)std::max(1, nCU);
+    return perCU > 16.0 ? 1 : (perCU >= 6.0 ? 2 : 4);
 }
 
 void plan_size(const PlanIn &in, BatchPlan &p) {
@@ -393,7 +406,15 @@
 
 static int run_tile_count(pvol_ctx *c, const BatchArgs &b, const BatchPlan &p, const LiArgs &t, const TileArgs *tile) {
     pvol_phase_mark(c, b.stream, PVOL_PHASE_TILE);
-    return ok(pvol_launchers(c->hs.volKind).tile(&t, tile, false, p.ldsTile, c->hs.candCap, b.stream, p.tileWavesPerTask, &c->lastTileKernel)) ? PVOL_OK : PVOL_E_NO_DEVICE;
+    const DevScene &h = c->hs;
+    TilePlainIn g = {};
+    g.tile = p.tile; g.volKind = h.volKind; g.nLights = h.nLights; g.light0Kind = h.nLights > 0 ? h.lights[0].kind : -1;
+    g.hasBvh = h.bvhNodes != 0; g.nSpheres = h.nSpheres; g.nTris = h.nTris; g.surfOn = h.surf.enabled != 0;
+    g.specLink = tile->specOn || tile->specLink != 0; g.tileGeneral = c->tileGeneral;
+    const bool plain = pvol_tile_plain_gate(&g) != 0;
+    c->lastTileForm = plain ? "plain" : "general";
+    const int waves = plain ? tile_waves_per_task_plain(b.nStreams, c->nCU, c->tileWaves) : p.tileWavesPerTask;
+    return ok(pvol_launchers(h.volKind).tile(&t, tile, false, p.ldsTile, h.candCap, b.stream, waves, plain, &c->lastTileKernel)) ? PVOL_OK : PVOL_E_NO_DEVICE;
 }
 static int run_par(pvol_ctx *c, const BatchArgs &b, const BatchPlan &p, LiArgs &a) {
     const RegionLaunchers &K = pvol_launchers(c->hs.volKind);
@@ -423,7 +444,8 @@
         if (p.specCap && spec_pool_reset(c, tile, p.specCap, b.stream) != PVOL_OK) return PVOL_E_NO_DEVICE;
         if (p.tile == PVOL_TILE_FUSED) {
             pvol_phase_mark(c, b.stream, PVOL_PHASE_TILE);
-            if (!ok(K.tile(&a, tile, true, p.ldsTile, c->hs.candCap, b.stream, p.tileWavesPerTask, &c->lastTileKernel))) return PVOL_E_NO_DEVICE;
+            c->lastTileForm = "general";
+            if (!ok(K.tile(&a, tile, true, p.ldsTile, c->hs.candCap, b.stream, p.tileWavesPerTask, false, &c->lastTileKernel))) return PVOL_E_NO_DEVICE;
         }
         pvol_phase_mark(c, b.stream, PVOL_PHASE_MARCH);
         if (!ok(K.liSlice(&a, p.ldsResolve, p.ldsPar, c->hs.candCap, c->statsOn, p.nWaves, b.stream, p.resolve != 0, p.groupForm, p.ldsGroup,
@@ -642,6 +664,7 @@
 
 const char *pvol_march_kernel_name(pvol_ctx *c) { return c ? c->lastKernel : ""; }
 const char *pvol_tile_kernel_name(pvol_ctx *c) { return c ? c->lastTileKernel : ""; }
+const char *pvol_tile_form_name(pvol_ctx *c) { return c ? c->lastTileForm : ""; }
 
 int pvol_enable_phase_timing(pvol_ctx *c, int on) {
     if (!c) return PVOL_E_INVALID;
diff --git a/cs348b-pbrt_amd/csrc/pvol_host.h b/cs348b-pbrt_amd/csrc/pvol_host.h
--- a/cs348b-pbrt_amd/csrc/pvol_host.h
+++ b/cs348b-pbrt_amd/csrc/pvol_host.h
@@ -58,7 +58,7 @@
 extern "C" hipError_t pvol_launch_surface(const SurfArgs *a, uint32_t nWaves, hipStream_t stream);
 extern "C" size_t pvol_tile_lds_bytes(int maxSteps, uint32_t spp, bool fused, int nTris, bool shadowRows);
 extern "C" hipError_t pvol_launch_tile(const LiArgs *args, const TileArgs *tile, bool fused, size_t ldsBytes, int candCap, hipStream_t stream, int wavesPerTask,
-                                       const char **form);
+                                       bool plain, const char **form);
 extern "C" hipError_t pvol_launch_li_par(const LiArgs *args, size_t ldsBytes, int candCap, bool stats, uint32_t nWaves, hipStream_t stream);
 struct RegionLaunchers {
     decltype(&pvol_launch_li_seq) liSeq;
@@ -80,7 +80,7 @@
 extern "C" hipError_t pvol_launch_li_par_exp(const LiArgs *args, size_t ldsBytes, int candCap, bool stats, uint32_t nWaves, hipStream_t stream);
 extern "C" hipError_t pvol_launch_surface_exp(const SurfArgs *a, uint32_t nWaves, hipStream_t stream);
 extern "C" hipError_t pvol_launch_tile_exp(const LiArgs *args, const TileArgs *tile, bool fused, size_t ldsBytes, int candCap, hipStream_t stream,
-                                           int wavesPerTask, const char **form);
+                                           int wavesPerTask, bool plain, const char **form);
 static inline const RegionLaunchers &pvol_launchers(int volKind) {
     static const RegionLaunchers base = {pvol_launch_li_seq, pvol_launch_li_slice, pvol_launch_li_group, pvol_launch_li_replay, pvol_launch_li_par,
                                          pvol_launch_surface, pvol_launch_tile};
@@ -162,6 +162,8 @@
     bool noLite = false;
     const char *lastKernel = "";
     const char *lastTileKernel = "";
+    const char *lastTileForm = "";
+    bool tileGeneral = false;
     int fixWavesPerCU = 16;
     int groupWavesPerCU = 12;
     bool noGroup = false;
@@ -263,6 +265,15 @@
 extern "C" BatchPlan plan_path(const PlanIn &in);
 extern "C" void plan_size(const PlanIn &in, BatchPlan &p);
 #define GRP_FORM_MOMENTS 3
+struct TilePlainIn {
+    int32_t tile;
+    int32_t volKind, nLights, light0Kind;
+    int32_t hasBvh, nSpheres, nTris;
+    int32_t surfOn, specLink;
+    int32_t tileGeneral;
+};
+static_assert(sizeof(TilePlainIn) == 40, "tests/test_tile_plain_gate.py mirrors it");
+extern "C" int pvol_tile_plain_gate(const TilePlainIn *in);
 extern "C" int pvol_moment_gate(const float *sigA, const float *sigS, double pathBound);
 struct MomentWeights { float w[12][32]; };
 extern "C" int pvol_moment_scene(DevScene &h, MomentWeights *w);
diff --git a/cs348b-pbrt_amd/csrc/pvol_tile_dev.h b/cs348b-pbrt_amd/csrc/pvol_tile_dev.h
--- a/cs348b-pbrt_amd/csrc/pvol_tile_dev.h
+++ b/cs348b-pbrt_amd/csrc/pvol_tile_dev.h
@@ -129,6 +129,7 @@
     return C;
 }
 
+template <bool PLAIN = false>
 __device__ uint32_t tile_count_draws(const DevScene &S, const CountConsts &C, const float *ltri, const float *trows, V3 o, V3 d, float maxt, float scatterU, bool blackS, bool lightBlack, uint32_t dbg = 0u,
                                      int slice = 0, int nSlices = 1, float mint = 0.f) {
     float t0, t1;
@@ -140,8 +141,9 @@
     const bool tryLight = !blackS && C.nLights > 0 && !lightBlack;
     const uint32_t fixedDraws = slice == 0 ? 4u + 7u * (uint32_t)nSamples : 0u;
     if (!tryLight || (dbg & 16u)) return fixedDraws;
-    if (trows && !C.bvh && !C.nSpheres && !(dbg & 8u)) {
+    if (PLAIN || (trows && !C.bvh && !C.nSpheres && !(dbg & 8u))) {
         const V3 ld = v3(C.ldir[0], C.ldir[1], C.ldir[2]);
+        const int nT = (PLAIN && (dbg & 8u)) ? 0 : C.nTris;
         for (int j = 0; j < nSamples; j += 2) {
             const V3 pA = o + d * tcur;
             tcur += step;
@@ -150,11 +152,11 @@
             if (nSlices > 1 && ((j >> 1) % nSlices) != slice) continue;
             const V3 pvA = xform_point(C.w2v, pA), pvB = xform_point(C.w2v, pB);
             bool inA, inB = j + 1 < nSamples;
-            if (is_region(C.volKind)) { inA = region_density(S, pvA) != 0.f; inB = inB && region_density(S, pvB) != 0.f; }
+            if (!PLAIN && is_region(C.volKind)) { inA = region_density(S, pvA) != 0.f; inB = inB && region_density(S, pvB) != 0.f; }
             else { inA = box_inside(C.lo, C.hi, pvA); inB = inB && box_inside(C.lo, C.hi, pvB); }
             if (!inA && !inB) continue;
             bool occA = false, occB = false;
-            for (int t = 0; t < C.nTris; ++t) {
+            for (int t = 0; t < nT; ++t) {
                 const f4 r0 = *reinterpret_cast<const f4 *>(trows + 16 * t), r1 = *reinterpret_cast<const f4 *>(trows + 16 * t + 4),
                          r2 = *reinterpret_cast<const f4 *>(trows + 16 * t + 8), r3 = *reinterpret_cast<const f4 *>(trows + 16 * t + 12);
                 TriPre tp;
@@ -167,49 +169,51 @@
         }
         return fixedDraws + u;
     }
-    for (int j = 0; j < nSamples; ++j) {
-        const V3 p = o + d * tcur;
-        tcur += step;
-        if (nSlices > 1 && (j % nSlices) != slice) continue;
-        const V3 pv = xform_point(C.w2v, p);
-        if (is_region(C.volKind) ? region_density(S, pv) == 0.f : !box_inside(C.lo, C.hi, pv)) continue;
-        RayD vis;
-        if (C.lightKind == PVOL_LIGHT_DISTANT) {
-            vis.o = p; vis.d = v3(C.ldir[0], C.ldir[1], C.ldir[2]); vis.mint = 0.f; vis.maxt = INFINITY;
-        } else {
-            const V3 lp = v3(C.lpos[0], C.lpos[1], C.lpos[2]);
-            const V3 wo = normalize(lp - p);
-            const float dist = len(p - lp);
-            vis.o = p; vis.d = vdiv(lp - p, dist); vis.mint = 0.f; vis.maxt = dist * (1.f - 0.f);
-            if (C.lightKind == PVOL_LIGHT_SPOT) {
-                V3 wl = normalize(v3(C.w2l[0] * -wo.x + C.w2l[1] * -wo.y + C.w2l[2] * -wo.z,
-                                     C.w2l[3] * -wo.x + C.w2l[4] * -wo.y + C.w2l[5] * -wo.z,
-                                     C.w2l[6] * -wo.x + C.w2l[7] * -wo.y + C.w2l[8] * -wo.z));
-                const float costheta = wl.z;
-                float fall = 1.f;
-                if (costheta < C.cosTotalWidth) fall = 0.f;
-                else if (!(costheta > C.cosFalloffStart)) {
-                    const float delta = (costheta - C.cosTotalWidth) / (C.cosFalloffStart - C.cosTotalWidth);
-                    fall = delta * delta * delta * delta;
+    if constexpr (!PLAIN) {
+        for (int j = 0; j < nSamples; ++j) {
+            const V3 p = o + d * tcur;
+            tcur += step;
+            if (nSlices > 1 && (j % nSlices) != slice) continue;
+            const V3 pv = xform_point(C.w2v, p);
+            if (is_region(C.volKind) ? region_density(S, pv) == 0.f : !box_inside(C.lo, C.hi, pv)) continue;
+            RayD vis;
+            if (C.lightKind == PVOL_LIGHT_DISTANT) {
+                vis.o = p; vis.d = v3(C.ldir[0], C.ldir[1], C.ldir[2]); vis.mint = 0.f; vis.maxt = INFINITY;
+            } else {
+                const V3 lp = v3(C.lpos[0], C.lpos[1], C.lpos[2]);
+                const V3 wo = normalize(lp - p);
+                const float dist = len(p - lp);
+                vis.o = p; vis.d = vdiv(lp - p, dist); vis.mint = 0.f; vis.maxt = dist * (1.f - 0.f);
+                if (C.lightKind == PVOL_LIGHT_SPOT) {
+                    V3 wl = normalize(v3(C.w2l[0] * -wo.x + C.w2l[1] * -wo.y + C.w2l[2] * -wo.z,
+                                         C.w2l[3] * -wo.x + C.w2l[4] * -wo.y + C.w2l[5] * -wo.z,
+                                         C.w2l[6] * -wo.x + C.w2l[7] * -wo.y + C.w2l[8] * -wo.z));
+                    const float costheta = wl.z;
+                    float fall = 1.f;
+                    if (costheta < C.cosTotalWidth) fall = 0.f;
+                    else if (!(costheta > C.cosFalloffStart)) {
+                        const float delta = (costheta - C.cosTotalWidth) / (C.cosFalloffStart - C.cosTotalWidth);
+                        fall = delta * delta * delta * delta;
+                    }
+                    if (fall == 0.f) continue;
                 }
-                if (fall == 0.f) continue;
             }
-        }
-        bool occ = false;
-        if (C.nSpheres && spheres_occluded(S, vis.o, vis.d, vis.mint, vis.maxt)) {
-            occ = true;
-        } else if (C.bvh) {
-            occ = bvh_occluded(S, vis.o, vis.d, vis.mint, vis.maxt);
-        } else if (trows) {
-            if (!(dbg & 8u)) occ = tri_rows_occluded(trows, C.nTris, vis.o, vis.d, vis.mint, vis.maxt);
-        } else {
-            for (int t = 0; t < ((dbg & 8u) ? 0 : C.nTris); ++t) {
-                const f4 a = *reinterpret_cast<const f4 *>(ltri + 12 * t), b = *reinterpret_cast<const f4 *>(ltri + 12 * t + 4),
-                         c = *reinterpret_cast<const f4 *>(ltri + 12 * t + 8);
-                occ = occ | tri_hit_v(v3(a.x, a.y, a.z), v3(a.w, b.x, b.y), v3(b.z, b.w, c.x), vis);
+            bool occ = false;
+            if (C.nSpheres && spheres_occluded(S, vis.o, vis.d, vis.mint, vis.maxt)) {
+                occ = true;
+            } else if (C.bvh) {
+                occ = bvh_occluded(S, vis.o, vis.d, vis.mint, vis.maxt);
+            } else if (trows) {
+                if (!(dbg & 8u)) occ = tri_rows_occluded(trows, C.nTris, vis.o, vis.d, vis.mint, vis.maxt);
+            } else {
+                for (int t = 0; t < ((dbg & 8u) ? 0 : C.nTris); ++t) {
+                    const f4 a = *reinterpret_cast<const f4 *>(ltri + 12 * t), b = *reinterpret_cast<const f4 *>(ltri + 12 * t + 4),
+                             c = *reinterpret_cast<const f4 *>(ltri + 12 * t + 8);
+                    occ = occ | tri_hit_v(v3(a.x, a.y, a.z), v3(a.w, b.x, b.y), v3(b.z, b.w, c.x), vis);
+                }
             }
-        }
-        if (!occ) ++u;
+            if (!occ) ++u;
+        }
     }
     return fixedDraws + u;
 }
@@ -296,8 +300,9 @@
     }
 };
 
-template <bool FUSED, int NREG, bool SPEC>
+template <bool FUSED, int NREG, bool SPEC, bool PLAIN = false>
 __global__ __launch_bounds__(LANES, FUSED ? 2 : 4) void tile_kernel(LiArgs A, TileArgs T) {
+    static_assert(!PLAIN || (!FUSED && !SPEC), "PLAIN is a form of the COUNT-mode pre-pass without the specular recursion");
     extern __shared__ __align__(16) unsigned char lds[];
     const DevScene &S = *A.scene;
     const int lane = threadIdx.x;
@@ -322,7 +327,7 @@
     }
     __syncthreads();
     float *trows = 0;
-    if (!FUSED && S.nLights > 0 && S.lights[0].kind == PVOL_LIGHT_DISTANT) {
+    if (PLAIN || (!FUSED && S.nLights > 0 && S.lights[0].kind == PVOL_LIGHT_DISTANT)) {
         trows = ltri + S.nTris * 12;
         tri_rows_prepare(S, v3(S.lights[0].dir[0], S.lights[0].dir[1], S.lights[0].dir[2]), trows, lane);
     }
@@ -352,8 +357,8 @@
     const bool blackS = spec_is_black(ld4(S.sigS, q));
     const bool lightBlack = S.nLights > 0 ? spec_is_black(ld4(S.lights[0].intensity, q)) : true;
     unsigned blackMask = 0u;
-    for (int l = 0; l < S.nLights; ++l) if (spec_is_black(ld4(S.lights[l].intensity, q))) blackMask |= 1u << l;
-    const bool surfOn = S.surf.enabled != 0;
+    if (!PLAIN) for (int l = 0; l < S.nLights; ++l) if (spec_is_black(ld4(S.lights[l].intensity, q))) blackMask |= 1u << l;
+    const bool surfOn = !PLAIN && S.surf.enabled != 0;
     pvol_ray *rays = T.rays;
     const CountConsts CC = count_consts(S);
     for (uint32_t k = begin; k < end; k += T.spp) {
@@ -377,9 +382,9 @@
                 tm = lerpf(L.time[i], T.shutterOpen, T.shutterClose);
                 su = L.scatter[i];
                 tile_camera_ray(T, imageX, imageY, &o, &d);
-                if (S.bvhNodes) { float th; if (bvh_closest(S, o, d, 0.f, INFINITY, &th) >= 0) maxt = th; }
+                if (!PLAIN && S.bvhNodes) { float th; if (bvh_closest(S, o, d, 0.f, INFINITY, &th) >= 0) maxt = th; }
                 else maxt = tile_clip(ltri, S.nTris, o, d);
-                if (S.nSpheres) { V3 ph; spheres_closest(S, o, d, 0.f, &maxt, &ph); }
+                if (!PLAIN && S.nSpheres) { V3 ph; spheres_closest(S, o, d, 0.f, &maxt, &ph); }
                 uint32_t link = 0u;
                 if (surfOn && maxt < INFINITY) {
                     SurfHit sh;
@@ -389,7 +394,7 @@
                         else glass = 1;
                     }
                 }
-                if (!FUSED && T.specLink) T.specLink[ri] = link;
+                if (!PLAIN && !FUSED && T.specLink) T.specLink[ri] = link;
                 pvol_ray pr;
                 pr.o[0] = o.x; pr.o[1] = o.y; pr.o[2] = o.z; pr.mint = 0.f;
                 pr.d[0] = d.x; pr.d[1] = d.y; pr.d[2] = d.z; pr.maxt = maxt;
@@ -399,7 +404,7 @@
                 T.xy[2 * ri + 1] = imageY;
             }
             if (!FUSED) {
-                uint32_t nd = (on && !(T.debugSkip & 2u)) ? tile_count_draws(S, CC, ltri, trows, o, d, maxt, su, blackS, lightBlack, T.debugSkip) : ((T.debugSkip & 2u) ? 270u : 0u);
+                uint32_t nd = (on && !(T.debugSkip & 2u)) ? tile_count_draws<PLAIN>(S, CC, ltri, trows, o, d, maxt, su, blackS, lightBlack, T.debugSkip) : ((T.debugSkip & 2u) ? 270u : 0u);
                 unsigned long long tot = nd + surfDraws;
                 for (int off = 32; off > 0; off >>= 1) tot += __shfl_xor(tot, off);
                 if (!(T.debugSkip & 4u)) rng_skip<true, true, true>(rng, tot, lane);
@@ -469,8 +474,9 @@
     }
 }
 
-template <int NW, bool SPEC>
+template <int NW, bool SPEC, bool PLAIN = false>
 __global__ __launch_bounds__(LANES * NW, (NW >= 8 ? 4 : 2)) void tile_mw_kernel(LiArgs A, TileArgs T, uint32_t partOff) {
+    static_assert(!PLAIN || !SPEC, "PLAIN has no specular recursion");
     extern __shared__ __align__(16) unsigned char lds[];
     constexpr bool W1 = (NW == 1);
     const DevScene &S = *A.scene;
@@ -485,7 +491,7 @@
     L.oth = reinterpret_cast<uint32_t *>(L.scatter + T.spp);
     const size_t triOff = (((size_t)MT_N * 4 + (size_t)T.spp * 5 * 4) + 15) & ~(size_t)15;
     float *ltri = reinterpret_cast<float *>(lds + triOff);
-    const bool shadowRows = S.nLights > 0 && S.lights[0].kind == PVOL_LIGHT_DISTANT;
+    const bool shadowRows = PLAIN || (S.nLights > 0 && S.lights[0].kind == PVOL_LIGHT_DISTANT);
     const size_t partHere = (triOff + (size_t)S.nTris * 12 * 4 + (shadowRows ? (size_t)S.nTris * 16 * 4 : 0) + 64 + 15) & ~(size_t)15;
     unsigned long long *part = reinterpret_cast<unsigned long long *>(lds + partHere);
     for (int i = tid; i < S.nTris * 12; i += LANES * NW) {
@@ -495,7 +501,7 @@
     }
     __syncthreads();
     float *trows = 0;
-    if (S.nLights > 0 && S.lights[0].kind == PVOL_LIGHT_DISTANT) {
+    if (shadowRows) {
         trows = ltri + S.nTris * 12;
         tri_rows_prepare(S, v3(S.lights[0].dir[0], S.lights[0].dir[1], S.lights[0].dir[2]), trows, tid);
     }
@@ -512,8 +518,8 @@
     const bool blackS = spec_is_black(ld4(S.sigS, q));
     const bool lightBlack = S.nLights > 0 ? spec_is_black(ld4(S.lights[0].intensity, q)) : true;
     unsigned blackMask = 0u;
-    for (int l = 0; l < S.nLights; ++l) if (spec_is_black(ld4(S.lights[l].intensity, q))) blackMask |= 1u << l;
-    const bool surfOn = S.surf.enabled != 0;
+    if (!PLAIN) for (int l = 0; l < S.nLights; ++l) if (spec_is_black(ld4(S.lights[l].intensity, q))) blackMask |= 1u << l;
+    const bool surfOn = !PLAIN && S.surf.enabled != 0;
     pvol_ray *rays = T.rays;
     const CountConsts CC = count_consts(S);
     const int groupsPerPixel = (int)((T.spp + LANES - 1) / LANES);
@@ -539,9 +545,9 @@
             V3 o, d;
             tile_camera_ray(T, imageX, imageY, &o, &d);
             float maxt = INFINITY;
-            if (S.bvhNodes) { float th; if (bvh_closest(S, o, d, 0.f, INFINITY, &th) >= 0) maxt = th; }
+            if (!PLAIN && S.bvhNodes) { float th; if (bvh_closest(S, o, d, 0.f, INFINITY, &th) >= 0) maxt = th; }
             else maxt = tile_clip(ltri, S.nTris, o, d);
-            if (S.nSpheres) { V3 ph; spheres_closest(S, o, d, 0.f, &maxt, &ph); }
+            if (!PLAIN && S.nSpheres) { V3 ph; spheres_closest(S, o, d, 0.f, &maxt, &ph); }
             if (slice == 0) {
                 uint32_t surfDraws = 0u;
                 const size_t ri = (size_t)st.first_ray + k + i;
@@ -550,7 +556,7 @@
                     SurfHit sh;
                     if (surf_closest(S, o, d, 0.f, &sh)) surfDraws = tile_surface_draws<SPEC>(S, T, CC, ltri, trows, sh, d, su, tm, ri, blackS, lightBlack, blackMask, A.counters, &link);
                 }
-                if (T.specLink) T.specLink[ri] = link;
+                if (!PLAIN && T.specLink) T.specLink[ri] = link;
                 pvol_ray pr;
                 pr.o[0] = o.x; pr.o[1] = o.y; pr.o[2] = o.z; pr.mint = 0.f;
                 pr.d[0] = d.x; pr.d[1] = d.y; pr.d[2] = d.z; pr.maxt = maxt;
@@ -560,7 +566,7 @@
                 T.xy[2 * ri + 1] = imageY;
                 mine += surfDraws;
             }
-            if (!(T.debugSkip & 2u)) mine += tile_count_draws(S, CC, ltri, trows, o, d, maxt, su, blackS, lightBlack, 0u, slice, NSL);
+            if (!(T.debugSkip & 2u)) mine += tile_count_draws<PLAIN>(S, CC, ltri, trows, o, d, maxt, su, blackS, lightBlack, 0u, slice, NSL);
             else if (slice == 0) mine += 270ull;
         }
         for (int off = 32; off > 0; off >>= 1) mine += __shfl_xor(mine, off);
@@ -580,27 +586,36 @@
            (shadowRows ? (size_t)nTris * 16 * 4 : 0) + 64;
 }
 
-template <bool SPEC>
+template <bool SPEC, bool PLAIN>
 static hipError_t launch_tile_t(const LiArgs *args, const TileArgs *tile, bool fused, size_t ldsBytes, int candCap, hipStream_t stream, int wavesPerTask,
                                 const char **form) {
     dim3 grid(args->nStreams), block(LANES);
     if (!fused && wavesPerTask > 1 && args->state == 0 && args->sliceK == 0) {
         const uint32_t partOff = (uint32_t)((ldsBytes + 15) & ~(size_t)15);
         const size_t bytes = partOff + 16 * 8;
-        if (wavesPerTask >= 16) { *form = "tile_mw_kernel<16>"; hipLaunchKernelGGL((tile_mw_kernel<16, SPEC>), grid, dim3(LANES * 16), bytes, stream, *args, *tile, partOff); }
-        else if (wavesPerTask >= 8) { *form = "tile_mw_kernel<8>"; hipLaunchKernelGGL((tile_mw_kernel<8, SPEC>), grid, dim3(LANES * 8), bytes, stream, *args, *tile, partOff); }
-        else if (wavesPerTask >= 4) { *form = "tile_mw_kernel<4>"; hipLaunchKernelGGL((tile_mw_kernel<4, SPEC>), grid, dim3(LANES * 4), bytes, stream, *args, *tile, partOff); }
-        else { *form = "tile_mw_kernel<2>"; hipLaunchKernelGGL((tile_mw_kernel<2, SPEC>), grid, dim3(LANES * 2), bytes, stream, *args, *tile, partOff); }
+        if (wavesPerTask >= 16) { *form = "tile_mw_kernel<16>"; hipLaunchKernelGGL((tile_mw_kernel<16, SPEC, PLAIN>), grid, dim3(LANES * 16), bytes, stream, *args, *tile, partOff); }
+        else if (wavesPerTask >= 8) { *form = "tile_mw_kernel<8>"; hipLaunchKernelGGL((tile_mw_kernel<8, SPEC, PLAIN>), grid, dim3(LANES * 8), bytes, stream, *args, *tile, partOff); }
+        else if (wavesPerTask >= 4) { *form = "tile_mw_kernel<4>"; hipLaunchKernelGGL((tile_mw_kernel<4, SPEC, PLAIN>), grid, dim3(LANES * 4), bytes, stream, *args, *tile, partOff); }
+        else { *form = "tile_mw_kernel<2>"; hipLaunchKernelGGL((tile_mw_kernel<2, SPEC, PLAIN>), grid, dim3(LANES * 2), bytes, stream, *args, *tile, partOff); }
         return hipGetLastError();
     }
     *form = fused ? "tile_kernel<fused>" : "tile_kernel<count>";
-    if (!fused) hipLaunchKernelGGL((tile_kernel<false, 4, SPEC>), grid, block, ldsBytes, stream, *args, *tile);
+    if (!fused) hipLaunchKernelGGL((tile_kernel<false, 4, SPEC, PLAIN>), grid, block, ldsBytes, stream, *args, *tile);
+    else if constexpr (PLAIN) return hipErrorInvalidValue;
     else if (candCap <= 4 * LANES) hipLaunchKernelGGL((tile_kernel<true, 4, SPEC>), grid, block, ldsBytes, stream, *args, *tile);
     else hipLaunchKernelGGL((tile_kernel<true, 12, SPEC>), grid, block, ldsBytes, stream, *args, *tile);
     return hipGetLastError();
 }
 extern "C" hipError_t pvol_launch_tile(const LiArgs *args, const TileArgs *tile, bool fused, size_t ldsBytes, int candCap, hipStream_t stream, int wavesPerTask,
-                                       const char **form) {
-    return tile->specOn ? launch_tile_t<true>(args, tile, fused, ldsBytes, candCap, stream, wavesPerTask, form)
-                        : launch_tile_t<false>(args, tile, fused, ldsBytes, candCap, stream, wavesPerTask, form);
-}
+                                       bool plain, const char **form) {
+    if (plain) {
+#if PVOL_REGION_EXP
+        return hipErrorInvalidValue;
+#else
+        if (fused || tile->specOn || tile->specLink) return hipErrorInvalidValue;
+        return launch_tile_t<false, true>(args, tile, false, ldsBytes, candCap, stream, wavesPerTask, form);
+#endif
+    }
+    return tile->specOn ? launch_tile_t<true, false>(args, tile, fused, ldsBytes, candCap, stream, wavesPerTask, form)
+                        : launch_tile_t<false, false>(args, tile, fused, ldsBytes, candCap, stream, wavesPerTask, form);
+}
diff --git a/cs348b-pbrt_amd/pvol.py b/cs348b-pbrt_amd/pvol.py
--- a/cs348b-pbrt_amd/pvol.py
+++ b/cs348b-pbrt_amd/pvol.py
@@ -159,6 +159,8 @@
         L.pvol_march_kernel_name.restype = C.c_char_p
         L.pvol_tile_kernel_name.argtypes = [C.c_void_p]
         L.pvol_tile_kernel_name.restype = C.c_char_p
+        L.pvol_tile_form_name.argtypes = [C.c_void_p]
+        L.pvol_tile_form_name.restype = C.c_char_p
         L.pvol_gaussian_filter_table.argtypes = [C.c_float, C.c_float, C.c_float, _f32p]
         L.pvol_gaussian_filter_table.restype = None
         L.pvol_compute_sub_window.argtypes = [C.POINTER(abi.Sampler), C.c_uint32, C.POINTER(C.c_int32)]
@@ -205,7 +207,7 @@
            "pvol_get_li_coalescing_stats", "pvol_preprocess_group", "pvol_render_frame_group",
            "pvol_film_window_from_crop", "pvol_film_sample_extent", "pvol_render_tasks_window_device",
            "pvol_film_add_samples_window_device", "pvol_film_resolve_window_device", "pvol_render_frame_ranks_window",
-           "pvol_render_frame_group_window", "pvol_tile_kernel_name", "pvol_set_triangle_normals",
+           "pvol_render_frame_group_window", "pvol_tile_kernel_name", "pvol_tile_form_name", "pvol_set_triangle_normals",
            "pvol_compute_radiance", "pvol_compute_radiance_arrays", "pvol_radiance_lo_count", "pvol_download_radiance_lo",
            "pvol_radiance_lookup", "pvol_radiance_lookup_device", "pvol_set_surface_integrator_maps",
            "pvol_build_gather_map", "pvol_build_gather_map_arrays", "pvol_gather_map_count", "pvol_gather_photons",
@@ -672,6 +674,9 @@
     def tile_kernel_name(self):
         return lib().pvol_tile_kernel_name(self._h).decode()
 
+    def tile_form_name(self):
+        return lib().pvol_tile_form_name(self._h).decode()
+
     def kernel_time_ms(self, reset=False):
         avg = C.c_double()
         n = C.c_uint64()
diff --git a/include/pvol.h b/include/pvol.h
--- a/include/pvol.h
+++ b/include/pvol.h
@@ -353,6 +353,7 @@
 int pvol_kernel_time_ms(pvol_ctx *ctx, double *avg_ms, uint64_t *launches, int reset);
 const char *pvol_march_kernel_name(pvol_ctx *ctx);
 const char *pvol_tile_kernel_name(pvol_ctx *ctx);
+const char *pvol_tile_form_name(pvol_ctx *ctx);
 
 int pvol_enable_phase_timing(pvol_ctx *ctx, int on);
 int pvol_get_phase_ms(pvol_ctx *ctx, double *out6, int reset);
```

After: 149.1, median of 6. 1.6% higher.
